# MiRaCLeXeoN/sduss

Measured on AMD Instinct MI355X. Metric: images/sec (node), SDXL 1024^2 50-step, fixed prompt, CFG, higher is better.
Workload: dtype bf16; 1 GPU; SDXL-base-1.0 UNet 1024x1024 50-step Euler, CFG 5.0, 4 requests/step (denoiser batch 8) per GPU, is_sliced=False, random-init weights of the real architecture (2.57 B params), one data-parallel replica per GPU, no collective; resolution=1024, steps_per_image=50

## Files before the change

### include/mxdenoise.h

```cpp
#ifndef MXDENOISE_H
#define MXDENOISE_H

#include <stddef.h>
#include <stdint.h>

#ifdef __cplusplus
extern "C" {
#endif

enum { MX_F32 = 0, MX_F16 = 1, MX_BF16 = 2 };

const char* mx_last_error(void);
int mx_version(void);
#define MX_PROF_KINDS 12
int mx_profile_enable(int on);
int mx_profile_collect(double* out);
int mx_profile_records(double* out, int max_records);

size_t mx_groupnorm_halo_workspace_bytes(int N, int C, int cpg);
int mx_groupnorm_halo(void* stream, const void* x, const void* gamma, const void* beta, void* y,
                      int N, int C, int H, int W, int cpg, double eps, int padding,
                      const int32_t* latent_offset, int n_latents, const int32_t* patch_map,
                      const int32_t* padding_idx, int dtype, void* workspace);
int mx_halo_only(void* stream, const void* x, void* y, int N, int C, int H, int W,
                 const int32_t* padding_idx, int dtype);


enum {
  MX_EPI_SILU     = 1 << 0,
  MX_EPI_GEGLU    = 1 << 1,
  MX_EPI_OUT_F32  = 1 << 2,
  MX_EPI_QKV      = 1 << 3,
  MX_EPI_GELU_TANH = 1 << 4,
  MX_EPI_RES_BCAST = 1 << 5,
  MX_EPI_RMSNORM  = 1 << 6,
  MX_EPI_GELU     = 1 << 7,
  MX_EPI_QUICK_GELU = 1 << 8,
  MX_EPI_GEGLU_TANH = 1 << 9
};

#define MX_MAX_SEGS 4
typedef struct mx_gemm_seg {
  const void* a;
  const void* a2;
  void* c;
  const void* residual;
  void* vt;
  const float* rowbias;
  const float* gate;
  const float* ln_stats;
  float* stats_out;
  int M;
  int rows_per_batch;
  int ldvt;
  int B, Hin, Win, Hout, Wout;
  int a_batch_rows, a_row_off, c_batch_rows, c_row_off;
} mx_gemm_seg;

typedef struct mx_gemm_desc {
  const void* a;
  const void* w;
  void* c;
  const float* bias;
  const float* rowbias;
  const void* residual;
  void* vt;
  int M, N, K;
  int lda, ldc, ldr, ldrb;
  int rows_per_batch;
  int flags;
  int seg, period, ldvt;
  int B, Hin, Win, Cin;
  int Hout, Wout;
  int stride;
  int up;
  int corner_patch;
  int a_batch_rows, a_row_off, c_batch_rows, c_row_off;
  const float* gate;
  int ldg;
  float out_scale;
  const float* rms_wq;
  const float* rms_wk;
  float rms_eps;
  int vhalo;
  const void* a2;
  int lda2, k_split;
  const float* ln_stats;
  const float* ln_colsum;
  int ln_slabs;
  float ln_eps;
  float* stats_out;
  const mx_gemm_seg* segs;
  int n_segs;
  int splitk;
  const float* ln_final;
  float* ln_final_out;
  unsigned* ln_final_cnt;
  float* gn_part_out;
  int cin_valid;
} mx_gemm_desc;

int mx_gemm(void* stream, const mx_gemm_desc* d);
int mx_gemm_launches(const mx_gemm_desc* d);
int mx_gemm_stats_slabs(const mx_gemm_desc* d);
int mx_gemm_ln_prefers_pass(const mx_gemm_desc* d);
int mx_gemm_ln_final_supported(const mx_gemm_desc* d);
int mx_gemm_gn_partials_supported(const mx_gemm_desc* d, int conv);
enum { MX_FORM_TILE_GENERIC = 0, MX_FORM_TILE_256 = 1, MX_FORM_TILE_128 = 2, MX_FORM_PERSISTENT_256 = 3, MX_FORM_SMALL_M = 4, MX_FORM_CONV_SMALL_N = 5, MX_FORM_CONV_SMALL_CIN = 6 };
int mx_gemm_form(const mx_gemm_desc* d, int conv);
int mx_gemm_kernel_name(const mx_gemm_desc* d, int conv, int launch, char* buf, int cap);
int mx_gemm_kernel_names(char* buf, int cap);
int mx_attention_kernel_name(int B, int H, int Lq, int Lk, int ldo, int prescaled, int causal, int bias, int key_chunk, int force_cross, char* buf, int cap);
int mx_attention_kernel_names(char* buf, int cap);
#define MX_STATS_PITCH(slabs) (((slabs) + 3) & ~3)
int mx_row_stats(void* stream, const void* x, int ldx, float* stats, int M, int C);
int mx_conv3x3(void* stream, const mx_gemm_desc* d);
int mx_gemm_splitk(const mx_gemm_desc* d, int conv);
void mx_gemm_release_scratch(void* stream, int all);

typedef struct mx_attn_tail_desc {
  mx_gemm_desc out1, to_q, out2;
  const void* k; int ldk;
  const void* vt; int ldvt; int64_t vt_batch_stride;
  int B, heads, L, ctx_len;
  unsigned* sync;
} mx_attn_tail_desc;
size_t mx_attn_tail_sync_bytes(int M);
int mx_attn_tail_supported(const mx_attn_tail_desc* d);
int mx_attn_tail_preferred(void);
int mx_attn_tail(void* stream, const mx_attn_tail_desc* d);
int mx_attn_tail_status(void* stream, const unsigned* sync, unsigned* word);

#define MX_VT_POS(key) (((key) & ~12) | (((key) & 4) << 1) | (((key) & 8) >> 1))
#define MX_VT_LD(Lk) (((Lk) + 15) / 16 * 16)

int mx_attention(void* stream, const void* q, int ldq, const void* k, int ldk, const void* vt, int ldvt,
                 int64_t vt_batch_stride, void* o, int ldo, int B, int H, int Lq, int Lk, float scale);
#define MX_ATTN_QSCALE(scale) ((scale) * 1.4426950408889634f)
int mx_attention_prescaled(void* stream, const void* q, int ldq, const void* k, int ldk, const void* vt, int ldvt,
                           int64_t vt_batch_stride, void* o, int ldo, int B, int H, int Lq, int Lk);
int mx_attention_cross_prescaled(void* stream, const void* q, int ldq, const void* k, int ldk, const void* vt, int ldvt,
                                 int64_t vt_batch_stride, void* o, int ldo, int B, int H, int Lq, int Lk);
typedef struct mx_attn_problem {
  const void* q; const void* k; const void* vt; void* o;
  int64_t vt_batch_stride;
  int B, Lq, Lk, ldvt;
} mx_attn_problem;
int mx_attention_prescaled_grouped(void* stream, const mx_attn_problem* probs, int n, int ldq, int ldk, int ldo, int H);
int mx_attention_prescaled_bias(void* stream, const void* q, int ldq, const void* k, int ldk, const void* vt, int ldvt,
                                int64_t vt_batch_stride, void* o, int ldo, int B, int H, int Lq, int Lk, const float* bias, int ldb);
int mx_attention_prescaled_causal(void* stream, const void* q, int ldq, const void* k, int ldk, const void* vt, int ldvt,
                                  int64_t vt_batch_stride, void* o, int ldo, int B, int H, int L);

int mx_layernorm(void* stream, const void* x, void* y, const float* gamma, const float* beta,
                 int M, int C, float eps);

int mx_rmsnorm(void* stream, const void* x, void* y, const float* w, int M, int C, float eps);

int mx_layernorm_mod(void* stream, const void* x, void* y, void* y2, const float* scale, const float* shift,
                     const float* scale2, const float* shift2, int ldmod, int M, int C, int rows_per_batch, float eps);
int mx_layernorm_mod_grouped(void* stream, const void* x, void* y, void* y2, const float* scale, const float* shift, const float* scale2,
                             const float* shift2, int ldmod, int C, float eps, const int* batches, const int* rows_per_batch, int n);
int mx_rmsnorm_heads(void* stream, void* x, int ld, int nbatch, int rows_per_batch, int batch_rows, int row_off,
                     int heads_total, int heads_q, const float* wq, const float* wk, float eps, float q_scale);

size_t mx_groupnorm_nhwc_workspace_bytes(int B, int H, int W, int C);
int mx_groupnorm_nhwc(void* stream, const void* x, void* y, const float* gamma, const float* beta,
                      int B, int H, int W, int C, int groups, float eps, int silu, int patch,
                      void* workspace);

int mx_groupnorm_nhwc_cat(void* stream, const void* x, int C1, const void* x2, void* y, const float* gamma, const float* beta,
                          int B, int H, int W, int C, int groups, float eps, int silu, int patch, void* workspace);
int mx_groupnorm_nhwc_from_partials(void* stream, const void* x, void* y, const float* gamma, const float* beta, int B, int H, int W, int C, int groups, float eps,
                                    int silu, const float* part, int chunk, const float* add_bias, const float* add_rowbias, int ldrb, void* workspace);

typedef struct mx_gn_problem { const void* x; const void* x2; void* y; int B, H, W; } mx_gn_problem;
size_t mx_groupnorm_nhwc_grouped_workspace_bytes(const mx_gn_problem* probs, int n, int C);
int mx_groupnorm_nhwc_grouped(void* stream, const mx_gn_problem* probs, int n, int C1, const float* gamma, const float* beta, int C, int groups,
                              float eps, int silu, int patch, void* workspace);

typedef struct mx_unet_config {
  int in_channels, out_channels;
  int n_levels;
  int block_out_channels[4];
  int layers_per_block;
  int down_has_attn[4];
  int transformer_layers[4];
  int num_heads[4];
  int cross_attention_dim;
  int addition_time_embed_dim;
  int projection_class_embeddings_input_dim;
  int norm_num_groups;
  float norm_eps, transformer_norm_eps, layer_norm_eps;
} mx_unet_config;

typedef struct mx_weight_entry {
  const char* name;
  uint64_t offset;
  uint64_t bytes;
} mx_weight_entry;

typedef struct mx_unet mx_unet;

mx_unet* mx_unet_create(const mx_unet_config* cfg);
void mx_unet_destroy(mx_unet* u);
int mx_unet_set_weights(mx_unet* u, const void* blob, uint64_t blob_bytes,
                        const mx_weight_entry* table, int n_entries);
int mx_unet_set_context_key(mx_unet* u, uint64_t key);
int mx_unet_context_stats(const mx_unet* u, long* hits, long* misses);
size_t mx_unet_workspace_bytes(const mx_unet* u, int batch, int H, int W, int ctx_len);
int mx_unet_validate(const mx_unet* u, int batch, int H, int W, int ctx_len);
int mx_unet_forward(mx_unet* u, void* stream, const void* latents, int io_dtype, const float* timesteps,
                    const void* ehs, const void* text_embeds, const float* time_ids, void* out,
                    int batch, int H, int W, int ctx_len, int gn_patch, void* workspace, size_t workspace_bytes);
typedef struct mx_unet_group { const void* latents; void* out; int batch, H, W; } mx_unet_group;
size_t mx_unet_workspace_bytes_mixed(const mx_unet* u, const mx_unet_group* groups, int n_groups, int ctx_len);
int mx_unet_forward_mixed(mx_unet* u, void* stream, const mx_unet_group* groups, int n_groups, int io_dtype, const float* timesteps,
                          const void* ehs, const void* text_embeds, const float* time_ids, int ctx_len, int gn_patch, void* workspace,
                          size_t workspace_bytes);
int mx_unet_forward_mixed_trace(mx_unet* u, void* stream, const mx_unet_group* groups, int n_groups, int io_dtype, const float* timesteps,
                                const void* ehs, const void* text_embeds, const float* time_ids, int ctx_len, int gn_patch, void* workspace,
                                size_t workspace_bytes, const char* stage, void* stage_out, size_t stage_out_bytes);
int mx_unet_forward_trace(mx_unet* u, void* stream, const void* latents, int io_dtype, const float* timesteps,
                          const void* ehs, const void* text_embeds, const float* time_ids, void* out,
                          int batch, int H, int W, int ctx_len, int gn_patch, void* workspace,
                          size_t workspace_bytes, const char* stage, void* stage_out, size_t stage_out_bytes);

typedef int (*mx_allgather_fn)(void* ctx, void* stream, const void* send, void* recv, size_t bytes_per_rank);
typedef struct mx_pp_comm { int rank, world; mx_allgather_fn all_gather; void* ctx; } mx_pp_comm;
size_t mx_unet_workspace_bytes_pp(const mx_unet* u, int batch, int H_local, int W, int ctx_len, int world);
int mx_unet_forward_pp(mx_unet* u, void* stream, const void* latents_local, int io_dtype, const float* timesteps, const void* ehs,
                       const void* text_embeds, const float* time_ids, void* out_local, int batch, int H_local, int W, int ctx_len,
                       const mx_pp_comm* comm, void* workspace, size_t workspace_bytes);
#define MX_PP_SYNC 0
#define MX_PP_WARMUP 1
#define MX_PP_STALE 2
typedef int (*mx_allgather_inplace_fn)(void* ctx, void* stream, void* region, size_t bytes_per_rank);
typedef struct mx_pp_stale { void* state; size_t state_bytes; int mode; int corrected_gn; mx_allgather_inplace_fn all_gather_async; } mx_pp_stale;
size_t mx_unet_pp_state_bytes(const mx_unet* u, int batch, int H_local, int W, int ctx_len, int world);
int mx_unet_forward_pp_stale(mx_unet* u, void* stream, const void* latents_local, int io_dtype, const float* timesteps, const void* ehs,
                             const void* text_embeds, const float* time_ids, void* out_local, int batch, int H_local, int W, int ctx_len,
                             const mx_pp_comm* comm, const mx_pp_stale* stale, void* workspace, size_t workspace_bytes);
int mx_unet_pp_comm_plan(const mx_unet* u, int batch, int H_local, int W, int ctx_len, const mx_pp_comm* comm);
int mx_attention_prescaled_chunked(void* stream, const void* q, int ldq, const void* k, int ldk, const void* vt, int ldvt,
                                   int64_t vt_batch_stride, void* o, int ldo, int B, int H, int Lq, int Lk, int key_chunk,
                                   int64_t k_batch_stride, int64_t k_chunk_stride, int64_t vt_chunk_stride);

typedef struct mx_mmdit_config {
  int patch_size, in_channels, out_channels;
  int num_layers;
  int num_attention_heads;
  int joint_attention_dim, pooled_projection_dim, pos_embed_max_size;
  int dual_attention[64];
  float norm_eps;
} mx_mmdit_config;

typedef struct mx_mmdit mx_mmdit;
mx_mmdit* mx_mmdit_create(const mx_mmdit_config* cfg);
void mx_mmdit_destroy(mx_mmdit* u);
int mx_mmdit_set_weights(mx_mmdit* u, const void* blob, uint64_t blob_bytes, const mx_weight_entry* table, int n_entries);
size_t mx_mmdit_workspace_bytes(const mx_mmdit* u, int batch, int H, int W, int ctx_len);
int mx_mmdit_validate(const mx_mmdit* u, int batch, int H, int W, int ctx_len);
int mx_mmdit_forward(mx_mmdit* u, void* stream, const void* latents, int io_dtype, const float* timesteps, const void* ehs,
                     const void* pooled, void* out, int batch, int H, int W, int ctx_len, void* workspace, size_t workspace_bytes);
// ... 117 lines not shown
```

### sduss_amd/csrc/gemm_args.h

```cpp
#pragma once
#include "common.h"
#include "../../include/mxdenoise.h"

namespace mx {

constexpr int kMaxSegs = MX_MAX_SEGS;
struct GemmSeg {
  const bf16_t* a; const bf16_t* a2; void* c; const bf16_t* residual; bf16_t* vt; const float* rowbias; const float* gate;
  const float* ln_stats; float* stats_out;
  int M, tile0, rows_per_batch, ldvt;
  int B, Hin, Win, Hout, Wout;
  int a_batch_rows, a_row_off, c_batch_rows, c_row_off;
};

struct GemmArgs {
  const bf16_t* a;
  const bf16_t* w;
  void* c;
  const float* bias;
  const float* rowbias;
  const bf16_t* residual;
  bf16_t* vt;
  int M, N, K;
  int lda, ldc, ldr, ldrb;
  int rows_per_batch;
  int flags;
  int seg, period, ldvt;
  int B, Hin, Win, Cin, Hout, Wout, stride, up, corner_patch;
  int a_batch_rows, a_row_off, c_batch_rows, c_row_off;
  const float* gate;
  int ldg;
  int xcd_map;
  float out_scale;
  const float* rms_wq;
  const float* rms_wk;
  float rms_eps;
  int stagger_ticks;
  int vhalo;
  const bf16_t* a2;
  int lda2, k_split;
  const float* ln_stats;
  const float* ln_colsum;
  int ln_slabs;
  float ln_eps;
  float* stats_out;
  const float* ln_final;
  float* ln_final_out;
  unsigned* ln_final_cnt;
  int ln_final_slabs;
  float* gn_part;
  int splitk;
  float* sk_ws;
  unsigned* sk_cnt;
  int nseg, mt_total;
  GemmSeg prob[kMaxSegs];
};

__device__ __forceinline__ int gemm_select_seg(GemmArgs& q, const GemmArgs& p, int& tm) {
  if (p.nseg <= 0) return 0;
  int s = 0;
#pragma unroll
  for (int i = 1; i < kMaxSegs; ++i) if (i < p.nseg && tm >= p.prob[i].tile0) s = i;
  const GemmSeg& g = p.prob[s];
  tm -= g.tile0;
  q.a = g.a; q.a2 = g.a2; q.c = g.c; q.residual = g.residual; q.vt = g.vt; q.rowbias = g.rowbias; q.gate = g.gate;
  q.ln_stats = g.ln_stats; q.stats_out = g.stats_out;
  q.M = g.M; q.rows_per_batch = g.rows_per_batch; q.ldvt = g.ldvt;
  q.B = g.B; q.Hin = g.Hin; q.Win = g.Win; q.Hout = g.Hout; q.Wout = g.Wout;
  q.a_batch_rows = g.a_batch_rows; q.a_row_off = g.a_row_off; q.c_batch_rows = g.c_batch_rows; q.c_row_off = g.c_row_off;
  return s;
}
__device__ __forceinline__ int gemm_m_tiles(const GemmArgs& p, int rows) { return p.nseg > 0 ? p.mt_total : (p.M + rows - 1) / rows; }

__device__ __forceinline__ f32x4 fma4(const f32x4 a, const float s, const f32x4 c) {
  return f32x4{fmaf(a[0], s, c[0]), fmaf(a[1], s, c[1]), fmaf(a[2], s, c[2]), fmaf(a[3], s, c[3])};
}

__device__ __forceinline__ float sum_over_fq(float x) {
  float a = x, b = x;
  asm volatile("s_nop 1\n\tv_permlane16_swap_b32 %0, %1" : "+v"(a), "+v"(b));
  a += b; b = a;
  asm volatile("s_nop 1\n\tv_permlane32_swap_b32 %0, %1" : "+v"(a), "+v"(b));
  return a + b;
}

template <int NI, int MI>
__device__ __forceinline__ void gemm_ln_init(const GemmArgs& p, f32x4 (&acc)[NI][MI], const int m_wave0, const int wave_n0, const int fr,
                                             const int fq, float (&rstd)[MI]) {
#pragma clang fp contract(off)
  const int slabs = p.ln_slabs;
  const int pitch = (slabs + 3) & ~3;
  float s1[MI], s2[MI];
#pragma unroll
  for (int j = 0; j < MI; ++j) { s1[j] = 0.f; s2[j] = 0.f; }
  for (int g = 4 * fq; g < slabs; g += 16) {
    constexpr int JC = MI > 4 ? 4 : MI;
#pragma unroll
    for (int j0 = 0; j0 < MI; j0 += JC) {
      f32x4 va[JC], vb[JC];
#pragma unroll
      for (int j = 0; j < JC; ++j) {
        const int m = m_wave0 + (j0 + j) * 16 + fr;
        const float* src = p.ln_stats + ((long)(m < p.M ? m : p.M - 1) * pitch + g) * 2;
        va[j] = *reinterpret_cast<const f32x4*>(src);
        vb[j] = *reinterpret_cast<const f32x4*>(src + 4);
      }
#pragma unroll
      for (int j = 0; j < JC; ++j) {
        s1[j0 + j] += va[j][0] + (g + 1 < slabs ? va[j][2] : 0.f) + (g + 2 < slabs ? vb[j][0] : 0.f) + (g + 3 < slabs ? vb[j][2] : 0.f);
        s2[j0 + j] += va[j][1] + (g + 1 < slabs ? va[j][3] : 0.f) + (g + 2 < slabs ? vb[j][1] : 0.f) + (g + 3 < slabs ? vb[j][3] : 0.f);
      }
    }
  }
  const float inv = 1.0f / (float)p.K;
  float nmean[MI];
#pragma unroll
  for (int j = 0; j < MI; ++j) {
    const float a = sum_over_fq(s1[j]), b = sum_over_fq(s2[j]);
    const float mean = a * inv;
    const float var = fmaxf(fmaf(-mean, mean, b * inv), 0.f);
    rstd[j] = rsqrtf(var + p.ln_eps);
    nmean[j] = -mean;
  }
#pragma unroll
  for (int i = 0; i < NI; ++i) {
    const int n = wave_n0 + i * 16 + fq * 4;
    const f32x4 cs = n < p.N ? *reinterpret_cast<const f32x4*>(p.ln_colsum + n) : f32x4{0.f, 0.f, 0.f, 0.f};
#pragma unroll
    for (int j = 0; j < MI; ++j) acc[i][j] = cs * nmean[j];
  }
}

__device__ __forceinline__ void gemm_ln_row(const GemmArgs& p, const int m, const int fq, float& rstd, float& rm) {
#pragma clang fp contract(off)
  const int mc = m < p.M ? m : p.M - 1;
  const int pitch = (p.ln_slabs + 3) & ~3;
  float s1 = 0.f, s2 = 0.f;
  for (int s = fq; s < p.ln_slabs; s += 4) {
    const f32x2 v = *reinterpret_cast<const f32x2*>(p.ln_stats + ((long)mc * pitch + s) * 2);
    s1 += v[0]; s2 += v[1];
  }
  s1 = sum_over_fq(s1); s2 = sum_over_fq(s2);
  const float inv = 1.0f / (float)p.K;
  const float mean = s1 * inv;
  const float var = fmaxf(fmaf(-mean, mean, s2 * inv), 0.f);
  rstd = rsqrtf(var + p.ln_eps);
  rm = rstd * mean;
}

__device__ __forceinline__ float row16_sum(float x) {
  x += __builtin_bit_cast(float, __builtin_amdgcn_update_dpp(0, __builtin_bit_cast(int, x), 0xB1, 0xF, 0xF, true));
  x += __builtin_bit_cast(float, __builtin_amdgcn_update_dpp(0, __builtin_bit_cast(int, x), 0x4E, 0xF, 0xF, true));
  x += __builtin_bit_cast(float, __builtin_amdgcn_update_dpp(0, __builtin_bit_cast(int, x), 0x141, 0xF, 0xF, true));
  x += __builtin_bit_cast(float, __builtin_amdgcn_update_dpp(0, __builtin_bit_cast(int, x), 0x140, 0xF, 0xF, true));
  return x;
}
template <int NI, int MI>
__device__ __forceinline__ void gemm_gn_partials(const GemmArgs& p, const f32x4 (&acc)[NI][MI], const int m_wave0, const int wave_n0, const int fr, const int fq) {
  static_assert(MI == 4, "one 64-token chunk per wave");
  if (m_wave0 >= p.M) return;
  float* dst = p.gn_part + ((long)(m_wave0 >> 6) * p.N + wave_n0 + fq * 4) * 2;
#pragma unroll
  for (int i = 0; i < NI; ++i) {
    f32x4 s = {0.f, 0.f, 0.f, 0.f}, q = {0.f, 0.f, 0.f, 0.f};
#pragma unroll
    for (int j = 0; j < MI; ++j) { s += acc[i][j]; q += acc[i][j] * acc[i][j]; }
#pragma unroll
    for (int e = 0; e < 4; ++e) { s[e] = row16_sum(s[e]); q[e] = row16_sum(q[e]); }
    if (fr == 0) {
      *reinterpret_cast<f32x4*>(dst + i * 32) = f32x4{s[0], q[0], s[1], q[1]};
      *reinterpret_cast<f32x4*>(dst + i * 32 + 4) = f32x4{s[2], q[2], s[3], q[3]};
    }
  }
}

__device__ __forceinline__ void gemm_ln_finalize(const GemmArgs& p, const int tm, const int nt, volatile int* ticket_word) {
#pragma clang fp contract(off)
  const int tid = threadIdx.x;
  asm volatile("s_waitcnt vmcnt(0)" ::: "memory");
  __syncthreads();
  if (tid == 0) *ticket_word = (int)__hip_atomic_fetch_add(p.ln_final_cnt + tm, 1u, __ATOMIC_RELAXED, __HIP_MEMORY_SCOPE_AGENT);
  __syncthreads();
  if (*ticket_word != nt - 1) return;
  if (tid == 0) __hip_atomic_store(p.ln_final_cnt + tm, 0u, __ATOMIC_RELAXED, __HIP_MEMORY_SCOPE_AGENT);
  const int slabs = p.ln_final_slabs;
  const int pitch = (slabs + 3) & ~3;
  const int m = tm * 256 + (tid >> 1);
  const int half = (slabs + 1) >> 1;
  const int s0 = (tid & 1) ? half : 0, s1 = (tid & 1) ? slabs : half;
  float a = 0.f, q = 0.f;
  if (m < p.M) {
    const unsigned long long* src = reinterpret_cast<const unsigned long long*>(p.stats_out + (long)m * pitch * 2);
    for (int s = s0; s < s1; ++s) {
      const unsigned long long v = __hip_atomic_load(src + s, __ATOMIC_RELAXED, __HIP_MEMORY_SCOPE_AGENT);
      a += __uint_as_float((unsigned)v); q += __uint_as_float((unsigned)(v >> 32));
    }
  }
  const float a2 = __shfl_xor(a, 1, 64), q2 = __shfl_xor(q, 1, 64);
  if (!(tid & 1) && m < p.M) {
    const float inv = 1.0f / (float)p.N;
    const float mean = (a + a2) * inv;
    const float var = fmaxf(fmaf(-mean, mean, (q + q2) * inv), 0.f);
    *reinterpret_cast<f32x2*>(p.ln_final_out + (long)m * 2) = f32x2{mean, rsqrtf(var + p.ln_eps)};
  }
}

template <int NI, int MI, bool KEEP>
__device__ __forceinline__ void gemm_ln_init_final(const GemmArgs& p, f32x4 (&acc)[NI][MI], const int m_wave0, const int wave_n0, const int fr,
// ... 573 lines not shown
```

### sduss_amd/csrc/gemm_bf16.hip

```cpp
#include <algorithm>
#include <cstdlib>

#include <mutex>
#include <unordered_map>

#include "common.h"
#include "../../include/mxdenoise.h"
#include "gemm_args.h"
#include "gemm_forms.h"

namespace mx {

constexpr int BM = 128;
constexpr int BK = 64;

__device__ __forceinline__ int swz(int row, int chunk) { return chunk ^ ((row >> 1) & 7); }

template <int BN, bool CONV>
__global__ __launch_bounds__(256, 2) void gemm_kernel(const GemmArgs pk) {
  constexpr int NI = BN / 32;
  constexpr int MI = 4;
  constexpr int WROWS = BN / 32;
  __shared__ __attribute__((aligned(16))) bf16_t sX[2][BM * BK];
  __shared__ __attribute__((aligned(16))) bf16_t sW[2][BN * BK];
// ... 55 lines not shown
        else rx[i] = (xoff[i] >= 0) ? *reinterpret_cast<const u32x4*>(p.a + xoff[i] + k0) : zero4;
      }
    } else {
      const int tap = k0 / p.Cin;
      const int c0 = k0 - tap * p.Cin;
      const int dy = tap / 3 - 1;
      const int dx = tap - (tap / 3) * 3 - 1;
      const int Hv = p.Hin << p.up, Wv = p.Win << p.up;
      const int P = p.corner_patch;
#pragma unroll
      for (int i = 0; i < 4; ++i) {
        int iy = cy[i] + dy;
        const int ix = cx[i] + dx;
        if (P > 0 && dy != 0 && dx != 0) {
          const bool cross_r = ((iy + P) / P) != ((cy[i] + P) / P);
          const bool cross_c = ((ix + P) / P) != ((cx[i] + P) / P);
          if (cross_r && cross_c) iy = cy[i];
        }
        const bool ok = (cb[i] >= 0) && (iy >= -p.vhalo) && (iy < Hv + p.vhalo) && (ix >= 0) && (ix < Wv);
        if (ok) {
          const long src = (((long)cb[i] * (p.Hin + 2 * p.vhalo) + (iy >> p.up) + p.vhalo) * p.Win + (ix >> p.up)) * p.Cin + c0 + sch * 8;
          rx[i] = *reinterpret_cast<const u32x4*>(p.a + src);
        } else {
          rx[i] = zero4;
        }
      }
    }
#pragma unroll
    for (int i = 0; i < WROWS; ++i)
      rw[i] = (woff[i] >= 0) ? *reinterpret_cast<const u32x4*>(p.w + woff[i] + k0) : zero4;
  };
  auto store_tile = [&](int buf) {
#pragma unroll
    for (int i = 0; i < 4; ++i) {
      const int row = srow + 32 * i;
      *reinterpret_cast<u32x4*>(&sX[buf][row * BK + swz(row, sch) * 8]) = rx[i];
    }
#pragma unroll
    for (int i = 0; i < WROWS; ++i) {
      const int row = srow + 32 * i;
      *reinterpret_cast<u32x4*>(&sW[buf][row * BK + swz(row, sch) * 8]) = rw[i];
    }
  };

  f32x4 acc[NI][MI];
#pragma unroll
  for (int i = 0; i < NI; ++i)
#pragma unroll
    for (int j = 0; j < MI; ++j) acc[i][j] = f32x4{0.f, 0.f, 0.f, 0.f};

  const int fr = lane & 15;
  const int fq = lane >> 4;

  load_tile(0);
  store_tile(0);
  __syncthreads();

  for (int kt = 0; kt < nk; ++kt) {
    const int buf = kt & 1;
    if (kt + 1 < nk) load_tile(kt + 1);
#pragma unroll
    for (int ks = 0; ks < 2; ++ks) {
      bf16x8 wf[NI], xf[MI];
#pragma unroll
      for (int i = 0; i < NI; ++i) {
        const int row = wn * (BN / 2) + i * 16 + fr;
        wf[i] = *reinterpret_cast<const bf16x8*>(&sW[buf][row * BK + swz(row, ks * 4 + fq) * 8]);
      }
#pragma unroll
      for (int j = 0; j < MI; ++j) {
        const int row = wm * 64 + j * 16 + fr;
        xf[j] = *reinterpret_cast<const bf16x8*>(&sX[buf][row * BK + swz(row, ks * 4 + fq) * 8]);
      }
#pragma unroll
      for (int i = 0; i < NI; ++i)
#pragma unroll
        for (int j = 0; j < MI; ++j)
          acc[i][j] = __builtin_amdgcn_mfma_f32_16x16x32_bf16(wf[i], xf[j], acc[i][j], 0, 0, 0);
    }
    if (kt + 1 < nk) store_tile(buf ^ 1);
    __syncthreads();
  }

  gemm_epilogue<NI, MI, BN>(p, acc, m0 + wm * 64, n0 + wn * (BN / 2), fr, fq);
}

int launch_v2(hipStream_t s, const GemmArgs& a, int bn, int form);
int launch_v5(hipStream_t s, const GemmArgs& a, int bn, int rows, int form);
int launch_v4(hipStream_t s, const GemmArgs& a, int form);
bool small_m_serves(const mx_gemm_desc* d, bool conv);
int small_m_form(long N, long K, int flags);
int launch_small_m(hipStream_t s, const GemmArgs& a, int form);
bool conv_small_n_serves(const mx_gemm_desc* d);
int launch_conv_small_n(hipStream_t s, const GemmArgs& a);
bool conv_small_cin_serves(const mx_gemm_desc* d);
int launch_conv_small_cin(hipStream_t s, const GemmArgs& a);

constexpr size_t kSplitKWsBytes = 96u << 20;
constexpr size_t kSplitKCntBytes = 64u << 10;
struct TileChoice { int bn; int rows; int splitk = 1; };
static long m_tiles_of(const mx_gemm_desc* d, int rows) {
  if (d->n_segs <= 0) return cdiv(d->M, rows);
  long t = 0;
  for (int i = 0; i < d->n_segs; ++i) t += cdiv(d->segs[i].M, rows);
  return t;
}
static long rows_of(const mx_gemm_desc* d) {
  if (d->n_segs <= 0) return d->M;
  long m = 0;
  for (int i = 0; i < d->n_segs; ++i) m += d->segs[i].M;
  return m;
}
static TileChoice pick_tile(const mx_gemm_desc* d, bool conv) {
  constexpr double v3_discount = 0.87;
  const TileChoice none = {0, 0};
  const long Mtot = rows_of(d);
  if (Mtot < 128 || d->K < 128) return none;
  if (d->flags & (MX_EPI_OUT_F32 | MX_EPI_RES_BCAST)) return none;
  if (d->n_segs <= 0) { if (d->rows_per_batch > 0 && d->rows_per_batch < 16) return none; }
  else for (int i = 0; i < d->n_segs; ++i) if (d->segs[i].rows_per_batch > 0 && d->segs[i].rows_per_batch < 16) return none;
  if (d->ldc % 8 != 0 || ((uintptr_t)d->c & 15) != 0) return none;
  if (d->residual && (d->ldr % 8 != 0 || ((uintptr_t)d->residual & 15) != 0)) return none;
  const bool geglu = (d->flags & MX_EPI_GEGLU) != 0, qkv = (d->flags & MX_EPI_QKV) != 0;
  bool fits32 = (long)d->N * d->K * 2 < (1L << 32);
  if (d->n_segs <= 0) {
    const long in_rows = d->a_batch_rows > 0 ? (long)(d->M / d->rows_per_batch + 1) * d->a_batch_rows : d->M;
    fits32 = fits32 && in_rows * d->lda * 2 < (1L << 32);
  } else {
    uintptr_t lo = (uintptr_t)d->segs[0].a;
    for (int i = 1; i < d->n_segs; ++i) lo = std::min(lo, (uintptr_t)d->segs[i].a);
    for (int i = 0; i < d->n_segs; ++i) {
      const mx_gemm_seg& g = d->segs[i];
      const long in_rows = g.a_batch_rows > 0 ? (long)(g.M / std::max(g.rows_per_batch, 1) + 1) * g.a_batch_rows : g.M;
      fits32 = fits32 && (long)((uintptr_t)g.a - lo) + in_rows * d->lda * 2 < (1L << 32);
    }
  }
  TileChoice best = none;
  double best_cost = 0;
  const TileChoice cands[5] = {{256, 256}, {160, 256}, {128, 256}, {160, 128}, {128, 128}};
  for (int c = 0; c < 5; ++c) {
    const int bn = cands[c].bn, rows = cands[c].rows;
    if (d->N % bn != 0 || Mtot < rows) continue;
    if (bn == 256 && (conv || !fits32 || d->a2 || d->ln_stats || d->stats_out)) continue;
    if (d->ln_final && bn != 256) continue;
    if (geglu && bn == 160) continue;
    if (qkv && d->seg % 64 != 0) continue;
    if ((d->flags & MX_EPI_RMSNORM) && bn == 160) continue;
    if (qkv && bn != 256 && d->seg % (bn / 2) != 0) continue;
    const long tiles = m_tiles_of(d, rows) * (d->N / bn);
    const int ncu = cu_count();
    const double cost = (double)((tiles + ncu - 1) / ncu) * (rows + bn) * (bn == 256 ? v3_discount : 1.0);
    if (best.rows == 0 || cost < best_cost) { best = cands[c]; best_cost = cost; }
  }
  if (d->splitk != 1 && best.rows == 128 && !d->a2 && d->K / 64 >= 16) {
    const int ncu = cu_count();
    const int nk = d->K / 64;
    double best_t = 0, unsplit_t = 0;
    TileChoice pick = best;
    const double mtot = (double)Mtot;
    for (int c = 3; c < 5; ++c) {
      const int bn = cands[c].bn;
      if (d->N % bn != 0 || (geglu && bn == 160) || (qkv && (d->seg % 64 != 0 || d->seg % (bn / 2) != 0)) || ((d->flags & MX_EPI_RMSNORM) && bn == 160)) continue;
      const long tiles = m_tiles_of(d, 128) * (d->N / bn);
      for (int sk = 1; sk <= 4; ++sk) {
        if (d->splitk > 1 && sk != 1 && sk != d->splitk) continue;
        if (nk / sk < 8 || (sk > 1 && tiles * sk > 2L * ncu)) continue;
        if (sk > 1 && (tiles * sk * 128L * bn * 4 > (long)kSplitKWsBytes || tiles * 4 > (long)kSplitKCntBytes)) continue;
        const double combine = sk > 1 ? 2.0 + (double)sk * mtot * d->N * 8.0 / 4.0e6 : 0.0;
        const double t = (double)((tiles * sk + ncu - 1) / ncu) * ((double)(nk / sk) * 0.57 * (128 + bn) / 256.0 + 5.0) + combine;
        if (sk == 1 && bn == best.bn) unsplit_t = t;
        if (best_t == 0 || t < best_t - 1e-9) { best_t = t; pick = TileChoice{bn, 128, sk}; }
      }
    }
    if (pick.splitk > 1 && unsplit_t > 0 && best_t <= 0.75 * unsplit_t) best = pick;
    if (d->splitk > 1) {
      double ft = 0;
      for (int c = 3; c < 5; ++c) {
        const int bn = cands[c].bn, sk = d->splitk;
        if (d->N % bn != 0 || (geglu && bn == 160) || (qkv && (d->seg % 64 != 0 || d->seg % (bn / 2) != 0)) || ((d->flags & MX_EPI_RMSNORM) && bn == 160)) continue;
        const long tiles = m_tiles_of(d, 128) * (d->N / bn);
        if (sk > 4 || nk / sk < 8 || tiles * sk * 128L * bn * 4 > (long)kSplitKWsBytes || tiles * 4 > (long)kSplitKCntBytes) continue;
        const double t = (double)((tiles * sk + ncu - 1) / ncu) * ((double)(nk / sk) * 0.57 * (128 + bn) / 256.0 + 5.0);
        if (ft == 0 || t < ft) { ft = t; best = TileChoice{bn, 128, sk}; }
      }
    }
  }
  return best;
}

struct SplitKScratch { float* ws = nullptr; unsigned* cnt = nullptr; };
struct SplitKPool {
  std::mutex mu;
  std::unordered_map<hipStream_t, SplitKScratch> per_stream;
  static void drop(SplitKScratch& b) { if (b.ws) (void)hipFree(b.ws); if (b.cnt) (void)hipFree(b.cnt); b = SplitKScratch{}; }
  ~SplitKPool() { for (auto& kv : per_stream) drop(kv.second); }
};
static SplitKPool& splitk_pool() { static SplitKPool p; return p; }
static bool splitk_scratch(hipStream_t s, SplitKScratch& out) {
  SplitKPool& pool = splitk_pool();
  std::lock_guard<std::mutex> lock(pool.mu);
  auto it = pool.per_stream.find(s);
  if (it != pool.per_stream.end()) { out = it->second; return out.ws != nullptr; }
  hipStreamCaptureMode mode = hipStreamCaptureModeRelaxed;
  (void)hipThreadExchangeStreamCaptureMode(&mode);
  SplitKScratch b;
  hipStream_t z = nullptr;
  bool ok = hipMalloc(&b.ws, kSplitKWsBytes) == hipSuccess && hipMalloc(&b.cnt, kSplitKCntBytes) == hipSuccess &&
            hipStreamCreateWithFlags(&z, hipStreamNonBlocking) == hipSuccess && hipMemsetAsync(b.cnt, 0, kSplitKCntBytes, z) == hipSuccess &&
            hipStreamSynchronize(z) == hipSuccess;
  if (z) (void)hipStreamDestroy(z);
  (void)hipThreadExchangeStreamCaptureMode(&mode);
  if (!ok) { (void)hipGetLastError(); SplitKPool::drop(b); return false; }
  pool.per_stream[s] = b;
  out = b;
  return true;
}
static void splitk_release(hipStream_t s, bool all) {
  SplitKPool& pool = splitk_pool();
  std::lock_guard<std::mutex> lock(pool.mu);
  if (all) { for (auto& kv : pool.per_stream) { (void)hipStreamSynchronize(kv.first); SplitKPool::drop(kv.second); } pool.per_stream.clear(); return; }
  auto it = pool.per_stream.find(s);
  if (it == pool.per_stream.end()) return;
  (void)hipStreamSynchronize(s);
  SplitKPool::drop(it->second);
  pool.per_stream.erase(it);
}

static int stats_slabs_of(const mx_gemm_desc* d, bool conv, const TileChoice& tc) {
  if (conv || tc.bn == 0 || tc.bn == 256) return 0;
  if (d->flags & (MX_EPI_GEGLU | MX_EPI_QKV | MX_EPI_OUT_F32)) return 0;
  if (d->a_batch_rows > 0 || d->c_batch_rows > 0) return 0;
  for (int i = 0; i < d->n_segs; ++i) if (d->segs[i].a_batch_rows > 0 || d->segs[i].c_batch_rows > 0) return 0;
  const int panel = tc.bn / 2;
  return d->N / panel;
}

static bool is_small_m_form(int form) {
  switch (form) {
#define MX_SM(id, k, targs) case id: return true;
    MX_GEMM_SMALL_M_FORMS(MX_SM)
#undef MX_SM
    default: return false;
  }
}

static int gemm_kernel_of(const mx_gemm_desc* d, bool conv, const TileChoice& tc) {
  if (d->ln_final && tc.bn != 256) return -1;
  if (small_m_serves(d, conv)) return small_m_form(d->N, d->K, d->flags);
  if (conv && conv_small_n_serves(d)) return GK_CONV_SMALL_N;
  if (conv && conv_small_cin_serves(d)) return GK_CONV_SMALL_CIN;
  const int feat = gemm_epi_features(d->flags);
  const bool geglu = (d->flags & MX_EPI_GEGLU) != 0;
  const bool vec = d->rowbias || d->gate;
  if (tc.bn == 256) {
    if (d->ln_final) {
      if (geglu) return (feat & EPI_F_ACT) ? -1 : GK_V4_GEGLU_LN;
      return feat == EPI_F_QKV ? GK_V4_QKV_LN : feat == 0 ? GK_V4_LN : -1;
    }
    if (geglu) return (feat & EPI_F_ACT) ? GK_V4_GEGLU_ACT : GK_V4_GEGLU;
    if (!vec) return feat == 0 ? GK_V4 : feat == EPI_F_QKV ? GK_V4_QKV : feat == EPI_F_TANH ? GK_V4_TANH : GK_V4_VEC_ALL;
    return feat == 0 ? GK_V4_VEC : GK_V4_VEC_ALL;
  }
  if (tc.bn != 0 && tc.rows == 256) {
    const bool b160 = tc.bn == 160;
    if (geglu) return (feat & EPI_F_ACT) ? GK_V5_128_GEGLU_ACT : GK_V5_128_GEGLU;
    if (conv) {
      if (feat == 0 && !vec) return b160 ? GK_V5_160_CONV : GK_V5_128_CONV;
      if (feat == 0) return b160 ? GK_V5_160_CONV_VEC : GK_V5_128_CONV_VEC;
      return b160 ? GK_V5_160_CONV_ALL : GK_V5_128_CONV_ALL;
    }
    if (feat == 0 && !vec) return b160 ? GK_V5_160 : GK_V5_128;
    if (feat == EPI_F_QKV && !vec) return b160 ? GK_V5_160_QKV : GK_V5_128_QKV;
    return b160 ? GK_V5_160_ALL : GK_V5_128_ALL;
  }
  if (tc.bn != 0) {
    const bool b160 = tc.bn == 160;
    if (geglu) return (feat & EPI_F_ACT) ? GK_V2_128_GEGLU_ACT : GK_V2_128_GEGLU;
    if (conv) return feat == 0 ? (b160 ? GK_V2_160_CONV : GK_V2_128_CONV) : (b160 ? GK_V2_160_CONV_ALL : GK_V2_128_CONV_ALL);
    if (feat == 0) return b160 ? GK_V2_160 : GK_V2_128;
    if (feat == EPI_F_QKV) return b160 ? GK_V2_160_QKV : GK_V2_128_QKV;
    return b160 ? GK_V2_160_ALL : GK_V2_128_ALL;
  }
  if (d->N % 128 == 0) return conv ? GK_GEN128_CONV : GK_GEN128;
  return conv ? GK_GEN64_CONV : GK_GEN64;
}

static int prepare(void* stream, const mx_gemm_desc* d, bool conv, GemmArgs& a, TileChoice& tc_out) {
  MX_CHECK(d != nullptr, "gemm: null descriptor");
  MX_CHECK(d->a && d->w && (d->c || (d->flags & MX_EPI_QKV)), "gemm: null operand");
  MX_CHECK(d->n_segs >= 0 && d->n_segs <= MX_MAX_SEGS && (d->n_segs == 0 || d->segs != nullptr), "gemm: bad n_segs / segs");
  MX_CHECK((d->n_segs > 0 || d->M > 0) && d->N > 0 && d->K > 0, "gemm: empty problem");
  for (int i = 0; i < d->n_segs; ++i) {
    const mx_gemm_seg& g = d->segs[i];
    MX_CHECK(g.M > 0 && g.a && (g.c != nullptr) == (d->c != nullptr), "gemm: grouped launch: empty problem or missing a / c");
    MX_CHECK((g.a2 != nullptr) == (d->a2 != nullptr && !conv) && (g.residual != nullptr) == (d->residual != nullptr) && (g.vt != nullptr) == (d->vt != nullptr) &&
             (g.rowbias != nullptr) == (d->rowbias != nullptr) && (g.gate != nullptr) == (d->gate != nullptr) &&
             (g.ln_stats != nullptr) == (d->ln_stats != nullptr) && (g.stats_out != nullptr) == (d->stats_out != nullptr),
             "gemm: grouped launch: a problem's optional operands must match the descriptor's");
    const void* ptrs[] = {g.a, g.a2, g.c, g.residual, g.vt, g.rowbias, g.gate, g.ln_stats, g.stats_out};
    for (const void* q : ptrs) MX_CHECK(((uintptr_t)q & 15) == 0, "gemm: grouped launch: operand pointers must be 16-byte aligned");
    if (d->rowbias || d->gate || g.a_batch_rows > 0 || g.c_batch_rows > 0 || (d->flags & (MX_EPI_QKV | MX_EPI_RES_BCAST)))
      MX_CHECK(g.rows_per_batch > 0, "gemm: grouped launch: rows_per_batch required");
    if (g.a_batch_rows > 0) MX_CHECK(!conv && g.a_row_off >= 0 && g.a_row_off + g.rows_per_batch <= g.a_batch_rows, "gemm: grouped launch: bad input row remap");
    if (g.c_batch_rows > 0) MX_CHECK(g.c_row_off >= 0 && g.c_row_off + g.rows_per_batch <= g.c_batch_rows, "gemm: grouped launch: bad output row remap");
    if (d->ln_stats || d->stats_out)
      MX_CHECK(g.a_batch_rows <= 0 && g.c_batch_rows <= 0, "gemm: grouped launch: the folded LayerNorm / stats_out exclude a problem's row remaps");
    if (d->flags & MX_EPI_QKV)
      MX_CHECK(g.M % g.rows_per_batch == 0 && g.ldvt >= MX_VT_LD(g.c_batch_rows > 0 ? g.c_batch_rows : g.rows_per_batch) && g.ldvt % 8 == 0,
               "gemm: grouped launch: QKV needs whole batches and ldvt >= MX_VT_LD(keys per batch)");
    if (conv) {
      const int Hv = g.Hin << d->up, Wv = g.Win << d->up;
      MX_CHECK(g.Hout == (Hv + d->stride - 1) / d->stride && g.Wout == (Wv + d->stride - 1) / d->stride && (long)g.B * g.Hout * g.Wout == g.M,
               "conv3x3: grouped launch: a problem's output grid does not match its input grid / stride / rows");
    }
    MX_CHECK((long)g.M * (conv ? 1 : d->lda) < 2147483647L, "gemm: grouped launch: operand exceeds 32-bit indexing");
  }
  MX_CHECK(d->K % BK == 0, "gemm: K must be a multiple of 64");
  MX_CHECK(d->N % 4 == 0, "gemm: N must be a multiple of 4");
  a.stagger_ticks = 0;
  a.vhalo = conv ? d->vhalo : 0;
  a.a2 = conv ? nullptr : (const bf16_t*)d->a2; a.lda2 = d->lda2; a.k_split = d->k_split;
  a.a = (const bf16_t*)d->a; a.w = (const bf16_t*)d->w; a.c = d->c;
  a.bias = d->bias; a.rowbias = d->rowbias; a.residual = (const bf16_t*)d->residual; a.vt = (bf16_t*)d->vt;
  a.M = d->M; a.N = d->N; a.K = d->K; a.lda = d->lda; a.ldc = d->ldc; a.ldr = d->ldr; a.ldrb = d->ldrb;
  a.rows_per_batch = d->rows_per_batch; a.flags = d->flags; a.seg = d->seg; a.period = d->period; a.ldvt = d->ldvt;
  a.B = d->B; a.Hin = d->Hin; a.Win = d->Win; a.Cin = d->Cin; a.Hout = d->Hout; a.Wout = d->Wout;
  a.stride = d->stride; a.up = d->up; a.corner_patch = d->corner_patch;
  a.a_batch_rows = d->a_batch_rows; a.a_row_off = d->a_row_off; a.c_batch_rows = d->c_batch_rows; a.c_row_off = d->c_row_off;
  a.gate = d->gate; a.ldg = d->ldg; a.out_scale = d->out_scale;
  a.rms_wq = d->rms_wq; a.rms_wk = d->rms_wk; a.rms_eps = d->rms_eps;
  a.ln_stats = d->ln_stats; a.ln_colsum = d->ln_colsum; a.ln_slabs = d->ln_slabs; a.ln_eps = d->ln_eps; a.stats_out = nullptr;
  a.ln_final = nullptr; a.ln_final_out = nullptr; a.ln_final_cnt = nullptr; a.ln_final_slabs = 0;
  if (d->ln_final) {
    MX_CHECK(!conv && !d->ln_stats && d->ln_colsum && d->n_segs == 0, "gemm: ln_final needs ln_colsum, excludes ln_stats and grouped launches (mx_gemm only)");
    MX_CHECK(!(d->flags & MX_EPI_RMSNORM) && d->a_batch_rows <= 0 && d->c_batch_rows <= 0 && !d->a2 && !d->rowbias && !d->gate && !d->stats_out,
             "gemm: ln_final excludes RMSNORM, the row remaps, the split A operand, per-sample vectors and stats_out");
    MX_CHECK((((uintptr_t)d->ln_final & 15) | ((uintptr_t)d->ln_colsum & 15)) == 0, "gemm: ln_final / ln_colsum must be 16-byte aligned");
    a.ln_final = d->ln_final;
  }
  a.nseg = d->n_segs; a.mt_total = 0;
  const bool grouped = d->n_segs > 0;
  if (d->ln_stats) {
    MX_CHECK(!conv && d->ln_colsum && d->ln_slabs > 0, "gemm: folded LayerNorm needs ln_colsum and ln_slabs > 0 (mx_gemm only)");
    MX_CHECK(!(d->flags & MX_EPI_RMSNORM) && d->a_batch_rows <= 0 && d->c_batch_rows <= 0 && !d->a2, "gemm: folded LayerNorm excludes RMSNORM, the row remaps and the split A operand");
    MX_CHECK((((uintptr_t)d->ln_stats & 15) | ((uintptr_t)d->ln_colsum & 15)) == 0, "gemm: ln_stats / ln_colsum must be 16-byte aligned");
  }
  a.xcd_map = 1;

  if (!conv && d->a2) {
    MX_CHECK(d->k_split > 0 && d->k_split < d->K && d->k_split % BK == 0, "gemm: k_split must be a multiple of 64 inside (0, K)");
    MX_CHECK(d->lda >= d->k_split && d->lda % 8 == 0 && d->lda2 >= d->K - d->k_split && d->lda2 % 8 == 0, "gemm: bad lda / lda2 for the split A operand");
    MX_CHECK(d->a_batch_rows <= 0 && ((uintptr_t)d->a2 & 15) == 0 && rows_of(d) * d->lda2 < 2147483647L, "gemm: split A operand excludes the row remap and needs 16-byte alignment");
  } else if (!conv) {
    MX_CHECK(d->lda >= d->K && d->lda % 8 == 0, "gemm: lda must be >= K and a multiple of 8");
  } else {
    MX_CHECK(d->Cin % BK == 0 && d->K == 9 * d->Cin, "conv3x3: Cin must be a multiple of 64 and K = 9*Cin");
    MX_CHECK(d->stride == 1 || d->stride == 2, "conv3x3: stride must be 1 or 2");
    MX_CHECK(d->up == 0 || d->up == 1, "conv3x3: up must be 0 or 1");
    MX_CHECK(!(d->up && d->stride != 1), "conv3x3: upsample only with stride 1");
    if (!grouped) {
      const int Hv = d->Hin << d->up, Wv = d->Win << d->up;
      MX_CHECK(d->Hout == (Hv + d->stride - 1) / d->stride && d->Wout == (Wv + d->stride - 1) / d->stride,
               "conv3x3: output grid does not match input grid / stride");
      MX_CHECK((long)d->B * d->Hout * d->Wout == d->M, "conv3x3: M != B*Hout*Wout");
    }
    MX_CHECK(2 * d->Cin <= 16384, "conv3x3: Cin > 8192 (the pipelined loader walks a 16 KB zero page for padding taps)");
    MX_CHECK(!(d->flags & MX_EPI_GEGLU), "conv3x3: no GEGLU epilogue");
    MX_CHECK(d->vhalo == 0 || (d->vhalo == 1 && d->corner_patch == 0), "conv3x3: vhalo must be 0 or 1 and excludes the sliced corner rule");
  }
  {
    const void* ptrs[] = {d->a, d->w, d->c, d->bias, d->rowbias, d->residual, d->gate, d->rms_wq, d->rms_wk};
    for (const void* q : ptrs) MX_CHECK(((uintptr_t)q & 15) == 0, "gemm: operand pointers must be 16-byte aligned");
  }
  if (!grouped && (d->rowbias || d->gate || d->a_batch_rows > 0 || d->c_batch_rows > 0 || (d->flags & (MX_EPI_QKV | MX_EPI_RES_BCAST))))
    MX_CHECK(d->rows_per_batch > 0, "gemm: rows_per_batch required");
  if (d->gate) MX_CHECK(d->ldg >= d->N && d->ldg % 4 == 0, "gemm: bad ldg");
  if (!grouped && d->a_batch_rows > 0) MX_CHECK(!conv && d->a_row_off >= 0 && d->a_row_off + d->rows_per_batch <= d->a_batch_rows, "gemm: bad input row remap");
  if (!grouped && d->c_batch_rows > 0) MX_CHECK(d->c_row_off >= 0 && d->c_row_off + d->rows_per_batch <= d->c_batch_rows, "gemm: bad output row remap");
  if (d->rowbias) MX_CHECK(d->ldrb >= d->N && d->ldrb % 4 == 0, "gemm: bad ldrb");
  if (!grouped) {
    const long in_rows = (!conv && d->a_batch_rows > 0) ? (long)(d->M / d->rows_per_batch + 1) * d->a_batch_rows : d->M;
    MX_CHECK(in_rows * (conv ? 1 : d->lda) < 2147483647L, "gemm: operand exceeds 32-bit indexing");
  }
  MX_CHECK((long)d->N * d->K < 2147483647L, "gemm: operand exceeds 32-bit indexing");
  if (d->residual) MX_CHECK(d->ldr >= d->N && d->ldr % 4 == 0, "gemm: bad ldr");
  const bool use128 = (d->N % 128 == 0);
  const TileChoice tc = pick_tile(d, conv);
  tc_out = tc;
  a.splitk = 0; a.sk_ws = nullptr; a.sk_cnt = nullptr;
  if (tc.splitk > 1) {
    SplitKScratch sk;
    MX_CHECK(splitk_scratch((hipStream_t)stream, sk), "gemm: the split-K scratch (96 MB per stream) could not be allocated; set mx_gemm_desc.splitk = 1 to run unsplit");
    a.splitk = tc.splitk; a.sk_ws = sk.ws; a.sk_cnt = sk.cnt;
  }
  if (d->stats_out) {
    MX_CHECK(stats_slabs_of(d, conv, tc) > 0, "gemm: stats_out is not supported for this shape / epilogue (see mx_gemm_stats_slabs)");
    MX_CHECK(((uintptr_t)d->stats_out & 15) == 0, "gemm: stats_out must be 16-byte aligned");
    a.stats_out = d->stats_out;
  }
  a.gn_part = nullptr;
  if (d->gn_part_out) {
    MX_CHECK(!grouped && tc.rows == 256 && tc.bn != 256 && tc.bn != 0 && tc.splitk <= 1, "gemm: gn_part_out needs an ungrouped launch on a 256-row tile (mx_gemm_gn_partials_supported)");
    MX_CHECK(d->flags == 0 && !d->residual && !d->gate && d->out_scale == 0.f && !d->ln_stats && !d->ln_final && d->a_batch_rows <= 0 && d->c_batch_rows <= 0,
             "gemm: gn_part_out needs an epilogue of bias (+ row bias) only");
    MX_CHECK(d->M % 64 == 0 && (!d->rowbias || d->rows_per_batch % 64 == 0) && ((uintptr_t)d->gn_part_out & 15) == 0, "gemm: gn_part_out needs M % 64 == 0, rows_per_batch % 64 == 0 and 16-byte alignment");
    a.gn_part = d->gn_part_out;
  }
  if (d->ln_final_out) {
    MX_CHECK(d->stats_out && d->ln_final_cnt && !grouped && tc.rows == 256 && tc.bn != 256 && tc.bn != 0,
             "gemm: ln_final_out needs stats_out, ln_final_cnt and an ungrouped launch on a 256-row tile (mx_gemm_ln_final_supported)");
    MX_CHECK((((uintptr_t)d->ln_final_out & 15) | ((uintptr_t)d->ln_final_cnt & 3)) == 0, "gemm: ln_final_out must be 16-byte aligned");
    a.ln_final_out = d->ln_final_out; a.ln_final_cnt = d->ln_final_cnt; a.ln_final_slabs = stats_slabs_of(d, conv, tc);
  }
  if (grouped) {
    const int rows = tc.rows > 0 ? tc.rows : BM;
    uintptr_t lo = (uintptr_t)d->segs[0].a;
    int t0 = 0;
    for (int i = 0; i < d->n_segs; ++i) {
      const mx_gemm_seg& g = d->segs[i];
      GemmSeg& o = a.prob[i];
      o.a = (const bf16_t*)g.a; o.a2 = conv ? nullptr : (const bf16_t*)g.a2; o.c = g.c; o.residual = (const bf16_t*)g.residual; o.vt = (bf16_t*)g.vt;
      o.rowbias = g.rowbias; o.gate = g.gate; o.ln_stats = g.ln_stats; o.stats_out = d->stats_out ? g.stats_out : nullptr;
      o.M = g.M; o.tile0 = t0; o.rows_per_batch = g.rows_per_batch; o.ldvt = g.ldvt;
      o.B = g.B; o.Hin = g.Hin; o.Win = g.Win; o.Hout = g.Hout; o.Wout = g.Wout;
      o.a_batch_rows = g.a_batch_rows; o.a_row_off = g.a_row_off; o.c_batch_rows = g.c_batch_rows; o.c_row_off = g.c_row_off;
      t0 += cdiv(g.M, rows);
      lo = std::min(lo, (uintptr_t)g.a);
    }
    a.mt_total = t0;
    a.a = (const bf16_t*)lo;
    a.M = (int)rows_of(d);
  }
  if (d->flags & MX_EPI_GEGLU) {
    MX_CHECK(use128, "gemm: GEGLU needs N % 128 == 0");
    MX_CHECK(!(d->flags & (MX_EPI_QKV | MX_EPI_OUT_F32)) && !d->residual && !d->rowbias && d->out_scale == 0.f, "gemm: GEGLU excludes other epilogues");
    MX_CHECK(d->ldc >= d->N / 2 && d->ldc % 4 == 0, "gemm: bad ldc for GEGLU");
  } else if (d->flags & MX_EPI_QKV) {
    MX_CHECK(d->seg > 0 && d->seg % 64 == 0 && d->period >= 2 && d->N % (d->seg * d->period) == 0, "gemm: bad QKV segments");
    MX_CHECK(d->vt != nullptr, "gemm: QKV needs vt");
    if (!grouped) {
      MX_CHECK(d->ldvt >= MX_VT_LD(d->c_batch_rows > 0 ? d->c_batch_rows : d->rows_per_batch), "gemm: QKV needs ldvt >= MX_VT_LD(keys per batch)");
      MX_CHECK(d->M % d->rows_per_batch == 0, "gemm: QKV needs M % rows_per_batch == 0");
    }
    MX_CHECK(d->ldc >= d->N / d->period * (d->period - 1) && d->ldc % 4 == 0, "gemm: bad ldc for QKV");
    MX_CHECK(!(d->flags & MX_EPI_OUT_F32), "gemm: QKV output is bf16");
    MX_CHECK(!d->rowbias && !d->gate && !d->residual, "gemm: QKV excludes the per-sample vectors and the residual (its V^T segment takes none of them)");
    if (d->flags & MX_EPI_RMSNORM)
      MX_CHECK(d->rms_wq && d->rms_wk && d->period == 3 && d->N % 128 == 0 && !conv, "gemm: RMSNORM needs rms_wq/rms_wk, period 3, N % 128 == 0");
  } else {
    MX_CHECK(d->ldc >= d->N && d->ldc % 4 == 0, "gemm: bad ldc");
  }
  return 0;
}

int gemm_prepare_for_chain(void* stream, const mx_gemm_desc* d, GemmArgs& a, int& bn, int& rows, int& splitk) {
  TileChoice tc;
  if (int rc = prepare(stream, d, false, a, tc)) return rc;
  bn = tc.bn; rows = tc.rows; splitk = tc.splitk;
  return 0;
}

static int launch(void* stream, const mx_gemm_desc* d, bool conv) {
  GemmArgs a;
  TileChoice tc;
  if (int rc = prepare(stream, d, conv, a, tc)) return rc;
  const bool grouped = d->n_segs > 0;
  const bool use128 = (d->N % 128 == 0);
  const int v2bn = tc.bn;
  dim3 block(256);
  hipStream_t s = (hipStream_t)stream;
  if (prof_enabled()) {
    const double kk = conv ? 9.0 * d->Cin : (double)d->K;
    const double Mt = (double)rows_of(d);
    double in_elems = conv ? (double)d->B * d->Hin * d->Win * d->Cin : Mt * d->K;
    if (conv && grouped) { in_elems = 0; for (int i = 0; i < d->n_segs; ++i) in_elems += (double)d->segs[i].B * d->segs[i].Hin * d->segs[i].Win * d->Cin; }
    const double flops = 2.0 * Mt * (double)d->N * kk;
    const double bytes = 2.0 * (in_elems + (double)d->N * d->K + Mt * d->N);
    const int kind = v2bn == 256 ? PROF_GEMM_V3_256 : v2bn ? (conv ? PROF_CONV_V2_160 : PROF_GEMM_V2_160) + (v2bn == 160 ? 0 : 2) : (conv ? PROF_CONV128 : PROF_GEMM128) + (use128 ? 0 : 1);
    prof_begin(s, kind, flops, bytes, (int)Mt, d->N, (int)kk);
  }
  const int mt128 = grouped ? a.mt_total : cdiv(d->M, BM);
  if (d->ln_final) MX_CHECK(v2bn == 256, "gemm: ln_final is the 256 x 256 kernel's form of the folded LayerNorm; this shape does not run there (use ln_stats)");
  const int form = gemm_kernel_of(d, conv, tc);
  MX_CHECK(form >= 0, v2bn == 256 ? "gemm: no 256 x 256 instantiation serves ln_final with this epilogue (GEGLU, QKV or plain bias only)"
                                   : "gemm: no kernel instantiation serves this descriptor");
  if (is_small_m_form(form)) {
    MX_CHECK(launch_small_m(s, a, form) == 0, "gemm: the small-M launcher was handed a form outside its list");
  } else if (form == GK_CONV_SMALL_N) {
    launch_conv_small_n(s, a);
  } else if (form == GK_CONV_SMALL_CIN) {
    launch_conv_small_cin(s, a);
  } else if (v2bn == 256) {
    MX_CHECK(launch_v4(s, a, form) == 0, "gemm: no 256 x 256 instantiation serves ln_final with this epilogue (GEGLU, QKV or plain bias only)");
  } else if (v2bn) {
    if (tc.rows == 256) MX_CHECK(launch_v5(s, a, v2bn, tc.rows, form) == 0, "gemm: the 256-row launcher was handed a form outside its list");
    else MX_CHECK(launch_v2(s, a, v2bn, form) == 0, "gemm: the 128-row launcher was handed a form outside its list");
  } else {
    const dim3 grid(mt128, use128 ? d->N / 128 : cdiv(d->N, 64));
    switch (form) {
#define MX_GEN(id, k, targs) case id: hipLaunchKernelGGL((k<MX_FORM_UNPAREN targs>), grid, block, 0, s, a); break;
      MX_GEMM_GENERIC_FORMS(MX_GEN)
#undef MX_GEN
      default: MX_CHECK(false, "gemm: the generic launcher was handed a form outside its list");
    }
  }
  prof_end(s);
  MX_LAUNCH_CHECK();
  return 0;
}

}

namespace mx {
static bool tail_split(const mx_gemm_desc* d, mx_gemm_desc& d1, mx_gemm_desc& d2) {
  if (d->n_segs != 0 || d->M <= 0 || d->N <= 0 || d->K <= 0 || d->N % 256 != 0) return false;
  if (d->flags & (MX_EPI_QKV | MX_EPI_OUT_F32 | MX_EPI_RES_BCAST | MX_EPI_RMSNORM)) return false;
  if (d->stats_out || d->ln_stats || d->ln_final || d->ln_final_out || d->a_batch_rows > 0 || d->c_batch_rows > 0 || d->splitk > 1) return false;
  if (pick_tile(d, false).bn != 256) return false;
  const int ncu = cu_count();
  if (ncu <= 0) return false;
  const long mt = cdiv(d->M, 256), nt = d->N / 256, tiles = mt * nt;
  const long full = tiles / ncu, rem = tiles % ncu;
  if (full < 1 || rem == 0 || rem * 2 > ncu || (full * ncu) % mt != 0) return false;
  const long nt1 = full * ncu / mt;
  if (nt1 <= 0 || nt1 >= nt) return false;
  const int N1 = (int)nt1 * 256, N2 = d->N - N1;
  const bool geglu = (d->flags & MX_EPI_GEGLU) != 0;
  const long cofs = geglu ? N1 / 2 : N1;
  d1 = *d; d2 = *d;
  d1.N = N1; d2.N = N2;
  d1.splitk = 1; d2.splitk = 1;
  d2.w = (const char*)d->w + (size_t)N1 * d->K * 2;
  if (d->bias) d2.bias = d->bias + N1;
  d2.c = (char*)d->c + (size_t)cofs * 2;
  if (geglu && d->residual) return false;
  if (d->residual) d2.residual = (const char*)d->residual + (size_t)N1 * 2;
  if (d->rowbias) d2.rowbias = d->rowbias + N1;
  if (d->gate) d2.gate = d->gate + N1;
  const TileChoice t2 = pick_tile(&d2, false);
  if (t2.bn == 0 || t2.bn == 256 || t2.rows + t2.bn > 384) return false;
  if (m_tiles_of(&d2, t2.rows) * (N2 / t2.bn) > ncu) return false;
  return pick_tile(&d1, false).bn == 256;
}
}

extern "C" int mx_gemm(void* stream, const mx_gemm_desc* d) {
  mx_gemm_desc d1, d2;
  if (d != nullptr && mx::tail_split(d, d1, d2)) { if (int rc = mx::launch(stream, &d1, false)) return rc; return mx::launch(stream, &d2, false); }
  return mx::launch(stream, d, false);
}
extern "C" int mx_gemm_launches(const mx_gemm_desc* d) { mx_gemm_desc d1, d2; return d != nullptr && mx::tail_split(d, d1, d2) ? 2 : 1; }
extern "C" int mx_gemm_form(const mx_gemm_desc* d, int conv) {
  if (!d || mx::rows_of(d) <= 0 || d->N <= 0 || d->K <= 0) return MX_FORM_TILE_GENERIC;
  if (mx::small_m_serves(d, conv != 0)) return MX_FORM_SMALL_M;
  if (conv && mx::conv_small_n_serves(d)) return MX_FORM_CONV_SMALL_N;
  if (conv && mx::conv_small_cin_serves(d)) return MX_FORM_CONV_SMALL_CIN;
  const mx::TileChoice tc = mx::pick_tile(d, conv != 0);
  return tc.bn == 256 ? MX_FORM_PERSISTENT_256 : tc.bn == 0 ? MX_FORM_TILE_GENERIC : tc.rows == 256 ? MX_FORM_TILE_256 : MX_FORM_TILE_128;
}
extern "C" int mx_gemm_stats_slabs(const mx_gemm_desc* d) {
  if (!d || mx::rows_of(d) <= 0 || d->N <= 0 || d->K <= 0) return 0;
  mx_gemm_desc q = *d;
  if (!q.stats_out) q.stats_out = reinterpret_cast<float*>(16);
  return mx::stats_slabs_of(&q, false, mx::pick_tile(&q, false));
}
extern "C" int mx_gemm_ln_prefers_pass(const mx_gemm_desc* d) {
  if (!d || mx::rows_of(d) <= 0 || d->N <= 0 || d->K <= 0) return 0;
  mx_gemm_desc plain = *d;
  plain.ln_stats = nullptr; plain.stats_out = nullptr;
  return mx::pick_tile(&plain, false).bn == 256;
}
extern "C" int mx_gemm_gn_partials_supported(const mx_gemm_desc* d, int conv) {
  if (!d || d->n_segs > 0 || d->M <= 0 || d->N <= 0 || d->K <= 0 || d->M % 64 != 0) return 0;
  if (d->flags != 0 || d->residual || d->gate || d->out_scale != 0.f || d->ln_stats || d->ln_final || d->a_batch_rows > 0 || d->c_batch_rows > 0) return 0;
  if (d->rowbias && (d->rows_per_batch <= 0 || d->rows_per_batch % 64 != 0)) return 0;
  const mx::TileChoice tc = mx::pick_tile(d, conv != 0);
  return tc.rows == 256 && tc.bn != 256 && tc.bn != 0 && tc.splitk <= 1;
}
extern "C" int mx_gemm_ln_final_supported(const mx_gemm_desc* d) {
  if (!d || d->n_segs > 0 || d->M <= 0 || d->N <= 0 || d->K <= 0) return 0;
  mx_gemm_desc q = *d;
  if (!q.stats_out) q.stats_out = reinterpret_cast<float*>(16);
  const mx::TileChoice tc = mx::pick_tile(&q, false);
  return tc.rows == 256 && tc.bn != 256 && tc.bn != 0 && mx::stats_slabs_of(&q, false, tc) > 0;
}
extern "C" int mx_conv3x3(void* stream, const mx_gemm_desc* d) { return mx::launch(stream, d, true); }
extern "C" void mx_gemm_release_scratch(void* stream, int all) { mx::splitk_release((hipStream_t)stream, all != 0); }
extern "C" int mx_gemm_splitk(const mx_gemm_desc* d, int conv) {
  if (!d || mx::rows_of(d) <= 0 || d->N <= 0 || d->K <= 0) return 0;
  return mx::pick_tile(d, conv != 0).splitk;
}

namespace mx {
static const char* const kGemmKernelNames[GK_COUNT] = {
  MX_GEMM_GENERIC_FORMS(MX_FORM_NAME_T) MX_GEMM_V2_FORMS(MX_FORM_NAME_T) MX_GEMM_V5_FORMS(MX_FORM_NAME_T) MX_GEMM_V4_FORMS(MX_FORM_NAME_T)
  MX_GEMM_SMALL_M_FORMS(MX_FORM_NAME_T) MX_GEMM_CONV_SMALL_FORMS(MX_FORM_NAME_P)
};
}
extern "C" int mx_gemm_kernel_name(const mx_gemm_desc* d, int conv, int launch, char* buf, int cap) {
  if (!d || mx::rows_of(d) <= 0 || d->N <= 0 || d->K <= 0 || launch < 0) return -1;
  mx_gemm_desc d1, d2;
  const mx_gemm_desc* q = d;
  if (!conv && mx::tail_split(d, d1, d2)) { if (launch > 1) return 0; q = launch == 0 ? &d1 : &d2; }
  else if (launch > 0) return 0;
  const int form = mx::gemm_kernel_of(q, conv != 0, mx::pick_tile(q, conv != 0));
  if (form < 0) return -1;
  return mx::copy_name(mx::kGemmKernelNames[form], buf, cap);
}
extern "C" int mx_gemm_kernel_names(char* buf, int cap) { return mx::join_names(mx::kGemmKernelNames, mx::GK_COUNT, buf, cap); }
```

### sduss_amd/csrc/gemm_bf16_v2.hip

```cpp
#include <cstdlib>

#include "common.h"
#include "../../include/mxdenoise.h"
#include "gemm_args.h"
#include "gemm_forms.h"
#include "gemm_dma_loader.h"

namespace mx {

template <int BN, int MI> struct RingDepth { static constexpr int value = MI == 4 ? 3 : (BN == 160 ? 4 : 5); };

template <int BN, int MI, bool CONV, int FEAT, bool GEGLU>
__global__ __launch_bounds__(512, 2) void gemm_v2_kernel(const GemmArgs pk) {
  constexpr int BM2 = 64 * MI;
  constexpr int NI = BN / 32;
  constexpr int LOADS = DmaTile<BN, MI>::LOADS;
  constexpr int NSTAGE = RingDepth<BN, MI>::value;
  __shared__ __attribute__((aligned(16))) bf16_t smem[NSTAGE * DmaTile<BN, MI>::STAGE_ELEMS];

  const int tid = threadIdx.x;
  const int lane = tid & 63;
  const int wave = __builtin_amdgcn_readfirstlane(tid >> 6);
  const int wm = wave >> 1;
  const int wn = wave & 1;
  GemmArgs p = pk;
  int tm, tn;
  const int n_tiles = gemm_m_tiles(pk, BM2) * (pk.N / BN);
  const int slice = pk.splitk > 1 ? (int)blockIdx.x / n_tiles : 0;
  const int tile_id = (int)blockIdx.x - slice * n_tiles;
  gemm_tile_of_block(tile_id, gemm_m_tiles(pk, BM2), pk.N / BN, pk.xcd_map, tm, tn);
  gemm_select_seg(p, pk, tm);
  const int nk_all = p.K / DMA_BK;
  const int k_first = pk.splitk > 1 ? (int)((long)nk_all * slice / pk.splitk) : 0;
  const int nk = pk.splitk > 1 ? (int)((long)nk_all * (slice + 1) / pk.splitk) - k_first : nk_all;
  constexpr bool SPLIT_K = true;
#include "gemm_dma_loader.inc"
  auto issue_next = [&](int stage) __attribute__((always_inline)) { issue_group(stage); advance_cursor(); };

  const int fr = lane & 15;
  const int fq = lane >> 4;

  auto load_frags = [&](int stage, int ks, bf16x8 (&wf)[NI], bf16x8 (&xf)[MI]) {
    const bf16_t* sx = smem + stage * STAGE_ELEMS;
    const bf16_t* sw = sx + BM2 * DMA_BK;
#pragma unroll
    for (int i = 0; i < NI; ++i) {
      const int row = wn * (BN / 2) + i * 16 + fr;
      wf[i] = *reinterpret_cast<const bf16x8*>(&sw[row * DMA_BK + swz(row, ks * 4 + fq) * 8]);
    }
#pragma unroll
    for (int j = 0; j < MI; ++j) {
      const int row = wm * 16 * MI + j * 16 + fr;
      xf[j] = *reinterpret_cast<const bf16x8*>(&sx[row * DMA_BK + swz(row, ks * 4 + fq) * 8]);
    }
  };
  constexpr int NM = NI * MI;
  constexpr int NF = NI + MI;

  setup_tile();
#pragma unroll
  for (int st = 0; st < NSTAGE - 1; ++st) issue_next(st);

  int stage = 0;
  {
    f32x4 acc[NI][MI];
#pragma unroll
    for (int i = 0; i < NI; ++i)
#pragma unroll
      for (int j = 0; j < MI; ++j) acc[i][j] = f32x4{0.f, 0.f, 0.f, 0.f};
    float ln_rstd[MI];
#pragma unroll
    for (int j = 0; j < MI; ++j) ln_rstd[j] = 1.0f;
    if constexpr (!CONV) {
      if (p.ln_stats != nullptr) {
        gemm_ln_init<NI, MI>(p, acc, tm * BM2 + wm * 16 * MI, tn * BN + wn * (BN / 2), fr, fq, ln_rstd);
        if (slice != 0) {
#pragma unroll
          for (int i = 0; i < NI; ++i)
#pragma unroll
            for (int j = 0; j < MI; ++j) acc[i][j] = f32x4{0.f, 0.f, 0.f, 0.f};
        }
      }
    }

    for (int kt = 0; kt < nk; ++kt) {
      constexpr int INFLIGHT = LOADS * (NSTAGE - 2);
      wait_vmcnt<INFLIGHT>();
      __builtin_amdgcn_s_barrier();
      bf16x8 wf0[NI], xf0[MI], wf1[NI], xf1[MI];
      load_frags(stage, 0, wf0, xf0);
      const int st2 = stage >= 1 ? stage - 1 : NSTAGE - 1;
      issue_group(st2);
      load_frags(stage, 1, wf1, xf1);
#pragma unroll
      for (int i = 0; i < NI; ++i)
#pragma unroll
        for (int j = 0; j < MI; ++j)
          acc[i][j] = __builtin_amdgcn_mfma_f32_16x16x32_bf16(wf0[i], xf0[j], acc[i][j], 0, 0, 0);
#pragma unroll
      for (int i = 0; i < NI; ++i)
#pragma unroll
        for (int j = 0; j < MI; ++j)
          acc[i][j] = __builtin_amdgcn_mfma_f32_16x16x32_bf16(wf1[i], xf1[j], acc[i][j], 0, 0, 0);
      __builtin_amdgcn_sched_group_barrier(0x100, NF, 0);
#pragma unroll
      for (int s = 0; s < LOADS; ++s) {
        __builtin_amdgcn_sched_group_barrier(0x008, 1, 0);
        __builtin_amdgcn_sched_group_barrier(0x020, 1, 0);
      }
#pragma unroll
      for (int s = 0; s < (NF + 1) / 2; ++s) {
        __builtin_amdgcn_sched_group_barrier(0x008, 1, 0);
        __builtin_amdgcn_sched_group_barrier(0x100, 2, 0);
      }
      __builtin_amdgcn_sched_group_barrier(0x008, 2 * NM - LOADS - (NF + 1) / 2, 0);
      advance_cursor();
      stage = stage == NSTAGE - 1 ? 0 : stage + 1;
    }

    const int m0 = tm * BM2, n0 = tn * BN;
    if (pk.splitk > 1) {
      if (!splitk_combine<NI, MI>(pk, acc, tile_id, slice, BM2 * BN, reinterpret_cast<volatile int*>(smem))) return;
    }
    static_assert(!GEGLU || (NI % 4 == 0 && !CONV), "the gated epilogue pairs whole 32-feature halves");
    gemm_epilogue_regs<NI, MI, GEGLU, true, true, true, FEAT>(p, acc, m0 + wm * 16 * MI, n0 + wn * (BN / 2), fr, fq, ln_rstd);
    wait_vmcnt<0>();
  }
}

int launch_v2(hipStream_t s, const GemmArgs& a, int bn, int form) {
  const int tiles = (a.nseg > 0 ? a.mt_total : cdiv(a.M, 128)) * (a.N / bn) * (a.splitk > 1 ? a.splitk : 1);
  dim3 grid(tiles), block(512);
  switch (form) {
#define MX_V2(id, k, targs) case id: hipLaunchKernelGGL((k<MX_FORM_UNPAREN targs>), grid, block, 0, s, a); return 0;
    MX_GEMM_V2_FORMS(MX_V2)
#undef MX_V2
    default: return 1;
  }
}

}
```

### sduss_amd/csrc/gemm_bf16_v5.hip

```cpp
#include <cstdlib>

#include "common.h"
#include "../../include/mxdenoise.h"
#include "gemm_args.h"
#include "gemm_forms.h"
#include "gemm_v5_body.h"

namespace mx {

template <int BN, int MI, bool CONV, int FEAT, bool GEGLU, bool VEC>
__global__ __launch_bounds__(512, 2) void gemm_v5_kernel(const GemmArgs pk) {
  constexpr int STAGE_ELEMS = (64 * MI + BN) * DMA_BK;
  __shared__ __attribute__((aligned(16))) bf16_t smem[NSTAGE5 * STAGE_ELEMS];
  int tm, tn;
  gemm_tile_of_block(blockIdx.x, gemm_m_tiles(pk, 64 * MI), pk.N / BN, pk.xcd_map, tm, tn);
  gemm_v5_tile<BN, MI, CONV, FEAT, GEGLU, VEC>(pk, tm, tn, smem);
}

int launch_v5(hipStream_t s, const GemmArgs& a, int bn, int rows, int form) {
  const int tiles = (a.nseg > 0 ? a.mt_total : cdiv(a.M, rows)) * (a.N / bn);
  dim3 grid(tiles), block(512);
  switch (form) {
#define MX_V5(id, k, targs) case id: hipLaunchKernelGGL((k<MX_FORM_UNPAREN targs>), grid, block, 0, s, a); return 0;
    MX_GEMM_V5_FORMS(MX_V5)
#undef MX_V5
    default: return 1;
  }
}

}

#if defined(MX_EXP) && MX_EXP == 8
extern "C" int mx_debug_v5_stamps(unsigned long long* out) { return (int)hipMemcpyFromSymbol(out, HIP_SYMBOL(mx::g_v5_stamps), sizeof(mx::g_v5_stamps)); }
#endif
```

### sduss_amd/csrc/gemm_dma_loader.inc

```
  constexpr int BM = DmaTile<BN, MI>::BM, WCH = DmaTile<BN, MI>::WCH, XI = DmaTile<BN, MI>::XI, WI = DmaTile<BN, MI>::WI, STAGE_ELEMS = DmaTile<BN, MI>::STAGE_ELEMS;
  const char* zero = reinterpret_cast<const char*>(g_zero_page);
  const int cs = tid & 7;
  const int tiles_per_tap = CONV ? p.Cin / DMA_BK : 1;

  bool parked = false;
  int is_kt = 0;
  const char* xsrc[XI];
  long xjump[XI];
  const char* wsrc[WI];
  int cb[XI], cy[XI], cx[XI];
  unsigned xchb[XI];
  int tap_next = 0, in_tap = 0;

  auto conv_set_tap = [&](int tap, int cbyte = 0) __attribute__((always_inline)) {
    const int dy = tap / 3 - 1;
    const int dx = tap - (tap / 3) * 3 - 1;
    const int Hv = p.Hin << p.up, Wv = p.Win << p.up;
    const int P = p.corner_patch;
#pragma unroll
    for (int i = 0; i < XI; ++i) {
      int iy = cy[i] + dy;
      const int ix = cx[i] + dx;
      if (P > 0 && dy != 0 && dx != 0) {
        const bool cross_r = ((iy + P) / P) != ((cy[i] + P) / P);
        const bool cross_c = ((ix + P) / P) != ((cx[i] + P) / P);
        if (cross_r && cross_c) iy = cy[i];
      }
      const bool ok = (cb[i] >= 0) && (iy >= -p.vhalo) && (iy < Hv + p.vhalo) && (ix >= 0) && (ix < Wv);
      const long off = ((((long)cb[i] * (p.Hin + 2 * p.vhalo) + (iy >> p.up) + p.vhalo) * p.Win + (ix >> p.up)) * p.Cin) * 2;
      xsrc[i] = (ok ? reinterpret_cast<const char*>(p.a) + off + cbyte : zero) + xchb[i];
    }
  };

  auto setup_tile = [&]() __attribute__((always_inline)) {
    const int m0 = tm * BM;
    const int n0 = tn * BN;
#pragma unroll
    for (int i = 0; i < XI; ++i) {
      const int row = (i * 512 + tid) >> 3;
      const int ch = swz(row, cs);
      const int m = m0 + row;
      if constexpr (!CONV) {
        const int mc = m < p.M ? m : p.M - 1;
        xsrc[i] = reinterpret_cast<const char*>(p.a) + (gemm_in_row(p, mc) * p.lda + ch * 8) * 2;
        xjump[i] = p.a2 != nullptr ? (reinterpret_cast<const char*>(p.a2) + ((long)mc * p.lda2 + ch * 8) * 2) - (xsrc[i] + (long)p.k_split * 2) : 0;
      } else {
        xchb[i] = ch * 16;
        if (m < p.M) {
          const int hw = p.Hout * p.Wout;
          const int b = m / hw;
          const int r = m - b * hw;
          const int oy = r / p.Wout;
          cb[i] = b; cy[i] = oy * p.stride; cx[i] = (r - oy * p.Wout) * p.stride;
        } else {
          cb[i] = -1; cy[i] = 0; cx[i] = 0;
        }
      }
    }
    if constexpr (SPLIT_K) { tap_next = CONV ? k_first / tiles_per_tap : 0; in_tap = CONV ? k_first - tap_next * tiles_per_tap : 0; }
    if constexpr (CONV) conv_set_tap(tap_next, in_tap * DMA_BK * 2);
    else if constexpr (SPLIT_K) {
#pragma unroll
      for (int i = 0; i < XI; ++i) xsrc[i] += (long)k_first * DMA_BK * 2;
    }
#pragma unroll
    for (int i = 0; i < WI; ++i) {
      int q = i * 512 + tid;
      if (q >= WCH) q -= WCH;
      const int row = q >> 3;
      wsrc[i] = reinterpret_cast<const char*>(p.w) + ((long)(n0 + row) * p.K + (long)k_first * DMA_BK + swz(row, cs) * 8) * 2;
    }
  };
  auto park_on_zero_page = [&]() __attribute__((always_inline)) {
#pragma unroll
    for (int i = 0; i < XI; ++i) xsrc[i] = zero + lane * 16;
#pragma unroll
    for (int i = 0; i < WI; ++i) wsrc[i] = zero + lane * 16;
  };

  auto issue_group = [&](int stage) __attribute__((always_inline)) {
    bf16_t* st = smem + stage * STAGE_ELEMS;
    bf16_t* sw = st + BM * DMA_BK;
#pragma unroll
    for (int i = 0; i < XI; ++i) glds16(xsrc[i], st + (i * 512 + wave * 64) * 8);
#pragma unroll
    for (int i = 0; i < WI; ++i) {
      const int qb = (i * 512 + wave * 64 >= WCH) ? i * 512 + wave * 64 - WCH : i * 512 + wave * 64;
      glds16(wsrc[i], sw + qb * 8);
    }
  };
  auto advance_cursor = [&]() __attribute__((always_inline)) {
    if (parked) return;
    if (++is_kt == nk) {
      is_kt = 0;
      parked = true;
      park_on_zero_page();
      return;
    }
#pragma unroll
    for (int i = 0; i < WI; ++i) wsrc[i] += DMA_BK * 2;
    if constexpr (!CONV) {
      const bool to_a2 = p.a2 != nullptr && is_kt * DMA_BK == p.k_split;
#pragma unroll
      for (int i = 0; i < XI; ++i) xsrc[i] += DMA_BK * 2 + (to_a2 ? xjump[i] : 0L);
    } else {
      if (++in_tap == tiles_per_tap) {
        in_tap = 0;
        conv_set_tap(++tap_next);
      } else {
#pragma unroll
        for (int i = 0; i < XI; ++i) xsrc[i] += DMA_BK * 2;
      }
    }
  };
```

### sduss_amd/csrc/gemm_forms.h

```cpp
#pragma once

#define MX_GEMM_GENERIC_FORMS(T)                          \
  T(GK_GEN64, gemm_kernel, (64, false))                   \
  T(GK_GEN64_CONV, gemm_kernel, (64, true))               \
  T(GK_GEN128, gemm_kernel, (128, false))                 \
  T(GK_GEN128_CONV, gemm_kernel, (128, true))

#define MX_GEMM_V2_FORMS(T)                                                    \
  T(GK_V2_128_GEGLU_ACT, gemm_v2_kernel, (128, 2, false, EPI_F_ACT, true))     \
  T(GK_V2_128_GEGLU, gemm_v2_kernel, (128, 2, false, 0, true))                 \
  T(GK_V2_160_CONV, gemm_v2_kernel, (160, 2, true, 0, false))                  \
  T(GK_V2_160_CONV_ALL, gemm_v2_kernel, (160, 2, true, EPI_F_ALL, false))      \
  T(GK_V2_128_CONV, gemm_v2_kernel, (128, 2, true, 0, false))                  \
  T(GK_V2_128_CONV_ALL, gemm_v2_kernel, (128, 2, true, EPI_F_ALL, false))      \
  T(GK_V2_160, gemm_v2_kernel, (160, 2, false, 0, false))                      \
  T(GK_V2_160_QKV, gemm_v2_kernel, (160, 2, false, EPI_F_QKV, false))          \
  T(GK_V2_160_ALL, gemm_v2_kernel, (160, 2, false, EPI_F_ALL, false))          \
  T(GK_V2_128, gemm_v2_kernel, (128, 2, false, 0, false))                      \
  T(GK_V2_128_QKV, gemm_v2_kernel, (128, 2, false, EPI_F_QKV, false))          \
  T(GK_V2_128_ALL, gemm_v2_kernel, (128, 2, false, EPI_F_ALL, false))

#define MX_GEMM_V5_FORMS(T)                                                           \
  T(GK_V5_128_GEGLU_ACT, gemm_v5_kernel, (128, 4, false, EPI_F_ACT, true, false))     \
  T(GK_V5_128_GEGLU, gemm_v5_kernel, (128, 4, false, 0, true, false))                 \
  T(GK_V5_160_CONV, gemm_v5_kernel, (160, 4, true, 0, false, false))                  \
  T(GK_V5_160_CONV_VEC, gemm_v5_kernel, (160, 4, true, 0, false, true))               \
  T(GK_V5_160_CONV_ALL, gemm_v5_kernel, (160, 4, true, EPI_F_ALL, false, true))       \
  T(GK_V5_128_CONV, gemm_v5_kernel, (128, 4, true, 0, false, false))                  \
  T(GK_V5_128_CONV_VEC, gemm_v5_kernel, (128, 4, true, 0, false, true))               \
  T(GK_V5_128_CONV_ALL, gemm_v5_kernel, (128, 4, true, EPI_F_ALL, false, true))       \
  T(GK_V5_160, gemm_v5_kernel, (160, 4, false, 0, false, false))                      \
  T(GK_V5_160_QKV, gemm_v5_kernel, (160, 4, false, EPI_F_QKV, false, false))          \
  T(GK_V5_160_ALL, gemm_v5_kernel, (160, 4, false, EPI_F_ALL, false, true))           \
  T(GK_V5_128, gemm_v5_kernel, (128, 4, false, 0, false, false))                      \
  T(GK_V5_128_QKV, gemm_v5_kernel, (128, 4, false, EPI_F_QKV, false, false))          \
  T(GK_V5_128_ALL, gemm_v5_kernel, (128, 4, false, EPI_F_ALL, false, true))

#define MX_GEMM_V4_FORMS(T)                                                 \
  T(GK_V4_GEGLU_LN, gemm_v4_kernel, (false, 0, true, true))                 \
  T(GK_V4_QKV_LN, gemm_v4_kernel, (false, EPI_F_QKV, false, true))          \
  T(GK_V4_LN, gemm_v4_kernel, (false, 0, false, true))                      \
  T(GK_V4_GEGLU_ACT, gemm_v4_kernel, (false, EPI_F_ACT, true))              \
  T(GK_V4_GEGLU, gemm_v4_kernel, (false, 0, true))                          \
  T(GK_V4, gemm_v4_kernel, (false, 0, false))                               \
  T(GK_V4_QKV, gemm_v4_kernel, (false, EPI_F_QKV, false))                   \
  T(GK_V4_TANH, gemm_v4_kernel, (false, EPI_F_TANH, false))                 \
  T(GK_V4_VEC_ALL, gemm_v4_kernel, (true, EPI_F_ALL, false))                \
  T(GK_V4_VEC, gemm_v4_kernel, (true, 0, false))

#define MX_GEMM_SMALL_M_FORMS(T)                                            \
  T(GK_SM_STREAM_F32, gemm_small_m_stream_kernel, (true))                   \
  T(GK_SM_STREAM, gemm_small_m_stream_kernel, (false))                      \
  T(GK_SM16_F32, gemm_small_m_kernel, (true, 16))                           \
  T(GK_SM16, gemm_small_m_kernel, (false, 16))                              \
  T(GK_SM4_F32, gemm_small_m_kernel, (true, 4))                             \
  T(GK_SM4, gemm_small_m_kernel, (false, 4))

#define MX_GEMM_CONV_SMALL_FORMS(P)                                         \
  P(GK_CONV_SMALL_N, conv3x3_small_n_kernel)                                \
  P(GK_CONV_SMALL_CIN, conv3x3_small_cin_kernel)

#define MX_FORM_UNPAREN(...) __VA_ARGS__
#define MX_FORM_TARGS(...) "<" #__VA_ARGS__ ">"
#define MX_FORM_NAME_T(id, k, targs) #k MX_FORM_TARGS targs,
#define MX_FORM_NAME_P(id, k) #k,

namespace mx {
enum GemmKernelId {
#define MX_FORM_ID_T(id, k, targs) id,
#define MX_FORM_ID_P(id, k) id,
  MX_GEMM_GENERIC_FORMS(MX_FORM_ID_T) MX_GEMM_V2_FORMS(MX_FORM_ID_T) MX_GEMM_V5_FORMS(MX_FORM_ID_T) MX_GEMM_V4_FORMS(MX_FORM_ID_T)
  MX_GEMM_SMALL_M_FORMS(MX_FORM_ID_T) MX_GEMM_CONV_SMALL_FORMS(MX_FORM_ID_P)
#undef MX_FORM_ID_T
#undef MX_FORM_ID_P
  GK_COUNT
};
}
```

### sduss_amd/csrc/gemm_v5_body.h

```cpp
#pragma once
#include "common.h"
#include "../../include/mxdenoise.h"
#include "gemm_args.h"
#include "gemm_dma_loader.h"

namespace mx {

constexpr int NSTAGE5 = 3;

#if defined(MX_EXP) && MX_EXP == 8
static __device__ unsigned long long g_v5_stamps[1024 * 2 * 4];
#define MX5_STAMP(slot) do { if (lane == 0 && (wave == 0 || wave == 7) && blockIdx.x < 1024) \
    g_v5_stamps[(blockIdx.x * 2 + (wave == 7)) * 4 + (slot)] = __builtin_amdgcn_s_memrealtime(); } while (0)
#else
#define MX5_STAMP(slot) do {} while (0)
#endif

template <int BN, int MI, bool CONV, int FEAT, bool GEGLU, bool VEC, bool WT = false>
__device__ __forceinline__ void gemm_v5_tile(const GemmArgs& pk, int tm, const int tn, bf16_t* const smem) {
  constexpr int BM5 = 64 * MI;
  constexpr int NI = BN / 32;
  constexpr int LOADS = DmaTile<BN, MI>::LOADS;

  const int tid = threadIdx.x;
  const int lane = tid & 63;
  const int wave = __builtin_amdgcn_readfirstlane(tid >> 6);
  const int wm = wave >> 1;
  const int wn = wave & 1;
  const bool group_b = wave >= 4;
  MX5_STAMP(0);
  GemmArgs p = pk;
  gemm_select_seg(p, pk, tm);
  const int nk = p.K / DMA_BK;
  constexpr bool SPLIT_K = false;
  constexpr int k_first = 0;
#include "gemm_dma_loader.inc"

  const int fr = lane & 15;
  const int fq = lane >> 4;
  unsigned wrd[2], xrd[2];
#pragma unroll
  for (int ks = 0; ks < 2; ++ks) {
    const int wrow = wn * (BN / 2) + fr, xrow = wm * 16 * MI + fr;
    wrd[ks] = (unsigned)(((BM5 * DMA_BK) + wrow * DMA_BK + swz(wrow, ks * 4 + fq) * 8) * 2);
    xrd[ks] = (unsigned)((xrow * DMA_BK + swz(xrow, ks * 4 + fq) * 8) * 2);
  }

  setup_tile();
  issue_group(0); advance_cursor();
  issue_group(1); advance_cursor();
  wait_vmcnt<LOADS>();

  f32x4 acc[NI][MI];
#pragma unroll
  for (int i = 0; i < NI; ++i)
#pragma unroll
    for (int j = 0; j < MI; ++j) acc[i][j] = f32x4{0.f, 0.f, 0.f, 0.f};
  float ln_rstd[MI];
#pragma unroll
  for (int j = 0; j < MI; ++j) ln_rstd[j] = 1.0f;
  if constexpr (!CONV) {
    if (p.ln_stats != nullptr) gemm_ln_init<NI, MI>(p, acc, tm * BM5 + wm * 16 * MI, tn * BN + wn * (BN / 2), fr, fq, ln_rstd);
  }
  MX_BAR();
  if (group_b) MX_BAR();
  MX5_STAMP(1);

  int stage = 0;
  for (int kt = 0; kt < nk; ++kt) {
    const char* sb = reinterpret_cast<const char*>(smem) + stage * (STAGE_ELEMS * 2);
    bf16x8 wf[2][NI], xf[2][MI];
#pragma unroll
    for (int ks = 0; ks < 2; ++ks) {
#pragma unroll
      for (int i = 0; i < NI; ++i) wf[ks][i] = *reinterpret_cast<const bf16x8*>(sb + wrd[ks] + i * (16 * DMA_BK * 2));
#pragma unroll
      for (int j = 0; j < MI; ++j) xf[ks][j] = *reinterpret_cast<const bf16x8*>(sb + xrd[ks] + j * (16 * DMA_BK * 2));
    }
    const int st2 = stage >= 1 ? stage - 1 : NSTAGE5 - 1;
    issue_group(st2);
    advance_cursor();
    wait_vmcnt<LOADS>();
    asm volatile("s_waitcnt lgkmcnt(0)" ::: "memory");
    __builtin_amdgcn_sched_barrier(0);
    MX_BAR();
    __builtin_amdgcn_s_setprio(1);
#pragma unroll
    for (int ks = 0; ks < 2; ++ks)
#pragma unroll
      for (int i = 0; i < NI; ++i)
#pragma unroll
        for (int j = 0; j < MI; ++j) acc[i][j] = __builtin_amdgcn_mfma_f32_16x16x32_bf16(wf[ks][i], xf[ks][j], acc[i][j], 0, 0, 0);
    __builtin_amdgcn_s_setprio(0);
    MX_BAR();
    stage = stage == NSTAGE5 - 1 ? 0 : stage + 1;
  }
  MX5_STAMP(2);
  if (!group_b) MX_BAR();

  const int m0 = tm * BM5, n0 = tn * BN;
  static_assert(!GEGLU || (NI % 4 == 0 && !CONV), "the gated epilogue pairs whole 32-feature halves");
  gemm_epilogue_regs<NI, MI, GEGLU, VEC, true, true, FEAT, true, false, WT>(p, acc, m0 + wm * 16 * MI, n0 + wn * (BN / 2), fr, fq, ln_rstd);
  if constexpr (!GEGLU && FEAT == 0 && MI == 4) {
    if (pk.gn_part != nullptr) gemm_gn_partials<NI, MI>(p, acc, m0 + wm * 16 * MI, n0 + wn * (BN / 2), fr, fq);
  }
  MX5_STAMP(3);
  wait_vmcnt<0>();
  if constexpr (!CONV && !GEGLU && BM5 == 256) {
    if (pk.ln_final_out != nullptr) gemm_ln_finalize(p, tm, pk.N / BN, reinterpret_cast<volatile int*>(smem));
  }
}


}
```

### sduss_amd/csrc/unet_sdxl.cpp

```cpp
#include <hip/hip_runtime.h>

#include <algorithm>
#include <cstring>
#include <functional>
#include <string>
#include <unordered_map>
#include <vector>

#include "../../include/mxdenoise.h"
#include "common.h"
#include <map>

#include "graph_cache.h"
#include "pp_exchange.h"
#include "patch_cache.h"

namespace mx {
int launch_prep_latent(hipStream_t s, const void* in, int dtype, void* out, int B, int Cin, int HW, int CP);
int launch_nhwc_to_nchw(hipStream_t s, const void* in, void* out, int dtype, int B, int C, int HW, int ld);
int launch_time_embed(hipStream_t s, const float* timesteps, const void* text_embeds, const float* time_ids,
                      void* tsin, void* addin, int B, int d0, int text_dim, int da);
int launch_concat(hipStream_t s, const void* a, const void* b, void* out, long M, int C1, int C2);
size_t gn_workspace_exact(int B, int H, int W, int C, int patch);
int launch_sq_diff_partial(hipStream_t s, const void* a, const void* b, long elems_per_sample, int B, double* partial, const int* slot = nullptr);
// ... 197 lines not shown
      mx_attn_problem q; std::memset(&q, 0, sizeof(q));
      const long r0 = (long)pc_ask_first[b] * pp;
      q.q = qc + r0 * C; q.o = oc + r0 * C;
      q.k = kbase + (k_sample_stride >= 0 ? (long)b * k_sample_stride : (pc_samp[b].row0 >> (2 * level)) * (long)ldk);
      q.vt = vtbase + vt_sample_off[b]; q.ldvt = ldvt_s[b];
      q.vt_batch_stride = vt_bstride_fixed > 0 ? vt_bstride_fixed : (int64_t)C * ldvt_s[b];
      q.B = 1; q.Lq = na * pp; q.Lk = Lk_s[b];
      pr.push_back(q);
    }
    for (size_t i = 0; i < pr.size(); i += MX_MAX_SEGS) {
      const int n = (int)std::min<size_t>(MX_MAX_SEGS, pr.size() - i);
      if (mx_attention_prescaled_grouped(stream, pr.data() + i, n, C, ldk, C, heads)) return fail(std::string("attention: ") + mx_last_error());
    }
    return true;
  }

  unsigned blocks_run = 0;
  std::vector<float> h_timesteps;
  bool lookup = false;
  const char* stage = nullptr; void* stage_out = nullptr; size_t stage_bytes = 0; bool stage_hit = false;
  std::string err;
  int pp_rank = 0, pp_world = 1, Htot = 0;
  bool is_pp() const { return pp_world > 1; }
  float* temb_all = nullptr; int temb_total = 0; int temb_off = 0;
  struct KV { bf16_t* k; bf16_t* vt; int ldk; int ldvt; long vt_bstride; int next; int dim; };
  std::vector<KV> kv;
  mx_unet::CtxEntry* ctx_e = nullptr;
  bool ctx_hit = false;

  bool fail(const std::string& m) { if (err.empty()) err = m; return false; }

  const void* w(const std::string& name, size_t expect_bytes) {
    if (dry && !lookup) return (const void*)(uintptr_t)0x1000;
    auto it = u->table.find(name);
    if (it == u->table.end()) { fail("missing weight '" + name + "'"); return nullptr; }
    if (it->second.second != expect_bytes) {
      fail("weight '" + name + "' has " + std::to_string(it->second.second) + " bytes, expected " + std::to_string(expect_bytes));
      return nullptr;
    }
    return u->blob + it->second.first;
  }
  const bf16_t* wb(const std::string& name, size_t elems) { return (const bf16_t*)w(name, elems * 2); }
  const float* wf(const std::string& name, size_t elems) { return (const float*)w(name, elems * 4); }

  template <typename T> T* alloc(size_t elems) {
    T* p = (T*)ar.alloc(elems * sizeof(T));
    if (!p) fail("workspace too small");
    return p;
  }

  bool ok() const { return err.empty(); }

  bool all_gather(const void* send, void* recv, size_t bytes_per_rank, bool keep_stale_own = false) {
    if (!ok()) return false;
    if (const char* e = px.all_gather(stream, dry, send, recv, bytes_per_rank, keep_stale_own)) return fail(e);
    return true;
  }
  bf16_t* alloc_padded(int h, int wd, int C) { return alloc<bf16_t>((size_t)B * (h + 2) * wd * C); }
  static bf16_t* interior(bf16_t* P, int wd, int C) { return P + (size_t)wd * C; }
  bool copy_to_padded(const bf16_t* x, bf16_t* P, int h, int wd, int C) {
    if (!ok()) return false;
    if (dry) return true;
    const size_t img = (size_t)h * wd * C * 2, pimg = (size_t)(h + 2) * wd * C * 2;
    if (hipMemcpy2DAsync(interior(P, wd, C), pimg, x, img, img, B, hipMemcpyDeviceToDevice, stream) != hipSuccess) return fail("copy_to_padded failed");
    return true;
  }
  bool halo_exchange(bf16_t* P, int h, int wd, int C) {
    if (!ok()) return false;
    const size_t m = ar.mark();
    const size_t row = (size_t)wd * C * 2, pimg = (size_t)(h + 2) * row;
    char* send = (char*)ar.alloc(2 * B * row);
    char* recv = (char*)ar.alloc((size_t)pp_world * 2 * B * row);
    if (!send || !recv) return fail("workspace too small");
    if (dry) { if (!all_gather(send, recv, 2 * B * row)) return false; }
    if (!dry) {
      char* Pc = (char*)P;
      bool e = hipMemcpy2DAsync(send, row, Pc + row, pimg, row, B, hipMemcpyDeviceToDevice, stream) != hipSuccess;
      e |= hipMemcpy2DAsync(send + B * row, row, Pc + (size_t)h * row, pimg, row, B, hipMemcpyDeviceToDevice, stream) != hipSuccess;
      if (e) return fail("halo pack failed");
      if (!all_gather(send, recv, 2 * B * row)) return false;
      if (pp_rank > 0) e |= hipMemcpy2DAsync(Pc, pimg, recv + ((size_t)(pp_rank - 1) * 2 + 1) * B * row, row, row, B, hipMemcpyDeviceToDevice, stream) != hipSuccess;
      else e |= hipMemset2DAsync(Pc, pimg, 0, row, B, stream) != hipSuccess;
      if (pp_rank < pp_world - 1) e |= hipMemcpy2DAsync(Pc + (size_t)(h + 1) * row, pimg, recv + ((size_t)(pp_rank + 1) * 2) * B * row, row, row, B, hipMemcpyDeviceToDevice, stream) != hipSuccess;
      else e |= hipMemset2DAsync(Pc + (size_t)(h + 1) * row, pimg, 0, row, B, stream) != hipSuccess;
      if (e) return fail("halo unpack failed");
    }
    ar.release(m);
    return true;
  }
  bool groupnorm_pp(const bf16_t* x, bf16_t* y, long y_img, const std::string& prefix, int h, int wd, int C, float eps, bool silu, int level,
                    const bf16_t* x2 = nullptr, int C1 = 0) {
    if (!ok()) return false;
    const size_t m = ar.mark();
    const int G = u->cfg.norm_num_groups;
    void* ws = ar.alloc(mx::gn_workspace_exact(B, h, wd, C, 0));
    double* sums = (double*)ar.alloc((size_t)B * G * 2 * sizeof(double));
    double* all = (double*)ar.alloc((size_t)pp_world * B * G * 2 * sizeof(double));
    if (!ws || !sums || !all) return fail("workspace too small");
    const float* g = wf(prefix + ".weight", C); const float* b = wf(prefix + ".bias", C);
    if (ok() && dry) all_gather(sums, all, (size_t)B * G * 2 * sizeof(double));
    if (ok() && !dry) {
      if (mx::launch_gn_pp_partial(stream, x, C1, x2, B, h, wd, C, G, ws, sums)) return fail(std::string("groupnorm: ") + mx_last_error());
      const bool corrected = px.mode == MX_PP_STALE && px.corrected_gn;
      if (!all_gather(sums, all, (size_t)B * G * 2 * sizeof(double), corrected)) return false;
      if (mx::launch_gn_pp_finish(stream, x, C1, x2, y, y_img, g, b, all, pp_world, B, h, wd, C, G, Htot >> level, eps, silu ? 1 : 0, ws,
                                  corrected ? sums : nullptr, pp_rank))
        return fail(std::string("groupnorm: ") + mx_last_error());
    }
    ar.release(m);
    return ok();
  }

  bool gemm(mx_gemm_desc& d, bool conv) {
    if (!ok()) return false;
    if (quiet()) return true;
    const int rc = conv ? mx_conv3x3(stream, &d) : mx_gemm(stream, &d);
    if (rc) return fail(std::string("gemm/conv: ") + mx_last_error());
    return true;
  }
  struct RowStats { float* buf = nullptr; int slabs = 0; float* fin = nullptr; unsigned* cnt = nullptr; };
  unsigned* ln_cnt = nullptr;
  static constexpr int kLnCnt = 4096;
  unsigned* tail_sync = nullptr;
  long tail_rows = 0;
  bool gemm_with_stats(mx_gemm_desc& d, RowStats& st, bool finalise = false) {
    if (!ok()) return false;
    const int slabs = mx_gemm_stats_slabs(&d);
    if (finalise) {
      if (slabs <= 0 || !mx_gemm_ln_final_supported(&d) || (d.M + 255) / 256 > kLnCnt) return fail("finalised row statistics: the producing launch cannot write them");
      d.ln_final_out = st.fin; d.ln_final_cnt = st.cnt; d.ln_eps = u->cfg.layer_norm_eps;
    }
    if (slabs > 0) { d.stats_out = st.buf; st.slabs = slabs; return gemm(d, false); }
    st.slabs = 1;
    if (!gemm(d, false)) return false;
    if (!quiet() && mx_row_stats(stream, d.c, d.ldc, st.buf, d.M, d.N)) return fail(std::string("row_stats: ") + mx_last_error());
    return true;
  }
  void use_ln(mx_gemm_desc& d, const RowStats& st, const std::string& csname, bool final = false) {
    if (final) d.ln_final = st.fin; else { d.ln_stats = st.buf; d.ln_slabs = st.slabs; }
    d.ln_colsum = wf(csname, d.N); d.ln_eps = u->cfg.layer_norm_eps;
  }
  bool linear(const bf16_t* a, int lda, const std::string& wname, const std::string& bname, void* c, int ldc, int M, int N,
              int K, const void* residual = nullptr, int ldr = 0, int flags = 0, float out_scale = 0.f, const bf16_t* a2 = nullptr, int lda2 = 0,
              const RowStats* ln = nullptr, RowStats* stats_out = nullptr, bool ln_final = false, bool finalise = false) {
    mx_gemm_desc d; std::memset(&d, 0, sizeof(d));
    d.out_scale = out_scale;
    if (a2) { d.a2 = a2; d.lda2 = lda2; d.k_split = lda; }
    d.a = a; d.lda = lda; d.w = wb(wname, (size_t)N * K); d.bias = bname.empty() ? nullptr : wf(bname, N);
    d.c = c; d.ldc = ldc; d.M = M; d.N = N; d.K = K; d.residual = residual; d.ldr = ldr; d.flags = flags;
    if (ln) use_ln(d, *ln, wname.substr(0, wname.size() - 6) + "colsum", ln_final);
    if (stats_out) return gemm_with_stats(d, *stats_out, finalise);
    return gemm(d, false);
  }
  int conv_cin_valid = 0;
  bool conv(const bf16_t* x, int Hin, int Win, int Cin, const std::string& prefix, bf16_t* out, int Cout, int stride, int up,
            int corner_patch, const float* rowbias = nullptr, int ldrb = 0, const void* residual = nullptr, int vhalo = 0, float* gn_part = nullptr,
            bool* gn_done = nullptr) {
    mx_gemm_desc d; std::memset(&d, 0, sizeof(d));
    d.vhalo = vhalo;
    const int Hv = Hin << up, Wv = Win << up;
    d.a = x; d.w = wb(prefix + ".weight", (size_t)Cout * 9 * Cin); d.bias = wf(prefix + ".bias", Cout);
    d.c = out; d.ldc = Cout; d.B = gB[0]; d.Hin = Hin; d.Win = Win; d.Cin = Cin;
    d.Hout = (Hv + stride - 1) / stride; d.Wout = (Wv + stride - 1) / stride; d.stride = stride; d.up = up;
    d.corner_patch = corner_patch;
    d.M = gB[0] * d.Hout * d.Wout; d.N = Cout; d.K = 9 * Cin;
    d.rowbias = rowbias; d.ldrb = ldrb; d.rows_per_batch = d.Hout * d.Wout;
    d.residual = residual; d.ldr = Cout;
    mx_gemm_seg sg[MX_MAX_SEGS];
    if (ng > 1) {
      std::memset(sg, 0, sizeof(sg));
      long in0 = 0, out0 = 0;
      for (int g = 0; g < ng; ++g) {
        mx_gemm_seg& q = sg[g];
        q.B = gB[g]; q.Hin = ch[g]; q.Win = cw[g];
        q.Hout = ((ch[g] << up) + stride - 1) / stride; q.Wout = ((cw[g] << up) + stride - 1) / stride;
        q.M = gB[g] * q.Hout * q.Wout; q.rows_per_batch = q.Hout * q.Wout;
        q.a = x + in0 * Cin; q.c = out + out0 * Cout;
        q.residual = residual ? (const bf16_t*)residual + out0 * Cout : nullptr;
        q.rowbias = rowbias ? rowbias + (long)gb0[g] * ldrb : nullptr;
        in0 += (long)gB[g] * ch[g] * cw[g]; out0 += q.M;
      }
      d.segs = sg; d.n_segs = ng;
    }
    if (gn_part && gn_done && ng == 1 && mx_gemm_gn_partials_supported(&d, 1)) { d.gn_part_out = gn_part; *gn_done = true; }
    d.cin_valid = conv_cin_valid;
    return gemm(d, true);
  }
  bool groupnorm(const bf16_t* x, bf16_t* y, const std::string& prefix, int h, int wd, int C, float eps, bool silu, int patch,
                 const bf16_t* x2 = nullptr, int C1 = 0) {
    if (!ok()) return false;
    const size_t m = ar.mark();
    mx_gn_problem pr[MX_MAX_SEGS];
    long r0 = 0;
    for (int k = 0; k < ng; ++k) {
      pr[k].x = x + r0 * (x2 ? C1 : C); pr[k].x2 = x2 ? x2 + r0 * (C - C1) : nullptr; pr[k].y = y + r0 * C;
      pr[k].B = gB[k]; pr[k].H = ch[k]; pr[k].W = cw[k];
      r0 += (long)gB[k] * ch[k] * cw[k];
    }
    const size_t need = ng > 1 ? mx_groupnorm_nhwc_grouped_workspace_bytes(pr, ng, C) : mx::gn_workspace_exact(gB[0], h, wd, C, patch);
    void* ws = ar.alloc(need);
    if (!ws) return fail("workspace too small");
    const float* g = wf(prefix + ".weight", C); const float* b = wf(prefix + ".bias", C);
    if (ok() && !quiet()) {
      if (mx_groupnorm_nhwc_grouped(stream, pr, ng, x2 ? C1 : C, g, b, C, u->cfg.norm_num_groups, eps, silu ? 1 : 0, patch, ws))
        fail(std::string("groupnorm: ") + mx_last_error());
    }
    ar.release(m);
    return ok();
  }
  bool groupnorm_from_partials(const bf16_t* x, bf16_t* y, const std::string& prefix, int h, int wd, int C, float eps, bool silu, const float* part,
                               const float* add_bias, const float* add_rowbias, int ldrb) {
    if (!ok()) return false;
    const size_t m = ar.mark();
    void* ws = ar.alloc(mx::gn_workspace_exact(gB[0], h, wd, C, 0));
    if (!ws) return fail("workspace too small");
    const float* g = wf(prefix + ".weight", C); const float* b = wf(prefix + ".bias", C);
    if (ok() && !quiet()) {
      if (mx_groupnorm_nhwc_from_partials(stream, x, y, g, b, gB[0], h, wd, C, u->cfg.norm_num_groups, eps, silu ? 1 : 0, part, 64, add_bias, add_rowbias, ldrb, ws))
        fail(std::string("groupnorm: ") + mx_last_error());
    }
    ar.release(m);
    return ok();
  }
  bool attention(const bf16_t* q, int ldq, const bf16_t* k, int ldk, const bf16_t* vt, int ldvt, long vt_bstride, bf16_t* o,
                 int ldo, int heads, int Lq, int Lk) {
    if (!ok()) return false;
    if (quiet()) return true;
    if (mx_attention_prescaled(stream, q, ldq, k, ldk, vt, ldvt, vt_bstride, o, ldo, B, heads, Lq, Lk))
      return fail(std::string("attention: ") + mx_last_error());
    return true;
  }
  bool attention_grouped(const mx_attn_problem* pr, int ldq, int ldk, int ldo, int heads) {
    if (!ok()) return false;
    if (quiet()) return true;
    if (mx_attention_prescaled_grouped(stream, pr, ng, ldq, ldk, ldo, heads)) return fail(std::string("attention: ") + mx_last_error());
    return true;
  }
  void dump(const std::string& name, const bf16_t* t, size_t elems) {
    if (!stage || quiet() || !ok() || stage_hit) return;
    if (name != stage) return;
    if (elems * 2 > stage_bytes) { fail("stage buffer too small for '" + name + "'"); return; }
    if (hipMemcpyAsync(stage_out, t, elems * 2, hipMemcpyDeviceToDevice, stream) != hipSuccess) fail("stage copy failed");
    stage_hit = true;
  }

  int level_patch(int level) const { return gn_patch > 0 ? std::max(gn_patch >> level, 1) : 0; }

  bf16_t* resnet(const std::string& p, const bf16_t* x, int h, int wd, int Cin, int Cout, int level, const bf16_t* x2 = nullptr, int C2 = 0) {
    const int M = (int)rows();
    const int C1 = Cin - C2;
    bf16_t* out = alloc<bf16_t>((size_t)M * Cout);
    const size_t m = ar.mark();
    const int patch = level_patch(level);
    if (is_pp()) {
      bf16_t* n1p = alloc_padded(h, wd, Cin);
      groupnorm_pp(x, interior(n1p, wd, Cin), (long)(h + 2) * wd * Cin, p + ".norm1", h, wd, Cin, u->cfg.norm_eps, true, level, x2, C1);
      halo_exchange(n1p, h, wd, Cin);
      bf16_t* h1 = alloc<bf16_t>((size_t)M * Cout);
      conv(n1p, h, wd, Cin, p + ".conv1", h1, Cout, 1, 0, 0, temb_all ? temb_all + temb_off : nullptr, temb_total, nullptr, 1);
      temb_off += Cout;
      bf16_t* n2p = alloc_padded(h, wd, Cout);
      groupnorm_pp(h1, interior(n2p, wd, Cout), (long)(h + 2) * wd * Cout, p + ".norm2", h, wd, Cout, u->cfg.norm_eps, true, level);
      halo_exchange(n2p, h, wd, Cout);
      const bf16_t* sc = x;
      if (Cin != Cout) {
        bf16_t* s2 = alloc<bf16_t>((size_t)M * Cout);
        if (x2) linear(x, C1, p + ".conv_shortcut.weight", p + ".conv_shortcut.bias", s2, Cout, M, Cout, Cin, nullptr, 0, 0, 0.f, x2, C2);
        else linear(x, Cin, p + ".conv_shortcut.weight", p + ".conv_shortcut.bias", s2, Cout, M, Cout, Cin);
        sc = s2;
      }
      conv(n2p, h, wd, Cout, p + ".conv2", out, Cout, 1, 0, 0, nullptr, 0, sc, 1);
      ar.release(m);
      dump(p, out, (size_t)M * Cout);
      return out;
    }
    if (pc) {
      bf16_t* n1 = alloc<bf16_t>((size_t)M * Cin);
      groupnorm(x, n1, p + ".norm1", h, wd, Cin, u->cfg.norm_eps, true, patch, x2, C1);
      bf16_t* h1 = alloc<bf16_t>((size_t)M * Cout);
      pc_conv(n1, h, wd, Cin, p + ".conv1", h1, Cout, 1, 0, patch, level, temb_all ? temb_all + temb_off : nullptr, temb_total, nullptr);
      temb_off += Cout;
      bf16_t* n2 = alloc<bf16_t>((size_t)M * Cout);
      groupnorm(h1, n2, p + ".norm2", h, wd, Cout, u->cfg.norm_eps, true, patch);
      const bf16_t* sc = x;
      if (Cin != Cout) {
        bf16_t* s2 = alloc<bf16_t>((size_t)M * Cout);
        if (x2) linear(x, C1, p + ".conv_shortcut.weight", p + ".conv_shortcut.bias", s2, Cout, M, Cout, Cin, nullptr, 0, 0, 0.f, x2, C2);
        else linear(x, Cin, p + ".conv_shortcut.weight", p + ".conv_shortcut.bias", s2, Cout, M, Cout, Cin);
        sc = s2;
      }
      pc_conv(n2, h, wd, Cout, p + ".conv2", out, Cout, 1, 0, patch, level, nullptr, 0, sc);
      ar.release(m);
      dump(p, out, (size_t)M * Cout);
      return out;
    }
    bf16_t* n1 = alloc<bf16_t>((size_t)M * Cin);
    groupnorm(x, n1, p + ".norm1", h, wd, Cin, u->cfg.norm_eps, true, patch, x2, C1);
    bf16_t* h1 = alloc<bf16_t>((size_t)M * Cout);
    float* gpart = nullptr;
    bool gdone = false;
    if (ng == 1 && patch == 0 && M % 64 == 0 && (h * wd) % 64 == 0) gpart = (float*)ar.alloc((size_t)(M / 64) * Cout * 2 * sizeof(float));
    conv(n1, h, wd, Cin, p + ".conv1", h1, Cout, 1, 0, patch, temb_all ? temb_all + temb_off : nullptr, temb_total, nullptr, 0, gpart, &gdone);
    temb_off += Cout;
    bf16_t* n2 = alloc<bf16_t>((size_t)M * Cout);
    if (gdone) groupnorm_from_partials(h1, n2, p + ".norm2", h, wd, Cout, u->cfg.norm_eps, true, gpart, wf(p + ".conv1.bias", Cout),
                                       temb_all ? temb_all + (temb_off - Cout) : nullptr, temb_total);
    else groupnorm(h1, n2, p + ".norm2", h, wd, Cout, u->cfg.norm_eps, true, patch);
    const bf16_t* sc = x;
    if (Cin != Cout) {
      bf16_t* s2 = alloc<bf16_t>((size_t)M * Cout);
      if (x2) linear(x, C1, p + ".conv_shortcut.weight", p + ".conv_shortcut.bias", s2, Cout, M, Cout, Cin, nullptr, 0, 0, 0.f, x2, C2);
      else linear(x, Cin, p + ".conv_shortcut.weight", p + ".conv_shortcut.bias", s2, Cout, M, Cout, Cin);
      sc = s2;
    }
    conv(n2, h, wd, Cout, p + ".conv2", out, Cout, 1, 0, patch, nullptr, 0, sc);
    ar.release(m);
    dump(p, out, (size_t)M * Cout);
    return out;
  }

  KV* kv_for(int dim) {
    for (auto& k : kv) if (k.dim == dim) return &k;
    return nullptr;
  }

  bf16_t* transformer(const std::string& p, const bf16_t* x, int h, int wd, int C, int heads, int layers, int level) {
    const int L = h * wd;
    const int M = (int)rows();
    const int ctx = u->cfg.cross_attention_dim;
    int gL[MX_MAX_SEGS], gldvt[MX_MAX_SEGS]; long gr0[MX_MAX_SEGS], gvt0[MX_MAX_SEGS], vt_elems = 0;
    for (int g = 0; g < ng; ++g) {
      gL[g] = ch[g] * cw[g]; gldvt[g] = MX_VT_LD(gL[g]); gr0[g] = row0(g); gvt0[g] = vt_elems;
      vt_elems += (long)gB[g] * C * gldvt[g];
    }
    bf16_t* out = alloc<bf16_t>((size_t)M * C);
    const size_t m0 = ar.mark();
    bf16_t* n = alloc<bf16_t>((size_t)M * C);
    if (is_pp()) groupnorm_pp(x, n, (long)L * C, p + ".norm", h, wd, C, u->cfg.transformer_norm_eps, false, level);
    else groupnorm(x, n, p + ".norm", h, wd, C, u->cfg.transformer_norm_eps, false, level_patch(level));
    bf16_t* y = alloc<bf16_t>((size_t)M * C);
    RowStats st;
    st.buf = (float*)ar.alloc((size_t)M * MX_STATS_PITCH(C / 64) * 2 * sizeof(float));
    if (!st.buf) fail("workspace too small");
    bf16_t* ln = n;
    const int ldvt = MX_VT_LD(L);
    bf16_t* qk = alloc<bf16_t>((size_t)M * 2 * C);
    bf16_t* vt = alloc<bf16_t>((size_t)vt_elems);
    bf16_t* ao = alloc<bf16_t>((size_t)M * C);
    bf16_t* q2 = alloc<bf16_t>((size_t)M * C);
    bf16_t* ff = alloc<bf16_t>((size_t)M * 4 * C);
    mx_gemm_seg qsegs[MX_MAX_SEGS];
    auto qkv_desc = [&](const std::string& b, const bf16_t* a) {
      mx_gemm_desc d; std::memset(&d, 0, sizeof(d));
      d.a = a; d.lda = C; d.w = wb(b + ".attn1.to_qkv.weight", (size_t)3 * C * C); d.bias = wf(b + ".attn1.to_qkv.bias", 3 * C);
      d.c = qk; d.ldc = 2 * C;
      d.M = M; d.N = 3 * C; d.K = C; d.flags = MX_EPI_QKV; d.seg = C; d.period = 3; d.vt = vt; d.ldvt = ldvt;
      d.rows_per_batch = L; d.out_scale = MX_ATTN_QSCALE(0.125f);
      if (ng > 1) {
        std::memset(qsegs, 0, sizeof(qsegs));
        for (int g = 0; g < ng; ++g) {
          qsegs[g].a = a + gr0[g] * C; qsegs[g].c = qk + gr0[g] * 2 * C; qsegs[g].vt = vt + gvt0[g];
          qsegs[g].M = gB[g] * gL[g]; qsegs[g].rows_per_batch = gL[g]; qsegs[g].ldvt = gldvt[g];
        }
        d.segs = qsegs; d.n_segs = ng;
      }
      return d;
    };
    auto use_ln_grouped = [&](mx_gemm_desc& d, const RowStats& st_) {
      if (d.n_segs > 0) for (int g = 0; g < ng; ++g) qsegs[g].ln_stats = st_.buf + gr0[g] * MX_STATS_PITCH(st_.slabs) * 2;
    };
    auto lin_desc = [&](const bf16_t* a, void* c, int ldc, int N, int flags, float out_scale) {
      mx_gemm_desc d; std::memset(&d, 0, sizeof(d));
      d.a = a; d.lda = C; d.w = a; d.c = c; d.ldc = ldc; d.M = M; d.N = N; d.K = C; d.flags = flags; d.out_scale = out_scale;
      return d;
    };
    bool pass1, pass2, pass3;
    {
      mx_gemm_desc d1 = qkv_desc(p + ".transformer_blocks.0", y);
      mx_gemm_desc d2 = lin_desc(y, q2, C, C, 0, MX_ATTN_QSCALE(0.125f));
      mx_gemm_desc d3 = lin_desc(y, ff, 4 * C, 8 * C, MX_EPI_GEGLU, 0.f);
      pass1 = mx_gemm_ln_prefers_pass(&d1) != 0; pass2 = mx_gemm_ln_prefers_pass(&d2) != 0; pass3 = mx_gemm_ln_prefers_pass(&d3) != 0;
    }
    const bool pass3_shape = pass3;
    bool fin1 = false, fin3 = false;
    if (!is_pp() && ln_cnt != nullptr && (M + 255) / 256 <= kLnCnt) {
      auto can_finalise = [&](int K, bool residual) {
        mx_gemm_desc d = lin_desc(y, y, C, C, 0, 0.f);
        d.K = K; d.lda = K; if (residual) { d.residual = y; d.ldr = C; }
        return mx_gemm_ln_final_supported(&d) != 0;
      };
      fin1 = ng == 1 && pass1 && can_finalise(C, false) && (layers == 1 || can_finalise(4 * C, true));
      fin3 = pass3 && can_finalise(C, true);
      if (pc) fin3 = false;
      if (fin1 || fin3 || (pc && pass3_shape)) { st.fin = (float*)ar.alloc((size_t)M * 2 * sizeof(float)); st.cnt = ln_cnt; if (!st.fin) fail("workspace too small"); }
    }
    const bool pc_fin3 = pc && pass3_shape && st.fin != nullptr;
    if (fin1) pass1 = false;
    if (fin3) pass3 = false;
    bool tail = mx_attn_tail_preferred() != 0 && !pc && !is_pp() && ng == 1 && !pass2 && tail_sync != nullptr && M <= tail_rows && L % 256 == 0;
    if (getenv("MX_ATTN_TAIL_DEBUG") && !quiet())
      fprintf(stderr, "[mx attn_tail] transformer %s: tail %d (pc %d pp %d ng %d pass2 %d sync %p M %d rows %ld L %d)\n", p.c_str(), (int)tail, (int)pc, (int)is_pp(), ng,
              (int)pass2, (void*)tail_sync, M, tail_rows, L);
    bf16_t* ao2 = nullptr;
    RowStats stA;
    if (tail) {
      ao2 = alloc<bf16_t>((size_t)M * C);
      stA.buf = (float*)ar.alloc((size_t)M * MX_STATS_PITCH(C / 64) * 2 * sizeof(float));
      if (!stA.buf) fail("workspace too small");
    }
    bf16_t* pqc = nullptr; bf16_t* paoc = nullptr; bf16_t* ptc = nullptr;
    if (pc) { pqc = alloc<bf16_t>((size_t)M * C); paoc = alloc<bf16_t>((size_t)M * C); ptc = alloc<bf16_t>((size_t)M * C); }
    auto normalise = [&]() {
      if (ok() && !quiet() && mx_layernorm(stream, y, ln, nullptr, nullptr, M, C, u->cfg.layer_norm_eps)) fail(std::string("layernorm: ") + mx_last_error());
    };
    linear(n, C, p + ".proj_in.weight", p + ".proj_in.bias", y, C, M, C, C, nullptr, 0, 0, 0.f, nullptr, 0, nullptr, pass1 ? nullptr : &st, false, fin1);
    bf16_t* k_send = nullptr; bf16_t* k_all = nullptr; bf16_t* vt_all = nullptr;
    if (is_pp()) {
      if (L % 64 != 0) fail("patch-parallel: local tokens per image must be a multiple of 64 at every attention level");
      k_send = alloc<bf16_t>((size_t)M * C);
      k_all = alloc<bf16_t>((size_t)pp_world * M * C);
      vt_all = alloc<bf16_t>((size_t)pp_world * B * C * ldvt);
    }
    KV* kvp = kv_for(C);
    if (!kvp && ok()) fail("no cross-attention K/V buffer for width " + std::to_string(C));
    for (int k = 0; k < layers && ok(); ++k) {
      const std::string b = p + ".transformer_blocks." + std::to_string(k);
      if (pc) {
        const int pp2 = (pc_p0 >> level) * (pc_p0 >> level);
        const int Mc = pc_count() * pp2;
        std::vector<long> vt_off(B); std::vector<int> ldvt_s(B), Lk_s(B);
        for (int g = 0; g < ng; ++g) for (int i = 0; i < gB[g]; ++i) { const int bb = gb0[g] + i; vt_off[bb] = gvt0[g] + (long)i * C * gldvt[g]; ldvt_s[bb] = gldvt[g]; Lk_s[bb] = gL[g]; }
        auto self_attention_all = [&]() {
          if (ng > 1) {
            mx_attn_problem pr[MX_MAX_SEGS];
            for (int g = 0; g < ng; ++g) {
              pr[g].q = qk + gr0[g] * 2 * C; pr[g].k = qk + gr0[g] * 2 * C + C; pr[g].vt = vt + gvt0[g]; pr[g].o = ao + gr0[g] * C;
              pr[g].vt_batch_stride = (int64_t)C * gldvt[g]; pr[g].B = gB[g]; pr[g].Lq = gL[g]; pr[g].Lk = gL[g]; pr[g].ldvt = gldvt[g];
            }
            attention_grouped(pr, 2 * C, 2 * C, C, heads);
          } else attention(qk, 2 * C, qk + C, 2 * C, vt, ldvt, (long)C * ldvt, ao, C, heads, L, L);
        };
        {
          if (pass1) normalise();
          mx_gemm_desc d = qkv_desc(b, pass1 ? ln : y);
          if (!pass1) { use_ln(d, st, b + ".attn1.to_qkv.colsum", fin1); if (!fin1) use_ln_grouped(d, st); } else wf(b + ".attn1.to_qkv.colsum", 3 * C);
          gemm(d, false);
        }
        char* reg1 = pc_region(level, C);
        if (!pc_partial) {
          self_attention_all();
          linear(ao, C, b + ".attn1.to_out.0.weight", b + ".attn1.to_out.0.bias", ptc, C, M, C, C);
          pc_store(ptc, reg1, level, C);
        } else {
          pc_gather_rows(qk, 2 * C, C, pqc, level);
          pc_attention(pqc, qk + C, 2 * C, -1, vt, vt_off.data(), ldvt_s.data(), 0, paoc, C, heads, level, Lk_s.data());
          linear(paoc, C, b + ".attn1.to_out.0.weight", b + ".attn1.to_out.0.bias", ptc, C, Mc, C, C);
          pc_scatter_rows(ptc, C, reg1, level);
        }
        const bool stats2 = !pc_partial && !pass2;
        if (stats2) { pc_load_stats(y, reg1, level, C, y, st.buf, nullptr); st.slabs = 1; }
        else pc_load(y, reg1, level, C, nullptr, 0, y);
        char* reg2 = pc_region(level, C);
        const int li = ok() ? kvp->next++ : 0;
        if (!pc_partial) {
          if (!stats2) normalise();
          linear(stats2 ? y : ln, C, b + ".attn2.to_q.weight", b + ".attn2.to_q.bias", q2, C, M, C, C, nullptr, 0, 0, MX_ATTN_QSCALE(0.125f), nullptr, 0, stats2 ? &st : nullptr);
          if (ok()) {
            if (ng > 1) {
              mx_attn_problem pr[MX_MAX_SEGS];
              for (int g = 0; g < ng; ++g) {
                pr[g].q = q2 + gr0[g] * C; pr[g].k = kvp->k + (size_t)li * C + (size_t)gb0[g] * ctx_len * kvp->ldk;
                pr[g].vt = kvp->vt + (size_t)li * C * kvp->ldvt + (size_t)gb0[g] * kvp->vt_bstride; pr[g].o = ao + gr0[g] * C;
                pr[g].vt_batch_stride = kvp->vt_bstride; pr[g].B = gB[g]; pr[g].Lq = gL[g]; pr[g].Lk = ctx_len; pr[g].ldvt = kvp->ldvt;
              }
              attention_grouped(pr, C, kvp->ldk, C, heads);
            } else attention(q2, C, kvp->k + (size_t)li * C, kvp->ldk, kvp->vt + (size_t)li * C * kvp->ldvt, kvp->ldvt, kvp->vt_bstride, ao, C, heads, L, ctx_len);
          }
          linear(ao, C, b + ".attn2.to_out.0.weight", b + ".attn2.to_out.0.bias", ptc, C, M, C, C);
          pc_store(ptc, reg2, level, C);
        } else {
          pc_gather_rows(y, C, C, paoc, level);
          if (ok() && !quiet() && mx_layernorm(stream, paoc, pqc, nullptr, nullptr, Mc, C, u->cfg.layer_norm_eps)) fail(std::string("layernorm: ") + mx_last_error());
          linear(pqc, C, b + ".attn2.to_q.weight", b + ".attn2.to_q.bias", q2, C, Mc, C, C, nullptr, 0, 0, MX_ATTN_QSCALE(0.125f));
          if (ok()) {
            std::vector<long> cvt_off(B); std::vector<int> cld(B, kvp->ldvt), clk(B, ctx_len);
            for (int bb = 0; bb < B; ++bb) cvt_off[bb] = (long)bb * kvp->vt_bstride;
            pc_attention(q2, kvp->k + (size_t)li * C, kvp->ldk, (long)ctx_len * kvp->ldk, kvp->vt + (size_t)li * C * kvp->ldvt, cvt_off.data(), cld.data(),
                         kvp->vt_bstride, paoc, C, heads, level, clk.data());
          }
          linear(paoc, C, b + ".attn2.to_out.0.weight", b + ".attn2.to_out.0.bias", ptc, C, Mc, C, C);
          pc_scatter_rows(ptc, C, reg2, level);
        }
        if (pc_fin3) pc_load_stats(y, reg2, level, C, y, nullptr, st.fin);
        else if (!pass3) { pc_load_stats(y, reg2, level, C, y, st.buf, nullptr); st.slabs = 1; }
        else pc_load(y, reg2, level, C, nullptr, 0, y);
        if (pass3 && !pc_fin3) normalise();
        {
          const bool folded = pc_fin3 || !pass3;
          linear(folded ? y : ln, C, b + ".ff.net.0.proj.weight", b + ".ff.net.0.proj.bias", ff, 4 * C, M, 8 * C, C, nullptr, 0, MX_EPI_GEGLU, 0.f, nullptr, 0,
                 folded ? &st : nullptr, nullptr, pc_fin3);
        }
        linear(ff, 4 * C, b + ".ff.net.2.weight", b + ".ff.net.2.bias", y, C, M, C, 4 * C, y, C, 0, 0.f, nullptr, 0, nullptr,
               (k + 1 < layers && !pass1) ? &st : nullptr, false, fin1 && k + 1 < layers);
        continue;
      }
      {
        if (pass1) normalise();
        mx_gemm_desc d = qkv_desc(b, pass1 ? ln : y);
        if (!pass1) { use_ln(d, st, b + ".attn1.to_qkv.colsum", fin1); if (!fin1) use_ln_grouped(d, st); } else wf(b + ".attn1.to_qkv.colsum", 3 * C);
        gemm(d, false);
      }
      if (is_pp()) {
        if (ok() && !dry && hipMemcpy2DAsync(k_send, (size_t)C * 2, qk + C, (size_t)2 * C * 2, (size_t)C * 2, M, hipMemcpyDeviceToDevice, stream) != hipSuccess)
          fail("patch-parallel: K pack failed");
        all_gather(k_send, k_all, (size_t)M * C * 2);
        all_gather(vt, vt_all, (size_t)B * C * ldvt * 2);
        if (ok() && !dry &&
            mx_attention_prescaled_chunked(stream, qk, 2 * C, k_all, C, vt_all, ldvt, (int64_t)C * ldvt, ao, C, B, heads, L, pp_world * L, L,
                                           (int64_t)L * C, (int64_t)M * C, (int64_t)B * C * ldvt))
          fail(std::string("attention: ") + mx_last_error());
      } else if (ng > 1) {
        mx_attn_problem pr[MX_MAX_SEGS];
        for (int g = 0; g < ng; ++g) {
          pr[g].q = qk + gr0[g] * 2 * C; pr[g].k = qk + gr0[g] * 2 * C + C; pr[g].vt = vt + gvt0[g]; pr[g].o = ao + gr0[g] * C;
          pr[g].vt_batch_stride = (int64_t)C * gldvt[g]; pr[g].B = gB[g]; pr[g].Lq = gL[g]; pr[g].Lk = gL[g]; pr[g].ldvt = gldvt[g];
        }
        attention_grouped(pr, 2 * C, 2 * C, C, heads);
      } else {
        attention(qk, 2 * C, qk + C, 2 * C, vt, ldvt, (long)C * ldvt, ao, C, heads, L, L);
      }
      bool chained = false;
      if (tail && ok()) {
        auto lin_d = [&](const bf16_t* a_, const std::string& stem, void* c_, const void* res) {
          mx_gemm_desc d; std::memset(&d, 0, sizeof(d));
          d.a = a_; d.lda = C; d.w = wb(stem + ".weight", (size_t)C * C); d.bias = wf(stem + ".bias", C); d.c = c_; d.ldc = C; d.M = M; d.N = C; d.K = C;
          d.residual = res; d.ldr = res ? C : 0;
          return d;
        };
        mx_attn_tail_desc td; std::memset(&td, 0, sizeof(td));
        td.out1 = lin_d(ao, b + ".attn1.to_out.0", y, y);
        td.out1.stats_out = stA.buf;
        const int slabs = mx_gemm_stats_slabs(&td.out1);
        td.to_q = lin_d(y, b + ".attn2.to_q", q2, nullptr);
        td.to_q.out_scale = MX_ATTN_QSCALE(0.125f);
        td.to_q.ln_stats = stA.buf; td.to_q.ln_slabs = slabs; td.to_q.ln_colsum = wf(b + ".attn2.to_q.colsum", C); td.to_q.ln_eps = u->cfg.layer_norm_eps;
        td.out2 = lin_d(ao2, b + ".attn2.to_out.0", y, y);
        if (!pass3) {
          td.out2.stats_out = st.buf;
          if (fin3) { td.out2.ln_final_out = st.fin; td.out2.ln_final_cnt = st.cnt; td.out2.ln_eps = u->cfg.layer_norm_eps; }
        }
        const int li = kvp->next;
        td.k = kvp->k + (size_t)li * C; td.ldk = kvp->ldk; td.vt = kvp->vt + (size_t)li * C * kvp->ldvt; td.ldvt = kvp->ldvt; td.vt_batch_stride = kvp->vt_bstride;
        td.B = B; td.heads = heads; td.L = L; td.ctx_len = ctx_len; td.sync = tail_sync;
        if (ok() && slabs > 0 && (quiet() || mx_attn_tail_supported(&td) != 0)) {
          chained = true;
          ++kvp->next;
          if (!pass3) st.slabs = slabs;
          if (!quiet() && mx_attn_tail(stream, &td)) fail(std::string("attn_tail: ") + mx_last_error());
        } else {
          if (getenv("MX_ATTN_TAIL_DEBUG")) fprintf(stderr, "[mx attn_tail] layer %s: slabs %d -> separate launches\n", b.c_str(), slabs);
          tail = false;
        }
      }
      if (!chained) {
        linear(ao, C, b + ".attn1.to_out.0.weight", b + ".attn1.to_out.0.bias", y, C, M, C, C, y, C, 0, 0.f, nullptr, 0, nullptr, pass2 ? nullptr : &st);
        if (pass2) normalise();
        linear(pass2 ? ln : y, C, b + ".attn2.to_q.weight", b + ".attn2.to_q.bias", q2, C, M, C, C, nullptr, 0, 0, MX_ATTN_QSCALE(0.125f), nullptr, 0,
               pass2 ? nullptr : &st);
        if (ok()) {
          const int li = kvp->next++;
          if (ng > 1) {
            mx_attn_problem pr[MX_MAX_SEGS];
            for (int g = 0; g < ng; ++g) {
              pr[g].q = q2 + gr0[g] * C; pr[g].k = kvp->k + (size_t)li * C + (size_t)gb0[g] * ctx_len * kvp->ldk;
              pr[g].vt = kvp->vt + (size_t)li * C * kvp->ldvt + (size_t)gb0[g] * kvp->vt_bstride; pr[g].o = ao + gr0[g] * C;
              pr[g].vt_batch_stride = kvp->vt_bstride; pr[g].B = gB[g]; pr[g].Lq = gL[g]; pr[g].Lk = ctx_len; pr[g].ldvt = kvp->ldvt;
            }
            attention_grouped(pr, C, kvp->ldk, C, heads);
          } else
          attention(q2, C, kvp->k + (size_t)li * C, kvp->ldk, kvp->vt + (size_t)li * C * kvp->ldvt, kvp->ldvt, kvp->vt_bstride,
                    ao, C, heads, L, ctx_len);
        }
        linear(ao, C, b + ".attn2.to_out.0.weight", b + ".attn2.to_out.0.bias", y, C, M, C, C, y, C, 0, 0.f, nullptr, 0, nullptr, pass3 ? nullptr : &st, false, fin3);
      }
      if (pass3) normalise();
      linear(pass3 ? ln : y, C, b + ".ff.net.0.proj.weight", b + ".ff.net.0.proj.bias", ff, 4 * C, M, 8 * C, C, nullptr, 0, MX_EPI_GEGLU, 0.f, nullptr, 0,
             pass3 ? nullptr : &st, nullptr, fin3);
      linear(ff, 4 * C, b + ".ff.net.2.weight", b + ".ff.net.2.bias", y, C, M, C, 4 * C, y, C, 0, 0.f, nullptr, 0, nullptr,
             (k + 1 < layers && !pass1) ? &st : nullptr, false, fin1 && k + 1 < layers);
    }
    linear(y, C, p + ".proj_out.weight", p + ".proj_out.bias", out, C, M, C, C, x, C);
    ar.release(m0);
    (void)ctx;
    dump(p, out, (size_t)M * C);
    return out;
  }

  bool run(const void* latents, int io_dtype, const float* timesteps, const void* ehs, const void* text_embeds,
           const float* time_ids, void* outp) {
    const mx_unet_config& c = u->cfg;
    const int nlev = c.n_levels;
    const int C0 = c.block_out_channels[0];
    const int T = 4 * C0;
    const int text_dim = c.projection_class_embeddings_input_dim - 6 * c.addition_time_embed_dim;
    const int addw = c.projection_class_embeddings_input_dim;
    const int ctx = c.cross_attention_dim;

    ln_cnt = (unsigned*)ar.alloc((size_t)kLnCnt * sizeof(unsigned));
    if (ok() && !quiet() && ln_cnt && hipMemsetAsync(ln_cnt, 0, (size_t)kLnCnt * sizeof(unsigned), stream) != hipSuccess) fail("ln tickets: memset failed");
    tail_rows = 0;
    for (int g = 0; g < ng; ++g) tail_rows += (long)gB[g] * gH[g] * gW[g];
    if (tail_rows > 0 && tail_rows < 2147483647L) {
      const size_t nb = mx_attn_tail_sync_bytes((int)tail_rows);
      tail_sync = (unsigned*)ar.alloc(nb);
      if (ok() && !quiet() && tail_sync && hipMemsetAsync(tail_sync, 0, nb, stream) != hipSuccess) fail("attention tail tickets: memset failed");
    }
    bf16_t* tsin = alloc<bf16_t>((size_t)B * C0);
    bf16_t* addin = alloc<bf16_t>((size_t)B * addw);
    if (ok() && !dry &&
        mx::launch_time_embed(stream, timesteps, text_embeds, time_ids, tsin, addin, B, C0, text_dim, c.addition_time_embed_dim))
      fail(mx_last_error());
    bf16_t* t1 = alloc<bf16_t>((size_t)B * T);
    bf16_t* t2 = alloc<bf16_t>((size_t)B * T);
    bf16_t* a1 = alloc<bf16_t>((size_t)B * T);
    bf16_t* semb = alloc<bf16_t>((size_t)B * T);
    linear(tsin, C0, "time_embedding.linear_1.weight", "time_embedding.linear_1.bias", t1, T, B, T, C0, nullptr, 0, MX_EPI_SILU);
    linear(t1, T, "time_embedding.linear_2.weight", "time_embedding.linear_2.bias", t2, T, B, T, T);
    linear(addin, addw, "add_embedding.linear_1.weight", "add_embedding.linear_1.bias", a1, T, B, T, addw, nullptr, 0, MX_EPI_SILU);
    linear(a1, T, "add_embedding.linear_2.weight", "add_embedding.linear_2.bias", semb, T, B, T, T, t2, T, MX_EPI_SILU);
    temb_total = 0;
    {
      int prev = C0;
      for (int i = 0; i < nlev; ++i) { for (int j = 0; j < c.layers_per_block; ++j) temb_total += c.block_out_channels[i]; prev = c.block_out_channels[i]; }
      (void)prev;
      temb_total += 2 * c.block_out_channels[nlev - 1];
      for (int i = 0; i < nlev; ++i) temb_total += (c.layers_per_block + 1) * c.block_out_channels[nlev - 1 - i];
    }
    temb_all = alloc<float>((size_t)B * temb_total);
    temb_off = 0;
    linear(semb, T, "temb_proj_all.weight", "temb_proj_all.bias", temb_all, temb_total, B, temb_total, T, nullptr, 0, MX_EPI_OUT_F32);

    kv.clear();
    {
      const std::vector<std::pair<int, int>> widths = kv_widths(c);
      const int ldvt = MX_VT_LD(ctx_len);
      size_t wi = 0;
      for (auto& wv : widths) {
        const int dim = wv.first, nl = wv.second;
        KV e; e.dim = dim; e.next = 0; e.ldk = nl * dim; e.ldvt = ldvt; e.vt_bstride = (long)nl * dim * ldvt;
        if (ctx_e && !dry) { e.k = ctx_e->k[wi]; e.vt = ctx_e->vt[wi]; }
        else { e.k = alloc<bf16_t>((size_t)B * ctx_len * nl * dim); e.vt = alloc<bf16_t>((size_t)B * nl * dim * ldvt); }
        ++wi;
        if (!(ctx_e && ctx_hit && !dry)) {
          mx_gemm_desc d; std::memset(&d, 0, sizeof(d));
          d.a = ehs; d.lda = ctx; d.w = wb("attn2_kv_all." + std::to_string(dim) + ".weight", (size_t)nl * 2 * dim * ctx);
          d.c = e.k; d.ldc = nl * dim; d.M = B * ctx_len; d.N = nl * 2 * dim; d.K = ctx; d.flags = MX_EPI_QKV; d.seg = dim; d.period = 2;
          d.vt = e.vt; d.ldvt = ldvt; d.rows_per_batch = ctx_len;
          gemm(d, false);
        }
        kv.push_back(e);
      }
    }

    int h = H, wd = W;
    for (int g = 0; g < ng; ++g) { ch[g] = gH[g]; cw[g] = gW[g]; }
    if (ng > 1 && (is_pp() || (bc && !pc))) fail("a mixed-resolution batch runs neither patch-parallel nor through the per-sample block cache");
    bf16_t* x0 = alloc<bf16_t>((size_t)rows() * kConvInPad);
    for (int g = 0; g < ng && ok() && !dry; ++g)
      if (mx::launch_prep_latent(stream, g_lat[g], io_dtype, x0 + row0(g) * kConvInPad, gB[g], c.in_channels, ch[g] * cw[g], kConvInPad)) fail(mx_last_error());
    bf16_t* x = alloc<bf16_t>((size_t)rows() * C0);
    if (is_pp()) {
      bf16_t* x0p = alloc_padded(h, wd, kConvInPad);
      copy_to_padded(x0, x0p, h, wd, kConvInPad);
      halo_exchange(x0p, h, wd, kConvInPad);
      conv(x0p, h, wd, kConvInPad, "conv_in", x, C0, 1, 0, 0, nullptr, 0, nullptr, 1);
    } else
    { conv_cin_valid = c.in_channels <= 8 ? 8 : 0; conv(x0, h, wd, kConvInPad, "conv_in", x, C0, 1, 0, 0); conv_cin_valid = 0; }
    dump("conv_in", x, (size_t)rows() * C0);

    struct Skip { bf16_t* t; int C; int h, wd; int level; };
    std::vector<Skip> skips;
    skips.push_back({x, C0, h, wd, 0});
    int lvl = 0;
    int Ccur = C0;
    auto down_block = [&](int i) {
      const int Cout = c.block_out_channels[i];
      for (int j = 0; j < c.layers_per_block && ok(); ++j) {
        const std::string rp = "down_blocks." + std::to_string(i) + ".resnets." + std::to_string(j);
        x = resnet(rp, x, h, wd, Ccur, Cout, i);
        Ccur = Cout;
        if (c.down_has_attn[i]) {
          const std::string ap = "down_blocks." + std::to_string(i) + ".attentions." + std::to_string(j);
          x = transformer(ap, x, h, wd, Cout, c.num_heads[i], c.transformer_layers[i], i);
        }
        skips.push_back({x, Cout, h, wd, i});
      }
      if (i != nlev - 1) {
        const std::string dp = "down_blocks." + std::to_string(i) + ".downsamplers.0";
        size_t drows = 0;
        for (int g = 0; g < ng; ++g) drows += (size_t)gB[g] * ((ch[g] + 1) / 2) * ((cw[g] + 1) / 2);
        bf16_t* d = alloc<bf16_t>(drows * Cout);
        if (is_pp()) {
          if (h % 2) fail("patch-parallel: local rows must stay even down to the last level");
          const size_t mk = ar.mark();
          bf16_t* xp = alloc_padded(h, wd, Cout);
          copy_to_padded(x, xp, h, wd, Cout);
          halo_exchange(xp, h, wd, Cout);
          conv(xp, h, wd, Cout, dp + ".conv", d, Cout, 2, 0, 0, nullptr, 0, nullptr, 1);
          ar.release(mk);
        } else if (pc)
        pc_conv(x, h, wd, Cout, dp + ".conv", d, Cout, 2, 0, level_patch(i), i, nullptr, 0, nullptr);
        else
        conv(x, h, wd, Cout, dp + ".conv", d, Cout, 2, 0, level_patch(i));
        h /= 2; wd /= 2;
        for (int g = 0; g < ng; ++g) { ch[g] = (ch[g] + 1) / 2; cw[g] = (cw[g] + 1) / 2; }
        x = d;
        lvl = i + 1;
        dump(dp, x, (size_t)rows() * Cout);
        skips.push_back({x, Cout, h, wd, i + 1});
      }
    };
    auto mid_block = [&]() {
      const int Cm = c.block_out_channels[nlev - 1];
      x = resnet("mid_block.resnets.0", x, h, wd, Cm, Cm, nlev - 1);
      x = transformer("mid_block.attentions.0", x, h, wd, Cm, c.num_heads[nlev - 1], c.transformer_layers[nlev - 1], nlev - 1);
      x = resnet("mid_block.resnets.1", x, h, wd, Cm, Cm, nlev - 1);
    };
    auto up_block = [&](int i) {
      const int level = nlev - 1 - i;
      const int Cout = c.block_out_channels[level];
      for (int j = 0; j < c.layers_per_block + 1 && ok(); ++j) {
        const Skip sk = skips.back(); skips.pop_back();
        const std::string rp = "up_blocks." + std::to_string(i) + ".resnets." + std::to_string(j);
        x = resnet(rp, x, h, wd, Ccur + sk.C, Cout, level, sk.t, sk.C);
        Ccur = Cout;
        if (c.down_has_attn[level]) {
          const std::string ap = "up_blocks." + std::to_string(i) + ".attentions." + std::to_string(j);
          x = transformer(ap, x, h, wd, Cout, c.num_heads[level], c.transformer_layers[level], level);
        }
      }
      if (i != nlev - 1) {
        const std::string upn = "up_blocks." + std::to_string(i) + ".upsamplers.0";
        bf16_t* d = alloc<bf16_t>((size_t)rows() * 4 * Cout);
        if (is_pp()) {
          const size_t mk = ar.mark();
          bf16_t* xp = alloc_padded(h, wd, Cout);
          copy_to_padded(x, xp, h, wd, Cout);
          halo_exchange(xp, h, wd, Cout);
          conv(xp, h, wd, Cout, upn + ".conv", d, Cout, 1, 1, 0, nullptr, 0, nullptr, 1);
          ar.release(mk);
        } else if (pc)
        pc_conv(x, h, wd, Cout, upn + ".conv", d, Cout, 1, 1, level_patch(level - 1), level, nullptr, 0, nullptr);
        else
        conv(x, h, wd, Cout, upn + ".conv", d, Cout, 1, 1, level_patch(level - 1));
        h *= 2; wd *= 2;
        for (int g = 0; g < ng; ++g) { ch[g] *= 2; cw[g] *= 2; }
        x = d;
        lvl = level - 1;
        dump(upn, x, (size_t)rows() * Cout);
      }
    };

    struct Ten { bf16_t* p; size_t per_sample; int C = 0; int level = 0; };
    auto run_block_pc = [&](int idx, bool is_up, const std::vector<Ten>& ins, const std::function<void()>& body) {
      const int nf = (int)ins.size();
// ... 693 lines not shown
```

### sduss_amd/lib.py

```python
from __future__ import annotations

import ctypes as C
import os
from typing import Optional

_HERE = os.path.dirname(os.path.abspath(__file__))
LIB_PATH = os.path.join(_HERE, "libmxdenoise.so")

MX_F32, MX_F16, MX_BF16 = 0, 1, 2
EPI_SILU, EPI_GEGLU, EPI_OUT_F32, EPI_QKV, EPI_GELU_TANH, EPI_RES_BCAST, EPI_RMSNORM, EPI_GELU, EPI_QUICK_GELU, EPI_GEGLU_TANH = 1, 2, 4, 8, 16, 32, 64, 128, 256, 512


class MxError(RuntimeError):
    """Raised for every non-zero status of the C ABI (the reference's launcher only printed
    cudaGetLastError and went on -- norm_silu_concat.cu:434-437; SURVEY.md section 8b asks to raise)."""


MAX_SEGS = 4


class GemmSeg(C.Structure):
    _fields_ = [
        ("a", C.c_void_p), ("a2", C.c_void_p), ("c", C.c_void_p), ("residual", C.c_void_p), ("vt", C.c_void_p), ("rowbias", C.c_void_p),
        ("gate", C.c_void_p), ("ln_stats", C.c_void_p), ("stats_out", C.c_void_p),
        ("M", C.c_int), ("rows_per_batch", C.c_int), ("ldvt", C.c_int),
        ("B", C.c_int), ("Hin", C.c_int), ("Win", C.c_int), ("Hout", C.c_int), ("Wout", C.c_int),
        ("a_batch_rows", C.c_int), ("a_row_off", C.c_int), ("c_batch_rows", C.c_int), ("c_row_off", C.c_int),
    ]


class GemmDesc(C.Structure):
    _fields_ = [
        ("a", C.c_void_p), ("w", C.c_void_p), ("c", C.c_void_p), ("bias", C.c_void_p), ("rowbias", C.c_void_p),
        ("residual", C.c_void_p), ("vt", C.c_void_p),
        ("M", C.c_int), ("N", C.c_int), ("K", C.c_int),
        ("lda", C.c_int), ("ldc", C.c_int), ("ldr", C.c_int), ("ldrb", C.c_int),
        ("rows_per_batch", C.c_int), ("flags", C.c_int),
        ("seg", C.c_int), ("period", C.c_int), ("ldvt", C.c_int),
        ("B", C.c_int), ("Hin", C.c_int), ("Win", C.c_int), ("Cin", C.c_int),
        ("Hout", C.c_int), ("Wout", C.c_int), ("stride", C.c_int), ("up", C.c_int), ("corner_patch", C.c_int),
        ("a_batch_rows", C.c_int), ("a_row_off", C.c_int), ("c_batch_rows", C.c_int), ("c_row_off", C.c_int),
        ("gate", C.c_void_p), ("ldg", C.c_int), ("out_scale", C.c_float), ("rms_wq", C.c_void_p), ("rms_wk", C.c_void_p), ("rms_eps", C.c_float), ("vhalo", C.c_int), ("a2", C.c_void_p), ("lda2", C.c_int), ("k_split", C.c_int),
        ("ln_stats", C.c_void_p), ("ln_colsum", C.c_void_p), ("ln_slabs", C.c_int), ("ln_eps", C.c_float), ("stats_out", C.c_void_p),
        ("segs", C.POINTER(GemmSeg)), ("n_segs", C.c_int), ("splitk", C.c_int),
        ("ln_final", C.c_void_p), ("ln_final_out", C.c_void_p), ("ln_final_cnt", C.c_void_p), ("gn_part_out", C.c_void_p), ("cin_valid", C.c_int),
    ]


class AttnTailDesc(C.Structure):
    _fields_ = [("out1", GemmDesc), ("to_q", GemmDesc), ("out2", GemmDesc),
                ("k", C.c_void_p), ("ldk", C.c_int), ("vt", C.c_void_p), ("ldvt", C.c_int), ("vt_batch_stride", C.c_int64),
                ("B", C.c_int), ("heads", C.c_int), ("L", C.c_int), ("ctx_len", C.c_int), ("sync", C.c_void_p)]


class AttnProblem(C.Structure):
    _fields_ = [("q", C.c_void_p), ("k", C.c_void_p), ("vt", C.c_void_p), ("o", C.c_void_p), ("vt_batch_stride", C.c_int64),
                ("B", C.c_int), ("Lq", C.c_int), ("Lk", C.c_int), ("ldvt", C.c_int)]


class GnProblem(C.Structure):
    _fields_ = [("x", C.c_void_p), ("x2", C.c_void_p), ("y", C.c_void_p), ("B", C.c_int), ("H", C.c_int), ("W", C.c_int)]


class UNetGroup(C.Structure):
    _fields_ = [("latents", C.c_void_p), ("out", C.c_void_p), ("batch", C.c_int), ("H", C.c_int), ("W", C.c_int)]


class UNetConfigC(C.Structure):
    _fields_ = [
        ("in_channels", C.c_int), ("out_channels", C.c_int), ("n_levels", C.c_int),
        ("block_out_channels", C.c_int * 4), ("layers_per_block", C.c_int),
        ("down_has_attn", C.c_int * 4), ("transformer_layers", C.c_int * 4), ("num_heads", C.c_int * 4),
        ("cross_attention_dim", C.c_int), ("addition_time_embed_dim", C.c_int),
        ("projection_class_embeddings_input_dim", C.c_int), ("norm_num_groups", C.c_int),
        ("norm_eps", C.c_float), ("transformer_norm_eps", C.c_float), ("layer_norm_eps", C.c_float),
    ]


class MMDiTConfigC(C.Structure):
    _fields_ = [
        ("patch_size", C.c_int), ("in_channels", C.c_int), ("out_channels", C.c_int), ("num_layers", C.c_int),
        ("num_attention_heads", C.c_int), ("joint_attention_dim", C.c_int), ("pooled_projection_dim", C.c_int),
        ("pos_embed_max_size", C.c_int), ("dual_attention", C.c_int * 64), ("norm_eps", C.c_float),
    ]


ALLGATHER_FN = C.CFUNCTYPE(C.c_int, C.c_void_p, C.c_void_p, C.c_void_p, C.c_void_p, C.c_size_t)


class PPComm(C.Structure):
    _fields_ = [("rank", C.c_int), ("world", C.c_int), ("all_gather", ALLGATHER_FN), ("ctx", C.c_void_p)]


ALLGATHER_INPLACE_FN = C.CFUNCTYPE(C.c_int, C.c_void_p, C.c_void_p, C.c_void_p, C.c_size_t)
PP_SYNC, PP_WARMUP, PP_STALE = 0, 1, 2


class PPStale(C.Structure):
    _fields_ = [("state", C.c_void_p), ("state_bytes", C.c_size_t), ("mode", C.c_int), ("corrected_gn", C.c_int),
                ("all_gather_async", ALLGATHER_INPLACE_FN)]


SKIP_PREDICT_FN = C.CFUNCTYPE(C.c_int, C.c_void_p, C.c_int, C.c_int, C.c_int, C.c_int, C.POINTER(C.c_float), C.POINTER(C.c_float),
                              C.POINTER(C.c_ubyte))
MSE_UNCACHED = 9.2233720368547758e18


SKIP_OBSERVE_FN = C.CFUNCTYPE(None, C.c_void_p, C.c_int, C.c_int, C.POINTER(C.c_float))


class BlockCacheC(C.Structure):
    _fields_ = [("predict", SKIP_PREDICT_FN), ("ctx", C.c_void_p), ("state", C.c_void_p), ("state_bytes", C.c_size_t),
                ("batch_key", C.c_uint64), ("cached_key", C.c_uint64), ("cached_valid", C.c_int), ("cached_batch", C.c_int),
                ("cached_h", C.c_int), ("cached_w", C.c_int), ("blocks_run", C.c_uint), ("blocks_run_hi", C.c_uint), ("observe", SKIP_OBSERVE_FN),
                ("slots", C.POINTER(C.c_int32)), ("slot_valid", C.POINTER(C.c_ubyte)), ("n_slots", C.c_int),
                ("max_h", C.c_int), ("max_w", C.c_int), ("patches_asked", C.c_ulonglong), ("patches_total", C.c_ulonglong)]


class CLIPConfigC(C.Structure):
    _fields_ = [("vocab_size", C.c_int), ("hidden_size", C.c_int), ("intermediate_size", C.c_int), ("num_hidden_layers", C.c_int),
                ("num_attention_heads", C.c_int), ("max_position_embeddings", C.c_int), ("hidden_act", C.c_int), ("projection_dim", C.c_int),
                ("eos_token_id", C.c_int), ("hidden_layer", C.c_int), ("layer_norm_eps", C.c_float)]


class T5ConfigC(C.Structure):
    _fields_ = [("vocab_size", C.c_int), ("d_model", C.c_int), ("d_ff", C.c_int), ("num_layers", C.c_int), ("num_heads", C.c_int),
                ("layer_norm_epsilon", C.c_float)]


class VAEConfigC(C.Structure):
    _fields_ = [("latent_channels", C.c_int), ("out_channels", C.c_int), ("n_levels", C.c_int), ("block_out_channels", C.c_int * 4),
                ("layers_per_block", C.c_int), ("norm_num_groups", C.c_int), ("norm_eps", C.c_float)]


class WeightEntry(C.Structure):
    _fields_ = [("name", C.c_char_p), ("offset", C.c_uint64), ("bytes", C.c_uint64)]


_vp, _i, _f, _d, _i64, _sz = C.c_void_p, C.c_int, C.c_float, C.c_double, C.c_int64, C.c_size_t
SYMBOLS = {
    "mx_last_error": (C.c_char_p, []),
    "mx_version": (_i, []),
    "mx_profile_enable": (_i, [_i]),
    "mx_profile_collect": (_i, [C.POINTER(C.c_double)]),
    "mx_profile_records": (_i, [C.POINTER(C.c_double), _i]),
    "mx_groupnorm_halo_workspace_bytes": (_sz, [_i, _i, _i]),
    "mx_groupnorm_halo": (_i, [_vp, _vp, _vp, _vp, _vp, _i, _i, _i, _i, _i, _d, _i, _vp, _i, _vp, _vp, _i, _vp]),
    "mx_halo_only": (_i, [_vp, _vp, _vp, _i, _i, _i, _i, _vp, _i]),
    "mx_gemm": (_i, [_vp, C.POINTER(GemmDesc)]),
    "mx_conv3x3": (_i, [_vp, C.POINTER(GemmDesc)]),
    "mx_gemm_stats_slabs": (_i, [C.POINTER(GemmDesc)]),
    "mx_gemm_ln_prefers_pass": (_i, [C.POINTER(GemmDesc)]),
    "mx_row_stats": (_i, [_vp, _vp, _i, _vp, _i, _i]),
    "mx_attention": (_i, [_vp, _vp, _i, _vp, _i, _vp, _i, _i64, _vp, _i, _i, _i, _i, _i, _f]),
    "mx_attention_prescaled": (_i, [_vp, _vp, _i, _vp, _i, _vp, _i, _i64, _vp, _i, _i, _i, _i, _i]),
    "mx_attention_cross_prescaled": (_i, [_vp, _vp, _i, _vp, _i, _vp, _i, _i64, _vp, _i, _i, _i, _i, _i]),
    "mx_attn_tail_sync_bytes": (_sz, [_i]),
    "mx_attn_tail_supported": (_i, [C.POINTER(AttnTailDesc)]),
    "mx_attn_tail_preferred": (_i, []),
    "mx_attn_tail": (_i, [_vp, C.POINTER(AttnTailDesc)]),
    "mx_attn_tail_status": (_i, [_vp, _vp, C.POINTER(C.c_uint)]),
    "mx_layernorm": (_i, [_vp, _vp, _vp, _vp, _vp, _i, _i, _f]),
    "mx_groupnorm_nhwc_workspace_bytes": (_sz, [_i, _i, _i, _i]),
    "mx_groupnorm_nhwc": (_i, [_vp, _vp, _vp, _vp, _vp, _i, _i, _i, _i, _i, _f, _i, _i, _vp]),
    "mx_groupnorm_nhwc_cat": (_i, [_vp, _vp, _i, _vp, _vp, _vp, _vp, _i, _i, _i, _i, _i, _f, _i, _i, _vp]),
    "mx_attention_prescaled_grouped": (_i, [_vp, C.POINTER(AttnProblem), _i, _i, _i, _i, _i]),
    "mx_groupnorm_nhwc_grouped_workspace_bytes": (_sz, [C.POINTER(GnProblem), _i, _i]),
    "mx_groupnorm_nhwc_grouped": (_i, [_vp, C.POINTER(GnProblem), _i, _i, _vp, _vp, _i, _i, _f, _i, _i, _vp]),
    "mx_unet_workspace_bytes_mixed": (_sz, [_vp, C.POINTER(UNetGroup), _i, _i]),
    "mx_unet_forward_mixed": (_i, [_vp, _vp, C.POINTER(UNetGroup), _i, _i, _vp, _vp, _vp, _vp, _i, _i, _vp, _sz]),
    "mx_unet_forward_mixed_trace": (_i, [_vp, _vp, C.POINTER(UNetGroup), _i, _i, _vp, _vp, _vp, _vp, _i, _i, _vp, _sz, C.c_char_p, _vp, _sz]),
    "mx_mmdit_workspace_bytes_mixed": (_sz, [_vp, C.POINTER(UNetGroup), _i, _i]),
    "mx_mmdit_forward_mixed": (_i, [_vp, _vp, C.POINTER(UNetGroup), _i, _i, _vp, _vp, _vp, _i, _vp, _sz]),
    "mx_unet_create": (_vp, [C.POINTER(UNetConfigC)]),
    "mx_unet_destroy": (None, [_vp]),
    "mx_unet_set_context_key": (_i, [_vp, C.c_uint64]),
    "mx_unet_context_stats": (_i, [_vp, C.POINTER(C.c_long), C.POINTER(C.c_long)]),
    "mx_unet_set_weights": (_i, [_vp, _vp, C.c_uint64, C.POINTER(WeightEntry), _i]),
    "mx_unet_workspace_bytes": (_sz, [_vp, _i, _i, _i, _i]),
    "mx_unet_validate": (_i, [_vp, _i, _i, _i, _i]),
    "mx_unet_forward": (_i, [_vp, _vp, _vp, _i, _vp, _vp, _vp, _vp, _vp, _i, _i, _i, _i, _i, _vp, _sz]),
    "mx_forest_predict": (_i, [_vp, _vp, _vp, _vp, _vp, _vp, _i, _vp, _i, _i, _vp]),
    "mx_mmdit_workspace_bytes_pp": (_sz, [_vp, _i, _i, _i, _i, _i]),
    "mx_mmdit_pp_state_bytes": (_sz, [_vp, _i, _i, _i, _i, _i]),
    "mx_mmdit_forward_pp": (_i, [_vp, _vp, _vp, _i, _vp, _vp, _vp, _vp, _i, _i, _i, _i, _vp, _vp, _vp, _sz]),
    "mx_mmdit_pp_comm_plan": (_i, [_vp, _i, _i, _i, _i, _vp]),
    "mx_unet_pp_state_bytes": (_sz, [_vp, _i, _i, _i, _i, _i]),
    "mx_unet_forward_pp_stale": (_i, [_vp, _vp, _vp, _i, _vp, _vp, _vp, _vp, _vp, _i, _i, _i, _i, _vp, _vp, _vp, _sz]),
    "mx_unet_block_cache_bytes": (_sz, [_vp, _i, _i, _i]),
    "mx_gemm_splitk": (_i, [_vp, _i]),
    "mx_gemm_release_scratch": (None, [_vp, _i]),
    "mx_gemm_ln_final_supported": (_i, [C.POINTER(GemmDesc)]),
    "mx_gemm_launches": (_i, [C.POINTER(GemmDesc)]),
    "mx_gemm_gn_partials_supported": (_i, [C.POINTER(GemmDesc), _i]),
    "mx_gemm_form": (_i, [C.POINTER(GemmDesc), _i]),
    "mx_gemm_kernel_name": (_i, [C.POINTER(GemmDesc), _i, _i, C.c_char_p, _i]),
    "mx_gemm_kernel_names": (_i, [C.c_char_p, _i]),
    "mx_attention_kernel_name": (_i, [_i, _i, _i, _i, _i, _i, _i, _i, _i, _i, C.c_char_p, _i]),
    "mx_attention_kernel_names": (_i, [C.c_char_p, _i]),
    "mx_groupnorm_nhwc_from_partials": (_i, [_vp, _vp, _vp, _vp, _vp, _i, _i, _i, _i, _i, C.c_float, _i, _vp, _i, _vp, _vp, _i, _vp]),
    "mx_unet_patch_cache_bytes": (_sz, [_vp, _i, _i, _i, _i]),
    "mx_mmdit_patch_cache_bytes": (_sz, [_vp, _i, _i, _i, _i, _i]),
    "mx_mmdit_workspace_bytes_cached_mixed": (_sz, [_vp, C.POINTER(UNetGroup), _i, _i, _i]),
    "mx_mmdit_forward_cached_mixed": (_i, [_vp, _vp, C.POINTER(UNetGroup), _i, _i, _vp, _vp, _vp, _i, _i, _vp, _sz, _vp]),
    "mx_unet_workspace_bytes_cached_mixed": (_sz, [_vp, C.POINTER(UNetGroup), _i, _i, _i]),
    "mx_unet_forward_cached_mixed": (_i, [_vp, _vp, C.POINTER(UNetGroup), _i, _i, _vp, _vp, _vp, _vp, _i, _i, _vp, _sz, _vp]),
    "mx_unet_forward_cached": (_i, [_vp, _vp, _vp, _i, _vp, _vp, _vp, _vp, _vp, _i, _i, _i, _i, _i, _vp, _sz, _vp]),
    "mx_mmdit_block_cache_bytes": (_sz, [_vp, _i, _i, _i, _i]),
    "mx_mmdit_forward_cached": (_i, [_vp, _vp, _vp, _i, _vp, _vp, _vp, _vp, _i, _i, _i, _i, _vp, _sz, _vp]),
    "mx_unet_forward_trace": (_i, [_vp, _vp, _vp, _i, _vp, _vp, _vp, _vp, _vp, _i, _i, _i, _i, _i, _vp, _sz,
                                   C.c_char_p, _vp, _sz]),
    "mx_unet_workspace_bytes_pp": (_sz, [_vp, _i, _i, _i, _i, _i]),
    "mx_unet_forward_pp": (_i, [_vp, _vp, _vp, _i, _vp, _vp, _vp, _vp, _vp, _i, _i, _i, _i, C.POINTER(PPComm), _vp, _sz]),
    "mx_unet_pp_comm_plan": (_i, [_vp, _i, _i, _i, _i, C.POINTER(PPComm)]),
    "mx_attention_prescaled_chunked": (_i, [_vp, _vp, _i, _vp, _i, _vp, _i, _i64, _vp, _i, _i, _i, _i, _i, _i, _i64, _i64, _i64]),
    "mx_layernorm_mod": (_i, [_vp, _vp, _vp, _vp, _vp, _vp, _vp, _vp, _i, _i, _i, _i, _f]),
    "mx_layernorm_mod_grouped": (_i, [_vp, _vp, _vp, _vp, _vp, _vp, _vp, _vp, _i, _i, _f, _vp, _vp, _i]),
    "mx_rmsnorm_heads": (_i, [_vp, _vp, _i, _i, _i, _i, _i, _i, _i, _vp, _vp, _f, _f]),
    "mx_mmdit_create": (_vp, [C.POINTER(MMDiTConfigC)]),
    "mx_mmdit_destroy": (None, [_vp]),
    "mx_mmdit_set_weights": (_i, [_vp, _vp, C.c_uint64, C.POINTER(WeightEntry), _i]),
    "mx_mmdit_workspace_bytes": (_sz, [_vp, _i, _i, _i, _i]),
    "mx_mmdit_validate": (_i, [_vp, _i, _i, _i, _i]),
    "mx_mmdit_forward": (_i, [_vp, _vp, _vp, _i, _vp, _vp, _vp, _vp, _i, _i, _i, _i, _vp, _sz]),
    "mx_mmdit_forward_trace": (_i, [_vp, _vp, _vp, _i, _vp, _vp, _vp, _vp, _i, _i, _i, _i, _vp, _sz, C.c_char_p, _vp, _sz]),
    "mx_vae_create": (_vp, [C.POINTER(VAEConfigC)]),
    "mx_vae_destroy": (None, [_vp]),
    "mx_vae_set_weights": (_i, [_vp, _vp, C.c_uint64, C.POINTER(WeightEntry), _i]),
    "mx_vae_workspace_bytes": (_sz, [_vp, _i, _i, _i]),
    "mx_vae_validate": (_i, [_vp, _i, _i, _i]),
    "mx_vae_decode": (_i, [_vp, _vp, _vp, _i, _vp, _i, _i, _i, _i, _vp, _sz]),
    "mx_clip_create": (_vp, [C.POINTER(CLIPConfigC)]),
    "mx_clip_destroy": (None, [_vp]),
    "mx_clip_set_weights": (_i, [_vp, _vp, C.c_uint64, C.POINTER(WeightEntry), _i]),
    "mx_clip_workspace_bytes": (_sz, [_vp, _i]),
    "mx_clip_validate": (_i, [_vp, _i]),
    "mx_clip_encode": (_i, [_vp, _vp, _vp, _vp, _vp, _i, _vp, _sz]),
    "mx_attention_prescaled_causal": (_i, [_vp, _vp, _i, _vp, _i, _vp, _i, _i64, _vp, _i, _i, _i, _i]),
    "mx_attention_prescaled_bias": (_i, [_vp, _vp, _i, _vp, _i, _vp, _i, _i64, _vp, _i, _i, _i, _i, _i, _vp, _i]),
    "mx_rmsnorm": (_i, [_vp, _vp, _vp, _vp, _i, _i, _f]),
    "mx_t5_create": (_vp, [C.POINTER(T5ConfigC)]),
    "mx_t5_destroy": (None, [_vp]),
    "mx_t5_set_weights": (_i, [_vp, _vp, C.c_uint64, C.POINTER(WeightEntry), _i]),
    "mx_t5_workspace_bytes": (_sz, [_vp, _i, _i]),
    "mx_t5_validate": (_i, [_vp, _i, _i]),
    "mx_t5_encode": (_i, [_vp, _vp, _vp, _vp, _i, _i, _vp, _sz]),
    "mx_cfg_flow_step": (_i, [_vp, _vp, _vp, _vp, _vp, _f, _i, _i64, _i]),
    "mx_euler_scale_input": (_i, [_vp, _vp, _vp, _vp, _i, _i, _i64, _i]),
    "mx_cfg_euler_step": (_i, [_vp, _vp, _vp, _vp, _vp, _f, _i, _i64, _i]),
}

_lib: Optional[C.CDLL] = None


def load() -> C.CDLL:
    global _lib
    if _lib is not None:
        return _lib
    path = os.environ.get("MXDENOISE_LIB", LIB_PATH)
    if not os.path.exists(path):
        raise MxError(f"{path} not found: build it with `python -c 'import __graft_entry__ as g; g.build()'` "
                      f"(or `make -C sduss_amd/csrc`). There is no CPU fallback for the product path.")
    lib = C.CDLL(path)
    for name, (res, args) in SYMBOLS.items():
        fn = getattr(lib, name)
        fn.restype = res
        fn.argtypes = args
    _lib = lib
    return lib


def check(status: int, what: str = "") -> None:
    if status != 0:
        msg = load().mx_last_error().decode("utf-8", "replace")
        raise MxError(f"{what}: {msg}" if what else msg)


def torch_dtype_code(dtype) -> int:
    import torch
    if dtype == torch.float32:
        return MX_F32
    if dtype == torch.float16:
        return MX_F16
    if dtype == torch.bfloat16:
        return MX_BF16
    raise MxError(f"unsupported dtype {dtype}")


def current_stream() -> int:
    import torch
    return torch.cuda.current_stream().cuda_stream


def _name_list(fn) -> list:
    n = fn(None, 0)
    buf = C.create_string_buffer(n + 1)
    fn(buf, n + 1)
    return buf.value.decode().split("\n")


def gemm_kernel_names() -> list:
    return _name_list(load().mx_gemm_kernel_names)


def attention_kernel_names() -> list:
    return _name_list(load().mx_attention_kernel_names)


def gemm_kernels_of(desc: "GemmDesc", conv: bool = False) -> list:
    lib, out, buf = load(), [], C.create_string_buffer(256)
    while True:
        n = lib.mx_gemm_kernel_name(C.byref(desc), int(conv), len(out), buf, len(buf))
        if n == 0:
            return out
        if n < 0:
            raise MxError("mx_gemm_kernel_name: no instantiation serves this descriptor")
        out.append(buf.value.decode())


def attention_kernel_of(B: int, H: int, Lq: int, Lk: int, ldo: int, prescaled: bool = True, causal: bool = False, bias: bool = False,
                        key_chunk: int = 0, force_cross: bool = False) -> str:
    buf = C.create_string_buffer(256)
    n = load().mx_attention_kernel_name(B, H, Lq, Lk, ldo, int(prescaled), int(causal), int(bias), key_chunk, int(force_cross), buf, len(buf))
    if n < 0:
        raise MxError("mx_attention_kernel_name: no instantiation serves this problem")
    return buf.value.decode()
```

### sduss_amd/weights.py

```python
from __future__ import annotations

import ctypes as C
import os
from typing import Dict, List, Optional, Tuple

import torch

from . import lib as _lib
from .config import UNetConfig, param_shapes, resnet_names, transformer_names

_ALIGN = 256
CONV_IN_PAD = 64


def synthetic_params(cfg: UNetConfig, device="cpu", seed: int = 10086) -> Dict[str, torch.Tensor]:
    g = torch.Generator(device=device).manual_seed(seed)
    out = {}
    for name, shape in sorted(param_shapes(cfg).items()):
        if name.endswith(".weight") and len(shape) >= 2:
            fan_in = 1
            for d in shape[1:]:
                fan_in *= d
            t = torch.randn(shape, generator=g, device=device) * fan_in ** -0.5
        elif name.endswith(".weight"):
            t = 1.0 + 0.1 * torch.randn(shape, generator=g, device=device)
        else:
            t = 0.05 * torch.randn(shape, generator=g, device=device)
        out[name] = t.to(torch.bfloat16)
    return out


def load_safetensors_dir(unet_dir: str) -> Tuple[UNetConfig, Dict[str, torch.Tensor]]:
    from safetensors.torch import load_file
    cfg = UNetConfig.from_hf_json(os.path.join(unet_dir, "config.json"))
    params: Dict[str, torch.Tensor] = {}
    files = sorted(f for f in os.listdir(unet_dir) if f.endswith(".safetensors"))
    if not files:
        raise FileNotFoundError(f"no .safetensors under {unet_dir}")
    pick = [f for f in files if "fp16" not in f] or files
    for f in pick:
        params.update(load_file(os.path.join(unet_dir, f)))
    return cfg, params


def load_mmdit_safetensors_dir(transformer_dir: str):
    from safetensors.torch import load_file
    from .config import MMDiTConfig
    cfg = MMDiTConfig.from_hf_json(os.path.join(transformer_dir, "config.json"))
    files = sorted(f for f in os.listdir(transformer_dir) if f.endswith(".safetensors"))
    if not files:
        raise FileNotFoundError(f"no .safetensors under {transformer_dir}")
    params: Dict[str, torch.Tensor] = {}
    for f in [f for f in files if "fp16" not in f] or files:
        params.update(load_file(os.path.join(transformer_dir, f)))
    return cfg, params


def _conv_pack(w: torch.Tensor, pad_in: int = 0) -> torch.Tensor:
    o, i, kh, kw = w.shape
    w = w.permute(0, 2, 3, 1)
    if pad_in and pad_in > i:
        w = torch.nn.functional.pad(w, (0, pad_in - i))
    return w.reshape(o, -1).contiguous()


def fold_layernorm(w: torch.Tensor, bias: Optional[torch.Tensor], gamma: torch.Tensor, beta: torch.Tensor):
    w32 = w.to(torch.float32)
    wf = (w32 * gamma.to(torch.float32)[None, :]).to(torch.bfloat16)
    colsum = wf.to(torch.float32).sum(dim=1)
    b = w32 @ beta.to(torch.float32)
    if bias is not None:
        b = b + bias.to(torch.float32)
    return wf.contiguous(), colsum.contiguous(), b.contiguous()


def params_as_held(cfg: UNetConfig, P: Dict[str, torch.Tensor]) -> Dict[str, torch.Tensor]:
    out = dict(P)
    for p, _dim, _h, layers in transformer_names(cfg):
        for k in range(layers):
            b = f"{p}.transformer_blocks.{k}"
            for names, nn in (((f"{b}.attn1.to_q.weight", f"{b}.attn1.to_k.weight", f"{b}.attn1.to_v.weight"), "norm1"),
                              ((f"{b}.attn2.to_q.weight",), "norm2"), ((f"{b}.ff.net.0.proj.weight",), "norm3")):
                g = P[f"{b}.{nn}.weight"].to(torch.float32)
                safe = torch.where(g.abs() > 1e-6, g, torch.ones_like(g))
                for n in names:
                    w = P[n].to(torch.float32)
                    held = (w * g[None, :]).to(torch.bfloat16).to(torch.float32) / safe[None, :]
                    out[n] = torch.where(g.abs()[None, :] > 1e-6, held, w).to(P[n].dtype)
    return out


def _geglu_interleave(t: torch.Tensor) -> torch.Tensor:
    half = t.shape[0] // 2
    h = t[:half].reshape(half // 32, 32, *t.shape[1:])
    g = t[half:].reshape(half // 32, 32, *t.shape[1:])
    return torch.cat([h, g], dim=1).reshape(t.shape).contiguous()


def pack(cfg: UNetConfig, P: Dict[str, torch.Tensor]) -> List[Tuple[str, torch.Tensor]]:
    missing = [k for k in param_shapes(cfg) if k not in P]
    if missing:
        raise KeyError(f"state dict lacks {len(missing)} tensors, e.g. {missing[:3]}")
    bf, f32 = torch.bfloat16, torch.float32
    out: List[Tuple[str, torch.Tensor]] = []

    def mat(name, t):
        out.append((name, t.to(bf).contiguous()))

    def vec(name, t):
        out.append((name, t.to(f32).contiguous()))

    mat("conv_in.weight", _conv_pack(P["conv_in.weight"], CONV_IN_PAD))
    vec("conv_in.bias", P["conv_in.bias"])
    for nm in ("time_embedding", "add_embedding"):
        for l in ("linear_1", "linear_2"):
            mat(f"{nm}.{l}.weight", P[f"{nm}.{l}.weight"])
            vec(f"{nm}.{l}.bias", P[f"{nm}.{l}.bias"])
    res = resnet_names(cfg)
    mat("temb_proj_all.weight", torch.cat([P[f"{p}.time_emb_proj.weight"] for p, _, _ in res], dim=0))
    vec("temb_proj_all.bias", torch.cat([P[f"{p}.time_emb_proj.bias"] for p, _, _ in res], dim=0))
    for p, cin, cout in res:
        vec(f"{p}.norm1.weight", P[f"{p}.norm1.weight"]); vec(f"{p}.norm1.bias", P[f"{p}.norm1.bias"])
        mat(f"{p}.conv1.weight", _conv_pack(P[f"{p}.conv1.weight"])); vec(f"{p}.conv1.bias", P[f"{p}.conv1.bias"])
        vec(f"{p}.norm2.weight", P[f"{p}.norm2.weight"]); vec(f"{p}.norm2.bias", P[f"{p}.norm2.bias"])
        mat(f"{p}.conv2.weight", _conv_pack(P[f"{p}.conv2.weight"])); vec(f"{p}.conv2.bias", P[f"{p}.conv2.bias"])
        if cin != cout:
            mat(f"{p}.conv_shortcut.weight", P[f"{p}.conv_shortcut.weight"].reshape(cout, cin))
            vec(f"{p}.conv_shortcut.bias", P[f"{p}.conv_shortcut.bias"])
    kv_by_dim: Dict[int, List[torch.Tensor]] = {}
    for p, dim, _h, layers in transformer_names(cfg):
        vec(f"{p}.norm.weight", P[f"{p}.norm.weight"]); vec(f"{p}.norm.bias", P[f"{p}.norm.bias"])
        for l in ("proj_in", "proj_out"):
            mat(f"{p}.{l}.weight", P[f"{p}.{l}.weight"].reshape(dim, dim)); vec(f"{p}.{l}.bias", P[f"{p}.{l}.bias"])
        for k in range(layers):
            b = f"{p}.transformer_blocks.{k}"
            def folded(name, w, bias, nn):
                wf, cs, bf_ = fold_layernorm(w, bias, P[f"{b}.{nn}.weight"], P[f"{b}.{nn}.bias"])
                mat(f"{name}.weight", wf); vec(f"{name}.colsum", cs); vec(f"{name}.bias", bf_)
            folded(f"{b}.attn1.to_qkv", torch.cat([P[f"{b}.attn1.to_q.weight"], P[f"{b}.attn1.to_k.weight"], P[f"{b}.attn1.to_v.weight"]], dim=0),
                   None, "norm1")
            mat(f"{b}.attn1.to_out.0.weight", P[f"{b}.attn1.to_out.0.weight"]); vec(f"{b}.attn1.to_out.0.bias", P[f"{b}.attn1.to_out.0.bias"])
            folded(f"{b}.attn2.to_q", P[f"{b}.attn2.to_q.weight"], None, "norm2")
            kv_by_dim.setdefault(dim, []).append(torch.cat([P[f"{b}.attn2.to_k.weight"], P[f"{b}.attn2.to_v.weight"]], dim=0))
            mat(f"{b}.attn2.to_out.0.weight", P[f"{b}.attn2.to_out.0.weight"]); vec(f"{b}.attn2.to_out.0.bias", P[f"{b}.attn2.to_out.0.bias"])
            folded(f"{b}.ff.net.0.proj", _geglu_interleave(P[f"{b}.ff.net.0.proj.weight"]), _geglu_interleave(P[f"{b}.ff.net.0.proj.bias"]), "norm3")
            mat(f"{b}.ff.net.2.weight", P[f"{b}.ff.net.2.weight"]); vec(f"{b}.ff.net.2.bias", P[f"{b}.ff.net.2.bias"])
    for dim, lst in kv_by_dim.items():
        mat(f"attn2_kv_all.{dim}.weight", torch.cat(lst, dim=0))
    n = len(cfg.block_out_channels)
    for i in range(n - 1):
        for p in (f"down_blocks.{i}.downsamplers.0.conv", f"up_blocks.{i}.upsamplers.0.conv"):
            mat(f"{p}.weight", _conv_pack(P[f"{p}.weight"])); vec(f"{p}.bias", P[f"{p}.bias"])
    vec("conv_norm_out.weight", P["conv_norm_out.weight"]); vec("conv_norm_out.bias", P["conv_norm_out.bias"])
    co = P["conv_out.weight"].shape[0]
    pad = (-co) % 4
    w = _conv_pack(P["conv_out.weight"]); bias = P["conv_out.bias"]
    if pad:
        w = torch.nn.functional.pad(w, (0, 0, 0, pad)); bias = torch.nn.functional.pad(bias, (0, pad))
    mat("conv_out.weight", w); vec("conv_out.bias", bias)
    return out


class PackedWeights:

    def __init__(self, entries: List[Tuple[str, torch.Tensor]], device):
        total = 0
        offs = []
        for _n, t in entries:
            total = (total + _ALIGN - 1) // _ALIGN * _ALIGN
            offs.append(total)
            total += t.numel() * t.element_size()
        self.blob = torch.empty(total + _ALIGN, dtype=torch.uint8, device=device)
        self.names = []
        for (name, t), off in zip(entries, offs):
            nb = t.numel() * t.element_size()
            self.blob[off:off + nb].copy_(t.reshape(-1).view(torch.uint8).to(device), non_blocking=False)
            self.names.append((name, off, nb))
        self.nbytes = total
        self._keep = [n.encode() for n, _, _ in self.names]
        arr = (_lib.WeightEntry * len(self.names))()
        for i, (n, off, nb) in enumerate(self.names):
            arr[i].name = self._keep[i]
            arr[i].offset = off
            arr[i].bytes = nb
        self.table = arr


def synthetic_mmdit_params(cfg, device="cpu", seed: int = 10086) -> Dict[str, torch.Tensor]:
    from .config import mmdit_param_shapes
    g = torch.Generator(device=device).manual_seed(seed)
    out = {}
    for name, shape in sorted(mmdit_param_shapes(cfg).items()):
        if name == "pos_embed.pos_embed":
            t = 0.5 * torch.randn(shape, generator=g, device=device)
        elif name.endswith(("norm_q.weight", "norm_k.weight", "norm_added_q.weight", "norm_added_k.weight")):
            t = 1.0 + 0.1 * torch.randn(shape, generator=g, device=device)
        elif name.endswith(".weight"):
            fan_in = 1
            for d in shape[1:]:
                fan_in *= d
            gain = 0.3 if (".norm1" in name or "norm_out" in name) else 1.0
            t = torch.randn(shape, generator=g, device=device) * gain * fan_in ** -0.5
        else:
            t = 0.05 * torch.randn(shape, generator=g, device=device)
        out[name] = t.to(torch.bfloat16)
    return out


def pack_mmdit(cfg, P: Dict[str, torch.Tensor]) -> List[Tuple[str, torch.Tensor]]:
    from .config import mmdit_param_shapes
    missing = [k for k in mmdit_param_shapes(cfg) if k not in P]
    if missing:
        raise KeyError(f"state dict lacks {len(missing)} tensors, e.g. {missing[:3]}")
    bf, f32 = torch.bfloat16, torch.float32
    out: List[Tuple[str, torch.Tensor]] = []

    def mat(name, t):
        out.append((name, t.to(bf).contiguous()))

    def vec(name, t):
        out.append((name, t.to(f32).contiguous()))

    def lin(dst, src):
        mat(f"{dst}.weight", P[f"{src}.weight"]); vec(f"{dst}.bias", P[f"{src}.bias"])

    d = cfg.dim
    mat("pos_embed.table", P["pos_embed.pos_embed"].reshape(-1, d))
    mat("pos_embed.proj.weight", _conv_pack(P["pos_embed.proj.weight"]))
    vec("pos_embed.proj.bias", P["pos_embed.proj.bias"])
    for n in ("time_text_embed.timestep_embedder.linear_1", "time_text_embed.timestep_embedder.linear_2",
              "time_text_embed.text_embedder.linear_1", "time_text_embed.text_embedder.linear_2", "context_embedder"):
        lin(n, n)
    ada_w, ada_b = [], []
    for i in range(cfg.num_layers):
        b = f"transformer_blocks.{i}"
        for n in (f"{b}.norm1.linear", f"{b}.norm1_context.linear"):
            ada_w.append(P[f"{n}.weight"]); ada_b.append(P[f"{n}.bias"])
    ada_w.append(P["norm_out.linear.weight"]); ada_b.append(P["norm_out.linear.bias"])
    mat("adaln_all.weight", torch.cat(ada_w, dim=0)); vec("adaln_all.bias", torch.cat(ada_b, dim=0))
    for i in range(cfg.num_layers):
        b = f"transformer_blocks.{i}"
        last = i == cfg.num_layers - 1
        dual = i in cfg.dual_attention_layers
        mat(f"{b}.attn.to_qkv.weight", torch.cat([P[f"{b}.attn.{n}.weight"] for n in ("to_q", "to_k", "to_v")], dim=0))
        vec(f"{b}.attn.to_qkv.bias", torch.cat([P[f"{b}.attn.{n}.bias"] for n in ("to_q", "to_k", "to_v")], dim=0))
        mat(f"{b}.attn.add_qkv.weight", torch.cat([P[f"{b}.attn.{n}.weight"] for n in ("add_q_proj", "add_k_proj", "add_v_proj")], dim=0))
        vec(f"{b}.attn.add_qkv.bias", torch.cat([P[f"{b}.attn.{n}.bias"] for n in ("add_q_proj", "add_k_proj", "add_v_proj")], dim=0))
        for n in ("norm_q", "norm_k", "norm_added_q", "norm_added_k"):
            vec(f"{b}.attn.{n}.weight", P[f"{b}.attn.{n}.weight"])
        lin(f"{b}.attn.to_out.0", f"{b}.attn.to_out.0")
        if not last:
            lin(f"{b}.attn.to_add_out", f"{b}.attn.to_add_out")
        if dual:
            mat(f"{b}.attn2.to_qkv.weight", torch.cat([P[f"{b}.attn2.{n}.weight"] for n in ("to_q", "to_k", "to_v")], dim=0))
            vec(f"{b}.attn2.to_qkv.bias", torch.cat([P[f"{b}.attn2.{n}.bias"] for n in ("to_q", "to_k", "to_v")], dim=0))
            for n in ("norm_q", "norm_k"):
                vec(f"{b}.attn2.{n}.weight", P[f"{b}.attn2.{n}.weight"])
            lin(f"{b}.attn2.to_out.0", f"{b}.attn2.to_out.0")
        lin(f"{b}.ff.net.0.proj", f"{b}.ff.net.0.proj"); lin(f"{b}.ff.net.2", f"{b}.ff.net.2")
        if not last:
            lin(f"{b}.ff_context.net.0.proj", f"{b}.ff_context.net.0.proj"); lin(f"{b}.ff_context.net.2", f"{b}.ff_context.net.2")
    lin("proj_out", "proj_out")
    return out
```

Baseline: 1.483 images/s.

## Fold ResNet 1x1 conv_shortcut into conv2 as extra K segment

For ResNet blocks whose input and output channel counts differ, the 1x1 shortcut projection is appended as an extra K segment of the conv2 3x3 implicit GEMM. The packed weight concatenates the conv2 and shortcut weights, and the two biases are summed. The DMA loader walks the nine taps and then the shortcut input rows. This removes a separate linear launch, the intermediate shortcut tensor write and the residual read in the epilogue. In exchange it adds a specialised v5 kernel form, only for 256-row tiles without split-K or grouping, plus extra weight memory for the duplicated packed weights.

New measurement: 1.493 images/s, median of 6. Within noise of the previous version (+0.7%).

```diff
diff --git a/include/mxdenoise.h b/include/mxdenoise.h
--- a/include/mxdenoise.h
+++ b/include/mxdenoise.h
@@ -98,6 +98,9 @@
   unsigned* ln_final_cnt;
   float* gn_part_out;
   int cin_valid;
+  const void* sc_a;
+  const void* sc_a2;
+  int sc_lda, sc_lda2, sc_cin, sc_k_split;
 } mx_gemm_desc;
 
 int mx_gemm(void* stream, const mx_gemm_desc* d);
@@ -106,10 +109,12 @@
 int mx_gemm_ln_prefers_pass(const mx_gemm_desc* d);
 int mx_gemm_ln_final_supported(const mx_gemm_desc* d);
 int mx_gemm_gn_partials_supported(const mx_gemm_desc* d, int conv);
+int mx_conv3x3_shortcut_supported(const mx_gemm_desc* d);
 enum { MX_FORM_TILE_GENERIC = 0, MX_FORM_TILE_256 = 1, MX_FORM_TILE_128 = 2, MX_FORM_PERSISTENT_256 = 3, MX_FORM_SMALL_M = 4, MX_FORM_CONV_SMALL_N = 5, MX_FORM_CONV_SMALL_CIN = 6 };
 int mx_gemm_form(const mx_gemm_desc* d, int conv);
 int mx_gemm_kernel_name(const mx_gemm_desc* d, int conv, int launch, char* buf, int cap);
 int mx_gemm_kernel_names(char* buf, int cap);
+int mx_conv3x3_shortcut_kernel_names(char* buf, int cap);
 int mx_attention_kernel_name(int B, int H, int Lq, int Lk, int ldo, int prescaled, int causal, int bias, int key_chunk, int force_cross, char* buf, int cap);
 int mx_attention_kernel_names(char* buf, int cap);
 #define MX_STATS_PITCH(slabs) (((slabs) + 3) & ~3)
diff --git a/sduss_amd/csrc/gemm_args.h b/sduss_amd/csrc/gemm_args.h
--- a/sduss_amd/csrc/gemm_args.h
+++ b/sduss_amd/csrc/gemm_args.h
@@ -54,6 +54,9 @@
   unsigned* sk_cnt;
   int nseg, mt_total;
   GemmSeg prob[kMaxSegs];
+  const bf16_t* sc_a;
+  const bf16_t* sc_a2;
+  int sc_lda, sc_lda2, sc_cin, sc_k1;
 };
 
 __device__ __forceinline__ int gemm_select_seg(GemmArgs& q, const GemmArgs& p, int& tm) {
diff --git a/sduss_amd/csrc/gemm_bf16.hip b/sduss_amd/csrc/gemm_bf16.hip
--- a/sduss_amd/csrc/gemm_bf16.hip
+++ b/sduss_amd/csrc/gemm_bf16.hip
@@ -231,7 +231,7 @@
     const double cost = (double)((tiles + ncu - 1) / ncu) * (rows + bn) * (bn == 256 ? v3_discount : 1.0);
     if (best.rows == 0 || cost < best_cost) { best = cands[c]; best_cost = cost; }
   }
-  if (d->splitk != 1 && best.rows == 128 && !d->a2 && d->K / 64 >= 16) {
+  if (d->splitk != 1 && best.rows == 128 && !d->a2 && !d->sc_a && d->K / 64 >= 16) {
     const int ncu = cu_count();
     const int nk = d->K / 64;
     double best_t = 0, unsplit_t = 0;
@@ -323,8 +323,27 @@
   }
 }
 
+static const char* sc_fold_error(const mx_gemm_desc* d) {
+  if (d->n_segs != 0) return "conv3x3: the folded shortcut excludes grouped launches";
+  if (d->stride != 1 || d->up != 0 || d->vhalo != 0 || d->corner_patch != 0 || d->cin_valid != 0)
+    return "conv3x3: the folded shortcut needs stride 1 and excludes upsampling, halo rows, the sliced corner rule and cin_valid";
+  if (d->flags != 0 || d->residual || d->rowbias || d->gate || d->out_scale != 0.f || d->stats_out || d->gn_part_out || d->ln_final_out)
+    return "conv3x3: the folded shortcut needs an epilogue of bias only";
+  if (d->sc_cin <= 0 || d->sc_cin % BK != 0 || 2 * d->sc_cin > 16384) return "conv3x3: sc_cin must be a multiple of 64 in (0, 8192]";
+  const int k1 = d->sc_a2 ? d->sc_k_split : d->sc_cin;
+  if (d->sc_a2 && (k1 <= 0 || k1 >= d->sc_cin || k1 % BK != 0)) return "conv3x3: sc_k_split must be a multiple of 64 inside (0, sc_cin)";
+  if (d->sc_lda < k1 || d->sc_lda % 8 != 0 || ((uintptr_t)d->sc_a & 15) != 0) return "conv3x3: bad sc_lda / sc_a alignment";
+  if (d->sc_a2 && (d->sc_lda2 < d->sc_cin - k1 || d->sc_lda2 % 8 != 0 || ((uintptr_t)d->sc_a2 & 15) != 0)) return "conv3x3: bad sc_lda2 / sc_a2 alignment";
+  if ((long)d->M * d->sc_lda >= 2147483647L || (d->sc_a2 && (long)d->M * d->sc_lda2 >= 2147483647L)) return "conv3x3: shortcut operand exceeds 32-bit indexing";
+  return nullptr;
+}
+
 static int gemm_kernel_of(const mx_gemm_desc* d, bool conv, const TileChoice& tc) {
   if (d->ln_final && tc.bn != 256) return -1;
+  if (d->sc_a) {
+    if (!conv || sc_fold_error(d) != nullptr || tc.rows != 256 || tc.bn == 256 || tc.bn == 0) return -1;
+    return tc.bn == 160 ? GK_V5_160_CONV_SC : GK_V5_128_CONV_SC;
+  }
   if (small_m_serves(d, conv)) return small_m_form(d->N, d->K, d->flags);
   if (conv && conv_small_n_serves(d)) return GK_CONV_SMALL_N;
   if (conv && conv_small_cin_serves(d)) return GK_CONV_SMALL_CIN;
@@ -418,6 +437,13 @@
     a.ln_final = d->ln_final;
   }
   a.nseg = d->n_segs; a.mt_total = 0;
+  a.sc_a = nullptr; a.sc_a2 = nullptr; a.sc_lda = 0; a.sc_lda2 = 0; a.sc_cin = 0; a.sc_k1 = 0;
+  if (d->sc_a) {
+    MX_CHECK(conv, "gemm: sc_a is mx_conv3x3's (the shortcut input of mx_gemm is its A operand)");
+    if (const char* e = sc_fold_error(d)) MX_CHECK(false, e);
+    a.sc_a = (const bf16_t*)d->sc_a; a.sc_a2 = (const bf16_t*)d->sc_a2; a.sc_lda = d->sc_lda; a.sc_lda2 = d->sc_a2 ? d->sc_lda2 : 0;
+    a.sc_cin = d->sc_cin; a.sc_k1 = d->sc_a2 ? d->sc_k_split : d->sc_cin;
+  }
   const bool grouped = d->n_segs > 0;
   if (d->ln_stats) {
     MX_CHECK(!conv && d->ln_colsum && d->ln_slabs > 0, "gemm: folded LayerNorm needs ln_colsum and ln_slabs > 0 (mx_gemm only)");
@@ -433,7 +459,7 @@
   } else if (!conv) {
     MX_CHECK(d->lda >= d->K && d->lda % 8 == 0, "gemm: lda must be >= K and a multiple of 8");
   } else {
-    MX_CHECK(d->Cin % BK == 0 && d->K == 9 * d->Cin, "conv3x3: Cin must be a multiple of 64 and K = 9*Cin");
+    MX_CHECK(d->Cin % BK == 0 && d->K == 9 * d->Cin + (d->sc_a ? d->sc_cin : 0), "conv3x3: Cin must be a multiple of 64 and K = 9*Cin (+ sc_cin with a folded shortcut)");
     MX_CHECK(d->stride == 1 || d->stride == 2, "conv3x3: stride must be 1 or 2");
     MX_CHECK(d->up == 0 || d->up == 1, "conv3x3: up must be 0 or 1");
     MX_CHECK(!(d->up && d->stride != 1), "conv3x3: upsample only with stride 1");
@@ -549,9 +575,9 @@
   dim3 block(256);
   hipStream_t s = (hipStream_t)stream;
   if (prof_enabled()) {
-    const double kk = conv ? 9.0 * d->Cin : (double)d->K;
+    const double kk = conv && !d->sc_a ? 9.0 * d->Cin : (double)d->K;
     const double Mt = (double)rows_of(d);
-    double in_elems = conv ? (double)d->B * d->Hin * d->Win * d->Cin : Mt * d->K;
+    double in_elems = conv ? (double)d->B * d->Hin * d->Win * d->Cin + (d->sc_a ? Mt * d->sc_cin : 0.0) : Mt * d->K;
     if (conv && grouped) { in_elems = 0; for (int i = 0; i < d->n_segs; ++i) in_elems += (double)d->segs[i].B * d->segs[i].Hin * d->segs[i].Win * d->Cin; }
     const double flops = 2.0 * Mt * (double)d->N * kk;
     const double bytes = 2.0 * (in_elems + (double)d->N * d->K + Mt * d->N);
@@ -561,6 +587,7 @@
   const int mt128 = grouped ? a.mt_total : cdiv(d->M, BM);
   if (d->ln_final) MX_CHECK(v2bn == 256, "gemm: ln_final is the 256 x 256 kernel's form of the folded LayerNorm; this shape does not run there (use ln_stats)");
   const int form = gemm_kernel_of(d, conv, tc);
+  if (d->sc_a) MX_CHECK(form >= 0, "conv3x3: this shape does not take a 256-row tile, where the folded shortcut runs (mx_conv3x3_shortcut_supported)");
   MX_CHECK(form >= 0, v2bn == 256 ? "gemm: no 256 x 256 instantiation serves ln_final with this epilogue (GEGLU, QKV or plain bias only)"
                                    : "gemm: no kernel instantiation serves this descriptor");
   if (is_small_m_form(form)) {
@@ -656,6 +683,10 @@
   const mx::TileChoice tc = mx::pick_tile(d, conv != 0);
   return tc.rows == 256 && tc.bn != 256 && tc.bn != 0 && tc.splitk <= 1;
 }
+extern "C" int mx_conv3x3_shortcut_supported(const mx_gemm_desc* d) {
+  if (!d || !d->sc_a || d->M <= 0 || d->N <= 0 || d->K <= 0 || d->Cin <= 0 || d->Cin % 64 != 0 || d->K != 9 * d->Cin + d->sc_cin) return 0;
+  return mx::gemm_kernel_of(d, true, mx::pick_tile(d, true)) >= 0;
+}
 extern "C" int mx_gemm_ln_final_supported(const mx_gemm_desc* d) {
   if (!d || d->n_segs > 0 || d->M <= 0 || d->N <= 0 || d->K <= 0) return 0;
   mx_gemm_desc q = *d;
@@ -674,7 +705,9 @@
 static const char* const kGemmKernelNames[GK_COUNT] = {
   MX_GEMM_GENERIC_FORMS(MX_FORM_NAME_T) MX_GEMM_V2_FORMS(MX_FORM_NAME_T) MX_GEMM_V5_FORMS(MX_FORM_NAME_T) MX_GEMM_V4_FORMS(MX_FORM_NAME_T)
   MX_GEMM_SMALL_M_FORMS(MX_FORM_NAME_T) MX_GEMM_CONV_SMALL_FORMS(MX_FORM_NAME_P)
+  MX_GEMM_V5_SC_FORMS(MX_FORM_NAME_T)
 };
+static_assert(GK_V5_160_CONV_SC == GK_PLAIN_COUNT && GK_COUNT == GK_PLAIN_COUNT + 2, "the folded-shortcut forms follow the plain ones");
 }
 extern "C" int mx_gemm_kernel_name(const mx_gemm_desc* d, int conv, int launch, char* buf, int cap) {
   if (!d || mx::rows_of(d) <= 0 || d->N <= 0 || d->K <= 0 || launch < 0) return -1;
@@ -686,4 +719,7 @@
   if (form < 0) return -1;
   return mx::copy_name(mx::kGemmKernelNames[form], buf, cap);
 }
-extern "C" int mx_gemm_kernel_names(char* buf, int cap) { return mx::join_names(mx::kGemmKernelNames, mx::GK_COUNT, buf, cap); }
+extern "C" int mx_gemm_kernel_names(char* buf, int cap) { return mx::join_names(mx::kGemmKernelNames, mx::GK_PLAIN_COUNT, buf, cap); }
+extern "C" int mx_conv3x3_shortcut_kernel_names(char* buf, int cap) {
+  return mx::join_names(mx::kGemmKernelNames + mx::GK_PLAIN_COUNT, mx::GK_COUNT - mx::GK_PLAIN_COUNT, buf, cap);
+}
diff --git a/sduss_amd/csrc/gemm_bf16_v2.hip b/sduss_amd/csrc/gemm_bf16_v2.hip
--- a/sduss_amd/csrc/gemm_bf16_v2.hip
+++ b/sduss_amd/csrc/gemm_bf16_v2.hip
@@ -34,6 +34,7 @@
   const int k_first = pk.splitk > 1 ? (int)((long)nk_all * slice / pk.splitk) : 0;
   const int nk = pk.splitk > 1 ? (int)((long)nk_all * (slice + 1) / pk.splitk) - k_first : nk_all;
   constexpr bool SPLIT_K = true;
+  constexpr bool SCUT = false;
 #include "gemm_dma_loader.inc"
   auto issue_next = [&](int stage) __attribute__((always_inline)) { issue_group(stage); advance_cursor(); };
 
diff --git a/sduss_amd/csrc/gemm_bf16_v5.hip b/sduss_amd/csrc/gemm_bf16_v5.hip
--- a/sduss_amd/csrc/gemm_bf16_v5.hip
+++ b/sduss_amd/csrc/gemm_bf16_v5.hip
@@ -17,12 +17,22 @@
   gemm_v5_tile<BN, MI, CONV, FEAT, GEGLU, VEC>(pk, tm, tn, smem);
 }
 
+template <int BN>
+__global__ __launch_bounds__(512, 2) void gemm_v5_conv_sc_kernel(const GemmArgs pk) {
+  constexpr int STAGE_ELEMS = (64 * 4 + BN) * DMA_BK;
+  __shared__ __attribute__((aligned(16))) bf16_t smem[NSTAGE5 * STAGE_ELEMS];
+  int tm, tn;
+  gemm_tile_of_block(blockIdx.x, gemm_m_tiles(pk, 64 * 4), pk.N / BN, pk.xcd_map, tm, tn);
+  gemm_v5_tile<BN, 4, true, 0, false, false, false, true>(pk, tm, tn, smem);
+}
+
 int launch_v5(hipStream_t s, const GemmArgs& a, int bn, int rows, int form) {
   const int tiles = (a.nseg > 0 ? a.mt_total : cdiv(a.M, rows)) * (a.N / bn);
   dim3 grid(tiles), block(512);
   switch (form) {
 #define MX_V5(id, k, targs) case id: hipLaunchKernelGGL((k<MX_FORM_UNPAREN targs>), grid, block, 0, s, a); return 0;
     MX_GEMM_V5_FORMS(MX_V5)
+    MX_GEMM_V5_SC_FORMS(MX_V5)
 #undef MX_V5
     default: return 1;
   }
diff --git a/sduss_amd/csrc/gemm_dma_loader.inc b/sduss_amd/csrc/gemm_dma_loader.inc
--- a/sduss_amd/csrc/gemm_dma_loader.inc
+++ b/sduss_amd/csrc/gemm_dma_loader.inc
@@ -11,6 +11,7 @@
   int cb[XI], cy[XI], cx[XI];
   unsigned xchb[XI];
   int tap_next = 0, in_tap = 0;
+  [[maybe_unused]] int tap_len = tiles_per_tap;
 
   auto conv_set_tap = [&](int tap, int cbyte = 0) __attribute__((always_inline)) {
     const int dy = tap / 3 - 1;
@@ -29,6 +30,17 @@
       const bool ok = (cb[i] >= 0) && (iy >= -p.vhalo) && (iy < Hv + p.vhalo) && (ix >= 0) && (ix < Wv);
       const long off = ((((long)cb[i] * (p.Hin + 2 * p.vhalo) + (iy >> p.up) + p.vhalo) * p.Win + (ix >> p.up)) * p.Cin) * 2;
       xsrc[i] = (ok ? reinterpret_cast<const char*>(p.a) + off + cbyte : zero) + xchb[i];
+    }
+  };
+
+  [[maybe_unused]] auto sc_set_src = [&](int seg) __attribute__((always_inline)) {
+    const char* base = reinterpret_cast<const char*>(seg == 0 ? p.sc_a : p.sc_a2);
+    const long ld = seg == 0 ? p.sc_lda : p.sc_lda2;
+    tap_len = (seg == 0 ? p.sc_k1 : p.sc_cin - p.sc_k1) / DMA_BK;
+#pragma unroll
+    for (int i = 0; i < XI; ++i) {
+      const long m = tm * BM + ((i * 512 + tid) >> 3);
+      xsrc[i] = (cb[i] >= 0 ? base + m * ld * 2 : zero) + xchb[i];
     }
   };
 
@@ -103,6 +115,15 @@
       const bool to_a2 = p.a2 != nullptr && is_kt * DMA_BK == p.k_split;
 #pragma unroll
       for (int i = 0; i < XI; ++i) xsrc[i] += DMA_BK * 2 + (to_a2 ? xjump[i] : 0L);
+    } else if constexpr (SCUT) {
+      if (++in_tap == tap_len) {
+        in_tap = 0;
+        if (++tap_next < 9) conv_set_tap(tap_next);
+        else sc_set_src(tap_next - 9);
+      } else {
+#pragma unroll
+        for (int i = 0; i < XI; ++i) xsrc[i] += DMA_BK * 2;
+      }
     } else {
       if (++in_tap == tiles_per_tap) {
         in_tap = 0;
diff --git a/sduss_amd/csrc/gemm_forms.h b/sduss_amd/csrc/gemm_forms.h
--- a/sduss_amd/csrc/gemm_forms.h
+++ b/sduss_amd/csrc/gemm_forms.h
@@ -36,6 +36,10 @@
   T(GK_V5_128_QKV, gemm_v5_kernel, (128, 4, false, EPI_F_QKV, false, false))          \
   T(GK_V5_128_ALL, gemm_v5_kernel, (128, 4, false, EPI_F_ALL, false, true))
 
+#define MX_GEMM_V5_SC_FORMS(T)                                                        \
+  T(GK_V5_160_CONV_SC, gemm_v5_conv_sc_kernel, (160))                                 \
+  T(GK_V5_128_CONV_SC, gemm_v5_conv_sc_kernel, (128))
+
 #define MX_GEMM_V4_FORMS(T)                                                 \
   T(GK_V4_GEGLU_LN, gemm_v4_kernel, (false, 0, true, true))                 \
   T(GK_V4_QKV_LN, gemm_v4_kernel, (false, EPI_F_QKV, false, true))          \
@@ -71,6 +75,9 @@
 #define MX_FORM_ID_P(id, k) id,
   MX_GEMM_GENERIC_FORMS(MX_FORM_ID_T) MX_GEMM_V2_FORMS(MX_FORM_ID_T) MX_GEMM_V5_FORMS(MX_FORM_ID_T) MX_GEMM_V4_FORMS(MX_FORM_ID_T)
   MX_GEMM_SMALL_M_FORMS(MX_FORM_ID_T) MX_GEMM_CONV_SMALL_FORMS(MX_FORM_ID_P)
+  GK_PLAIN_COUNT,
+  GK_SC_FIRST_ = GK_PLAIN_COUNT - 1,
+  MX_GEMM_V5_SC_FORMS(MX_FORM_ID_T)
 #undef MX_FORM_ID_T
 #undef MX_FORM_ID_P
   GK_COUNT
diff --git a/sduss_amd/csrc/gemm_v5_body.h b/sduss_amd/csrc/gemm_v5_body.h
--- a/sduss_amd/csrc/gemm_v5_body.h
+++ b/sduss_amd/csrc/gemm_v5_body.h
@@ -16,7 +16,7 @@
 #define MX5_STAMP(slot) do {} while (0)
 #endif
 
-template <int BN, int MI, bool CONV, int FEAT, bool GEGLU, bool VEC, bool WT = false>
+template <int BN, int MI, bool CONV, int FEAT, bool GEGLU, bool VEC, bool WT = false, bool SCUT = false>
 __device__ __forceinline__ void gemm_v5_tile(const GemmArgs& pk, int tm, const int tn, bf16_t* const smem) {
   constexpr int BM5 = 64 * MI;
   constexpr int NI = BN / 32;
@@ -99,6 +99,7 @@
   if (!group_b) MX_BAR();
 
   const int m0 = tm * BM5, n0 = tn * BN;
+  static_assert(!SCUT || CONV, "the shortcut segment follows the taps of a conv");
   static_assert(!GEGLU || (NI % 4 == 0 && !CONV), "the gated epilogue pairs whole 32-feature halves");
   gemm_epilogue_regs<NI, MI, GEGLU, VEC, true, true, FEAT, true, false, WT>(p, acc, m0 + wm * 16 * MI, n0 + wn * (BN / 2), fr, fq, ln_rstd);
   if constexpr (!GEGLU && FEAT == 0 && MI == 4) {
diff --git a/sduss_amd/csrc/unet_sdxl.cpp b/sduss_amd/csrc/unet_sdxl.cpp
--- a/sduss_amd/csrc/unet_sdxl.cpp
+++ b/sduss_amd/csrc/unet_sdxl.cpp
@@ -373,18 +373,25 @@
     if (stats_out) return gemm_with_stats(d, *stats_out, finalise);
     return gemm(d, false);
   }
+  struct ScFold { const bf16_t* a; int lda; const bf16_t* a2; int lda2; int cin; int k_split; };
   int conv_cin_valid = 0;
   bool conv(const bf16_t* x, int Hin, int Win, int Cin, const std::string& prefix, bf16_t* out, int Cout, int stride, int up,
             int corner_patch, const float* rowbias = nullptr, int ldrb = 0, const void* residual = nullptr, int vhalo = 0, float* gn_part = nullptr,
-            bool* gn_done = nullptr) {
+            bool* gn_done = nullptr, const ScFold* sc = nullptr, bool* sc_done = nullptr) {
     mx_gemm_desc d; std::memset(&d, 0, sizeof(d));
     d.vhalo = vhalo;
     const int Hv = Hin << up, Wv = Win << up;
-    d.a = x; d.w = wb(prefix + ".weight", (size_t)Cout * 9 * Cin); d.bias = wf(prefix + ".bias", Cout);
+    d.a = x;
+    if (sc) {
+      d.sc_a = sc->a; d.sc_lda = sc->lda; d.sc_a2 = sc->a2; d.sc_lda2 = sc->lda2; d.sc_cin = sc->cin; d.sc_k_split = sc->k_split;
+      d.w = wb(prefix + "_sc.weight", (size_t)Cout * (9 * Cin + sc->cin)); d.bias = wf(prefix + "_sc.bias", Cout);
+    } else {
+      d.w = wb(prefix + ".weight", (size_t)Cout * 9 * Cin); d.bias = wf(prefix + ".bias", Cout);
+    }
     d.c = out; d.ldc = Cout; d.B = gB[0]; d.Hin = Hin; d.Win = Win; d.Cin = Cin;
     d.Hout = (Hv + stride - 1) / stride; d.Wout = (Wv + stride - 1) / stride; d.stride = stride; d.up = up;
     d.corner_patch = corner_patch;
-    d.M = gB[0] * d.Hout * d.Wout; d.N = Cout; d.K = 9 * Cin;
+    d.M = gB[0] * d.Hout * d.Wout; d.N = Cout; d.K = 9 * Cin + (sc ? sc->cin : 0);
     d.rowbias = rowbias; d.ldrb = ldrb; d.rows_per_batch = d.Hout * d.Wout;
     d.residual = residual; d.ldr = Cout;
     mx_gemm_seg sg[MX_MAX_SEGS];
@@ -405,6 +412,10 @@
     }
     if (gn_part && gn_done && ng == 1 && mx_gemm_gn_partials_supported(&d, 1)) { d.gn_part_out = gn_part; *gn_done = true; }
     d.cin_valid = conv_cin_valid;
+    if (sc) {
+      *sc_done = ok() && ng == 1 && mx_conv3x3_shortcut_supported(&d) != 0;
+      if (!*sc_done) return ok();
+    }
     return gemm(d, true);
   }
   bool groupnorm(const bf16_t* x, bf16_t* y, const std::string& prefix, int h, int wd, int C, float eps, bool silu, int patch,
@@ -465,6 +476,10 @@
     stage_hit = true;
   }
 
+  static bool sc_fold_enabled() {
+    static const bool on = [] { const char* e = getenv("MX_CONV_SHORTCUT_FOLD"); return !(e && e[0] == '0'); }();
+    return on;
+  }
   int level_patch(int level) const { return gn_patch > 0 ? std::max(gn_patch >> level, 1) : 0; }
 
   bf16_t* resnet(const std::string& p, const bf16_t* x, int h, int wd, int Cin, int Cout, int level, const bf16_t* x2 = nullptr, int C2 = 0) {
@@ -527,14 +542,21 @@
     if (gdone) groupnorm_from_partials(h1, n2, p + ".norm2", h, wd, Cout, u->cfg.norm_eps, true, gpart, wf(p + ".conv1.bias", Cout),
                                        temb_all ? temb_all + (temb_off - Cout) : nullptr, temb_total);
     else groupnorm(h1, n2, p + ".norm2", h, wd, Cout, u->cfg.norm_eps, true, patch);
-    const bf16_t* sc = x;
-    if (Cin != Cout) {
-      bf16_t* s2 = alloc<bf16_t>((size_t)M * Cout);
-      if (x2) linear(x, C1, p + ".conv_shortcut.weight", p + ".conv_shortcut.bias", s2, Cout, M, Cout, Cin, nullptr, 0, 0, 0.f, x2, C2);
-      else linear(x, Cin, p + ".conv_shortcut.weight", p + ".conv_shortcut.bias", s2, Cout, M, Cout, Cin);
-      sc = s2;
-    }
-    conv(n2, h, wd, Cout, p + ".conv2", out, Cout, 1, 0, patch, nullptr, 0, sc);
+    bool folded = false;
+    if (Cin != Cout && ng == 1 && patch == 0 && sc_fold_enabled() && u->table.count(p + ".conv2_sc.weight") != 0) {
+      const ScFold f = {x, x2 ? C1 : Cin, x2, C2, Cin, x2 ? C1 : 0};
+      conv(n2, h, wd, Cout, p + ".conv2", out, Cout, 1, 0, patch, nullptr, 0, nullptr, 0, nullptr, nullptr, &f, &folded);
+    }
+    if (!folded) {
+      const bf16_t* sc = x;
+      if (Cin != Cout) {
+        bf16_t* s2 = alloc<bf16_t>((size_t)M * Cout);
+        if (x2) linear(x, C1, p + ".conv_shortcut.weight", p + ".conv_shortcut.bias", s2, Cout, M, Cout, Cin, nullptr, 0, 0, 0.f, x2, C2);
+        else linear(x, Cin, p + ".conv_shortcut.weight", p + ".conv_shortcut.bias", s2, Cout, M, Cout, Cin);
+        sc = s2;
+      }
+      conv(n2, h, wd, Cout, p + ".conv2", out, Cout, 1, 0, patch, nullptr, 0, sc);
+    }
     ar.release(m);
     dump(p, out, (size_t)M * Cout);
     return out;
@@ -828,10 +850,14 @@
     const int ctx = c.cross_attention_dim;
 
     ln_cnt = (unsigned*)ar.alloc((size_t)kLnCnt * sizeof(unsigned));
-    if (ok() && !quiet() && ln_cnt && hipMemsetAsync(ln_cnt, 0, (size_t)kLnCnt * sizeof(unsigned), stream) != hipSuccess) fail("ln tickets: memset failed");
+    if (ok() && !quiet() && ln_cnt) {
+      const hipError_t e = hipMemsetAsync(ln_cnt, 0, (size_t)kLnCnt * sizeof(unsigned), stream);
+      if (e != hipSuccess) fail(std::string("ln tickets: memset failed: ") + hipGetErrorString(e));
+    }
     tail_rows = 0;
     for (int g = 0; g < ng; ++g) tail_rows += (long)gB[g] * gH[g] * gW[g];
-    if (tail_rows > 0 && tail_rows < 2147483647L) {
+    tail_sync = nullptr;
+    if (mx_attn_tail_preferred() != 0 && tail_rows > 0 && tail_rows < 2147483647L) {
       const size_t nb = mx_attn_tail_sync_bytes((int)tail_rows);
       tail_sync = (unsigned*)ar.alloc(nb);
       if (ok() && !quiet() && tail_sync && hipMemsetAsync(tail_sync, 0, nb, stream) != hipSuccess) fail("attention tail tickets: memset failed");
diff --git a/sduss_amd/lib.py b/sduss_amd/lib.py
--- a/sduss_amd/lib.py
+++ b/sduss_amd/lib.py
@@ -44,6 +44,7 @@
         ("ln_stats", C.c_void_p), ("ln_colsum", C.c_void_p), ("ln_slabs", C.c_int), ("ln_eps", C.c_float), ("stats_out", C.c_void_p),
         ("segs", C.POINTER(GemmSeg)), ("n_segs", C.c_int), ("splitk", C.c_int),
         ("ln_final", C.c_void_p), ("ln_final_out", C.c_void_p), ("ln_final_cnt", C.c_void_p), ("gn_part_out", C.c_void_p), ("cin_valid", C.c_int),
+        ("sc_a", C.c_void_p), ("sc_a2", C.c_void_p), ("sc_lda", C.c_int), ("sc_lda2", C.c_int), ("sc_cin", C.c_int), ("sc_k_split", C.c_int),
     ]
 
 
@@ -193,9 +194,11 @@
     "mx_gemm_ln_final_supported": (_i, [C.POINTER(GemmDesc)]),
     "mx_gemm_launches": (_i, [C.POINTER(GemmDesc)]),
     "mx_gemm_gn_partials_supported": (_i, [C.POINTER(GemmDesc), _i]),
+    "mx_conv3x3_shortcut_supported": (_i, [C.POINTER(GemmDesc)]),
     "mx_gemm_form": (_i, [C.POINTER(GemmDesc), _i]),
     "mx_gemm_kernel_name": (_i, [C.POINTER(GemmDesc), _i, _i, C.c_char_p, _i]),
     "mx_gemm_kernel_names": (_i, [C.c_char_p, _i]),
+    "mx_conv3x3_shortcut_kernel_names": (_i, [C.c_char_p, _i]),
     "mx_attention_kernel_name": (_i, [_i, _i, _i, _i, _i, _i, _i, _i, _i, _i, C.c_char_p, _i]),
     "mx_attention_kernel_names": (_i, [C.c_char_p, _i]),
     "mx_groupnorm_nhwc_from_partials": (_i, [_vp, _vp, _vp, _vp, _vp, _i, _i, _i, _i, _i, C.c_float, _i, _vp, _i, _vp, _vp, _i, _vp]),
@@ -303,6 +306,10 @@
     return _name_list(load().mx_gemm_kernel_names)
 
 
+def conv_shortcut_kernel_names() -> list:
+    return _name_list(load().mx_conv3x3_shortcut_kernel_names)
+
+
 def attention_kernel_names() -> list:
     return _name_list(load().mx_attention_kernel_names)
 
diff --git a/sduss_amd/weights.py b/sduss_amd/weights.py
--- a/sduss_amd/weights.py
+++ b/sduss_amd/weights.py
@@ -62,6 +62,13 @@
     if pad_in and pad_in > i:
         w = torch.nn.functional.pad(w, (0, pad_in - i))
     return w.reshape(o, -1).contiguous()
+
+
+def pack_conv_shortcut(w2: torch.Tensor, b2: torch.Tensor, wsc: torch.Tensor, bsc: torch.Tensor):
+    bf, f32 = torch.bfloat16, torch.float32
+    cout, cin = wsc.shape[0], wsc.shape[1]
+    w = torch.cat([_conv_pack(w2).to(bf), wsc.reshape(cout, cin).to(bf)], dim=1).contiguous()
+    return w, (b2.to(f32) + bsc.to(f32)).contiguous()
 
 
 def fold_layernorm(w: torch.Tensor, bias: Optional[torch.Tensor], gamma: torch.Tensor, beta: torch.Tensor):
@@ -127,6 +134,8 @@
         if cin != cout:
             mat(f"{p}.conv_shortcut.weight", P[f"{p}.conv_shortcut.weight"].reshape(cout, cin))
             vec(f"{p}.conv_shortcut.bias", P[f"{p}.conv_shortcut.bias"])
+            w_sc, b_sc = pack_conv_shortcut(P[f"{p}.conv2.weight"], P[f"{p}.conv2.bias"], P[f"{p}.conv_shortcut.weight"], P[f"{p}.conv_shortcut.bias"])
+            mat(f"{p}.conv2_sc.weight", w_sc); vec(f"{p}.conv2_sc.bias", b_sc)
     kv_by_dim: Dict[int, List[torch.Tensor]] = {}
     for p, dim, _h, layers in transformer_names(cfg):
         vec(f"{p}.norm.weight", P[f"{p}.norm.weight"]); vec(f"{p}.norm.bias", P[f"{p}.norm.bias"])
```
